# PKU-VCL-Geometry/GeoSplatting

Measured on AMD Instinct MI355X. Metric: fwd+bwd views/sec at 2M Gaussians, 800x800, higher is better.
Workload: dtype f32

## Files before the change

geosplatting_amd/_lib.py:

```python
from __future__ import annotations

import ctypes as C
import os
from typing import Optional

import torch

_HERE = os.path.dirname(os.path.abspath(__file__))
LIB_PATH = os.path.join(_HERE, "libgeosplat_hip.so")

GS_MAX_LEVELS = 16


class GsEnv(C.Structure):
    _fields_ = [("lut", C.c_void_p), ("lut_res", C.c_int), ("base", C.c_void_p), ("base_res", C.c_int),
                ("num_levels", C.c_int), ("levels", C.c_void_p * GS_MAX_LEVELS), ("res", C.c_int * GS_MAX_LEVELS),
                ("min_roughness", C.c_float), ("max_roughness", C.c_float)]


class GsTailView(C.Structure):
    _fields_ = [("viewmat", C.c_void_p), ("K", C.c_void_p), ("cam_pos", C.c_void_p), ("vis_records", C.c_void_p), ("v_packed", C.c_void_p),
                ("packed_index", C.c_void_p), ("W", C.c_int), ("H", C.c_int)]


class GsTileLevel(C.Structure):
    _fields_ = [("R", C.c_int), ("n_mirrors", C.c_int), ("margin", C.c_int), ("bw", C.c_int), ("nb", C.c_int), ("tile_begin", C.c_int),
                ("tile_end", C.c_int), ("reserved", C.c_int), ("src", C.c_void_p), ("scale", C.c_void_p), ("out_scale", C.c_void_p),
                ("bounds", C.c_void_p), ("tiles", C.c_void_p), ("segments", C.c_void_p), ("row_begin", C.c_void_p), ("row_counts", C.c_void_p),
                ("desc", C.c_void_p), ("weights", C.c_void_p), ("dst", C.c_void_p), ("lds_bytes", C.c_size_t)]


class GsDensifyTensor(C.Structure):
    _fields_ = [("src", C.c_void_p), ("dst", C.c_void_p), ("floats_per_row", C.c_int), ("kind", C.c_int)]


class GsTsdfView(C.Structure):
    _fields_ = [("depth_alpha", C.c_void_p), ("viewmat", C.c_void_p), ("K", C.c_void_p), ("W", C.c_int), ("H", C.c_int)]


class GsEnvGrad(C.Structure):
    _fields_ = [("base", C.c_void_p), ("levels", C.c_void_p * GS_MAX_LEVELS)]


SYMBOLS = [
    "gs_last_error", "gs_version", "gs_project_ws_bytes", "gs_project_fwd", "gs_project_fwd_vis", "gs_project_fwd_vis_ex", "gs_isect_emit", "gs_sort_ws_bytes",
    "gs_isect_sort", "gs_isect_bin_ws_bytes", "gs_isect_bin", "gs_isect_offsets", "gs_raster_ws_bytes", "gs_raster_fwd", "gs_raster_prepare", "gs_raster_prepare_vis", "gs_raster_composite", "gs_raster_grad_stride", "gs_raster_bwd", "gs_raster_bwd_acc", "gs_selftest_rcp", "gs_selftest_exp", "gs_selftest_cube_edges", "gs_isect_bin_cap", "gs_isect_offsets_cap", "gs_isect_bin_tiles_cap", "gs_isect_offsets_tiles_cap", "gs_raster_prepare_vis_cap", "gs_raster_composite_cap", "gs_raster_bwd_cap", "gs_raster_bwd_acc_cap", "gs_raster_composite_tone", "gs_raster_bwd_tone_acc", "gs_raster_log_ws_bytes", "gs_raster_composite_tone_log", "gs_raster_bwd_tone_log_acc", "gs_project_bwd_cap", "gs_project_bwd", "gs_project_bwd_ex", "gs_shade_fwd",
    "gs_shade_bwd_ws_bytes", "gs_shade_bwd_plan_blocks", "gs_shade_bwd", "gs_tonemap_fwd", "gs_tonemap_bwd", "gs_tonemap_fwd3", "gs_tonemap_bwd3", "gs_cubemap_mip_fwd", "gs_cubemap_mip_chain_fwd", "gs_cube_sample_linear",
    "gs_cubemap_mip_bwd", "gs_diffuse_cubemap_fwd", "gs_diffuse_cubemap_bwd", "gs_specular_bounds", "gs_specular_bounds_ws_bytes", "gs_specular_bounds_fast", "gs_cube_dir_table",
    "gs_specular_cubemap_fwd", "gs_specular_cubemap_bwd", "gs_specular_tiles_count", "gs_specular_tiles_fill",
    "gs_specular_tiles_check", "gs_specular_tiles_apply", "gs_specular_tiles_apply_multi", "gs_mgadapter_fwd", "gs_mgadapter_bwd", "gs_vertex_normals_fwd",
    "gs_vertex_normals_bwd", "gs_photo_loss_ws_bytes", "gs_photo_loss", "gs_smooth_loss_ws_bytes", "gs_smooth_loss", "gs_hashgrid_fwd", "gs_hashgrid_bwd_ws_bytes", "gs_hashgrid_bwd", "gs_hashgrid_bwd_fixed_ws_bytes", "gs_hashgrid_bwd_fixed", "gs_mlp_wgrad_ws_bytes", "gs_mlp_wgrad",
    "gs_flexicubes_ws_bytes", "gs_flexicubes_count", "gs_flexicubes_fwd", "gs_flexicubes_bwd", "gs_flexicubes_entropy_fwd",
    "gs_flexicubes_entropy_bwd", "gs_front_ws_bytes", "gs_front_fwd", "gs_isect_bin_front_ws_bytes", "gs_isect_bin_front", "gs_isect_bin_front_classes", "gs_tail_bwd", "gs_tail_bwd_multi", "gs_tail_bwd_multi_parts", "gs_tail_priv_ws_bytes", "gs_tail_priv_reduce", "gs_smooth_gather", "gs_smooth_fold", "gs_activation_chain",
    "gs_densify_stats", "gs_densify_ws_bytes", "gs_densify_plan", "gs_densify_fill",
    "gs_surfel_project_ws_bytes", "gs_surfel_project_fwd", "gs_surfel_project_bwd", "gs_surfel_raster_fwd", "gs_surfel_grad_stride",
    "gs_surfel_raster_bwd",
    "gs_tsdf_integrate", "gs_tsdf_extract_ws_bytes", "gs_tsdf_extract_count", "gs_tsdf_extract_fill",
    "gs_meshraster_ws_bytes", "gs_meshraster_fwd", "gs_meshraster_resolve", "gs_meshraster_bwd", "gs_mesh_interp_fwd",
    "gs_mesh_interp_bwd",
    "gs_mesh_topology_bytes", "gs_mesh_topology_build", "gs_meshaa_fwd", "gs_meshaa_bwd",
    "gs_tex2d_fwd", "gs_tex2d_bwd", "gs_meshshade_fwd", "gs_meshshade_bwd",
    "gs_bvh_bytes", "gs_bvh_ws_bytes", "gs_bvh_build", "gs_ray_occluded", "gs_ray_closest",
    "gs_envshade_fwd", "gs_envshade_bwd",
    "gs_denoise_tiled_fits", "gs_denoise_fwd", "gs_denoise_bwd",
]

_lib: Optional[C.CDLL] = None


class GeoSplatHipError(RuntimeError):
    pass


def lib() -> C.CDLL:
    global _lib
    if _lib is None:
        if not os.path.exists(LIB_PATH):
            raise GeoSplatHipError(
                f"{LIB_PATH} not found: build it with `python -m geosplatting_amd.build` "
                "(hipcc --offload-arch=gfx950).  geosplatting_amd has no CPU / PyTorch fallback.")
        l = C.CDLL(LIB_PATH)
        l.gs_last_error.restype = C.c_char_p
        l.gs_project_ws_bytes.restype = C.c_size_t
        l.gs_project_ws_bytes.argtypes = [C.c_int]
        l.gs_sort_ws_bytes.restype = C.c_size_t
        l.gs_sort_ws_bytes.argtypes = [C.c_int64, C.c_int, C.c_int]
        l.gs_isect_bin_ws_bytes.restype = C.c_size_t
        l.gs_isect_bin_ws_bytes.argtypes = [C.c_int, C.c_int64, C.c_int, C.c_int]
        l.gs_shade_bwd_ws_bytes.restype = C.c_size_t
        l.gs_shade_bwd_ws_bytes.argtypes = [C.c_void_p, C.c_int]
        l.gs_shade_bwd_plan_blocks.restype = C.c_int
        l.gs_shade_bwd_plan_blocks.argtypes = [C.c_void_p, C.c_int, C.c_int, C.c_void_p]
        l.gs_hashgrid_bwd_ws_bytes.restype = C.c_size_t
        l.gs_hashgrid_bwd_ws_bytes.argtypes = [C.c_int, C.c_int, C.c_int]
        l.gs_hashgrid_bwd_fixed_ws_bytes.restype = C.c_size_t
        l.gs_hashgrid_bwd_fixed_ws_bytes.argtypes = [C.c_int, C.c_int, C.c_int, C.c_int]
        l.gs_mlp_wgrad_ws_bytes.restype = C.c_size_t
        l.gs_mlp_wgrad_ws_bytes.argtypes = [C.c_int64]
        l.gs_flexicubes_ws_bytes.restype = C.c_size_t
        l.gs_flexicubes_ws_bytes.argtypes = [C.c_int, C.c_int, C.c_int]
        l.gs_photo_loss_ws_bytes.restype = C.c_size_t
        l.gs_photo_loss_ws_bytes.argtypes = [C.c_int, C.c_int]
        l.gs_smooth_loss_ws_bytes.restype = C.c_size_t
        l.gs_smooth_loss_ws_bytes.argtypes = [C.c_int, C.c_int]
        l.gs_specular_bounds_ws_bytes.restype = C.c_size_t
        l.gs_specular_bounds_ws_bytes.argtypes = [C.c_int]
        l.gs_front_ws_bytes.restype = C.c_size_t
        l.gs_front_ws_bytes.argtypes = [C.c_int]
        l.gs_isect_bin_front_ws_bytes.restype = C.c_size_t
        l.gs_isect_bin_front_ws_bytes.argtypes = [C.c_int, C.c_int64, C.c_int, C.c_int]
        l.gs_tail_priv_ws_bytes.restype = C.c_size_t
        l.gs_tail_priv_ws_bytes.argtypes = [C.c_void_p, C.c_int]
        l.gs_raster_log_ws_bytes.restype = C.c_size_t
        l.gs_raster_log_ws_bytes.argtypes = [C.c_int64, C.c_int, C.c_int, C.c_int]
        l.gs_raster_ws_bytes.restype = C.c_size_t
        l.gs_raster_ws_bytes.argtypes = [C.c_int64, C.c_int, C.c_int, C.c_int, C.c_int]
        l.gs_densify_ws_bytes.restype = C.c_size_t
        l.gs_densify_ws_bytes.argtypes = [C.c_int64, C.c_int]
        l.gs_surfel_project_ws_bytes.restype = C.c_size_t
        l.gs_surfel_project_ws_bytes.argtypes = [C.c_int]
        l.gs_tsdf_extract_ws_bytes.restype = C.c_size_t
        l.gs_tsdf_extract_ws_bytes.argtypes = [C.c_int, C.c_int, C.c_int]
        l.gs_tsdf_integrate.argtypes = [C.c_int, C.c_int, C.c_int, C.c_float, C.c_float, C.c_float, C.c_float, C.c_float, C.c_float,
                                        C.c_float, C.c_int, C.c_void_p, C.c_void_p, C.c_void_p]
        l.gs_tsdf_extract_count.argtypes = [C.c_int, C.c_int, C.c_int, C.c_void_p, C.c_void_p, C.c_size_t, C.c_void_p, C.c_void_p]
        l.gs_tsdf_extract_fill.argtypes = [C.c_int, C.c_int, C.c_int, C.c_float, C.c_float, C.c_float, C.c_float, C.c_void_p,
                                           C.c_void_p, C.c_size_t, C.c_int64, C.c_int64, C.c_void_p, C.c_void_p, C.c_void_p]
        l.gs_meshraster_ws_bytes.restype = C.c_size_t
        l.gs_meshraster_ws_bytes.argtypes = [C.c_int64, C.c_int, C.c_int]
        mesh_head = [C.c_int64, C.c_int64, C.c_void_p, C.c_void_p, C.c_float, C.c_float, C.c_float, C.c_float, C.c_int, C.c_int, C.c_float]
        l.gs_meshraster_fwd.argtypes = mesh_head + [C.c_int, C.c_void_p, C.c_size_t, C.c_void_p, C.c_void_p]
        l.gs_meshraster_resolve.argtypes = mesh_head + [C.c_void_p, C.c_size_t, C.c_void_p, C.c_void_p]
        l.gs_meshraster_bwd.argtypes = mesh_head + [C.c_void_p, C.c_void_p, C.c_void_p, C.c_void_p]
        l.gs_mesh_interp_fwd.argtypes = [C.c_int64, C.c_int, C.c_int64, C.c_int64, C.c_int, C.c_void_p, C.c_void_p, C.c_void_p, C.c_void_p,
                                         C.c_void_p]
        l.gs_mesh_interp_bwd.argtypes = [C.c_int64, C.c_int, C.c_int64, C.c_int64, C.c_int, C.c_void_p, C.c_void_p, C.c_void_p, C.c_void_p,
                                         C.c_void_p, C.c_void_p, C.c_void_p]
        l.gs_mesh_topology_bytes.restype = C.c_size_t
        l.gs_mesh_topology_bytes.argtypes = [C.c_int64]
        l.gs_mesh_topology_build.argtypes = [C.c_int64, C.c_void_p, C.c_void_p, C.c_size_t, C.c_void_p]
        aa_head = mesh_head + [C.c_int, C.c_void_p, C.c_size_t, C.c_int, C.c_void_p, C.c_void_p]
        l.gs_meshaa_fwd.argtypes = aa_head + [C.c_void_p, C.c_void_p, C.c_void_p]
        l.gs_meshaa_bwd.argtypes = aa_head + [C.c_void_p, C.c_void_p, C.c_void_p, C.c_void_p]
        tex_head = [C.c_int64, C.c_int, C.c_int, C.c_int, C.c_int, C.c_void_p, C.c_void_p]
        l.gs_tex2d_fwd.argtypes = tex_head + [C.c_void_p, C.c_void_p]
        l.gs_tex2d_bwd.argtypes = tex_head + [C.c_void_p, C.c_void_p, C.c_void_p, C.c_void_p]
        shade_head = [C.c_int, C.c_int, C.c_void_p, C.c_void_p, C.c_void_p, C.c_void_p, C.c_int, C.c_int, C.c_void_p, C.c_int, C.c_int,
                      C.c_void_p, C.c_void_p, C.c_void_p, C.c_int, C.c_float, C.c_int]
        l.gs_meshshade_fwd.argtypes = shade_head + [C.c_void_p, C.c_void_p]
        l.gs_meshshade_bwd.argtypes = shade_head + [C.c_void_p] * 8
        l.gs_bvh_bytes.restype = C.c_size_t
        l.gs_bvh_bytes.argtypes = [C.c_int64]
        l.gs_bvh_ws_bytes.restype = C.c_size_t
        l.gs_bvh_ws_bytes.argtypes = [C.c_int64]
        l.gs_bvh_build.argtypes = [C.c_int64, C.c_int64, C.c_void_p, C.c_void_p, C.c_void_p, C.c_size_t, C.c_void_p, C.c_size_t, C.c_void_p]
        ray_head = [C.c_int64, C.c_int64, C.c_void_p, C.c_void_p, C.c_void_p, C.c_int64, C.c_int, C.c_void_p, C.c_void_p, C.c_int,
                    C.c_float, C.c_float]
        l.gs_ray_occluded.argtypes = ray_head + [C.c_void_p, C.c_void_p]
        l.gs_ray_closest.argtypes = ray_head + [C.c_void_p, C.c_void_p, C.c_void_p, C.c_void_p]
        env_head = ([C.c_int64] + [C.c_void_p] * 7 + [C.c_int, C.c_int] + [C.c_void_p] * 4 + [C.c_int, C.c_int, C.c_void_p, C.c_int64, C.c_int,
                    C.c_float, C.c_int64, C.c_int64, C.c_void_p, C.c_void_p, C.c_void_p, C.c_int])
        l.gs_envshade_fwd.argtypes = env_head + [C.c_void_p] * 7
        l.gs_envshade_bwd.argtypes = env_head + [C.c_int] + [C.c_void_p] * 8
        l.gs_denoise_tiled_fits.argtypes = [C.c_int, C.c_double]
        l.gs_denoise_fwd.argtypes = [C.c_int] * 5 + [C.c_void_p] * 3 + [C.c_double, C.c_int] + [C.c_void_p] * 3
        l.gs_denoise_bwd.argtypes = [C.c_int] * 5 + [C.c_void_p] * 2 + [C.c_double, C.c_int] + [C.c_void_p] * 4
        _lib = l
    return _lib


def check(rc: int, what: str) -> None:
    if rc != 0:
        raise GeoSplatHipError(f"{what} failed ({rc}): {lib().gs_last_error().decode()}")


def ptr(t: Optional[torch.Tensor]) -> Optional[C.c_void_p]:
    if t is None:
        return None
    assert t.is_cuda and t.is_contiguous(), "device-resident contiguous tensors only"
    return C.c_void_p(t.data_ptr())


def stream() -> C.c_void_p:
    return C.c_void_p(torch.cuda.current_stream().cuda_stream)


def f32(x: float) -> C.c_float:
    return C.c_float(float(x))


def i64(x: int) -> C.c_int64:
    return C.c_int64(int(x))


def require_cuda(*tensors: torch.Tensor) -> None:
    for t in tensors:
        if t is not None and not t.is_cuda:
            raise GeoSplatHipError("geosplatting_amd ops run on the GPU only (tensor on %s); there is no CPU path" % t.device)


_shared_streams = {}


def shared_stream(device: torch.device, role: str) -> "torch.cuda.Stream":
    key = (device.index if device.index is not None else torch.cuda.current_device(), role)
    st = _shared_streams.get(key)
# ... 4 lines not shown
```

geosplatting_amd/csrc/gs_raster.hip:

```cpp
#include "gs_common.h"
#include "gs_tone.h"
#include <stdlib.h>

#pragma clang fp contract(off)

#define GS_TILE 16
#define GS_ALPHA_MIN (1.0f / 255.0f)

#ifdef GS_RASTER_STATS
__device__ unsigned long long g_raster_stats[8];
extern "C" int gs_raster_stats_read(unsigned long long* host8, int reset)
{
    if (hipMemcpyFromSymbol(host8, HIP_SYMBOL(g_raster_stats), sizeof(unsigned long long) * 8) != hipSuccess) return -1;
    if (reset) { unsigned long long z[8] = {0}; if (hipMemcpyToSymbol(HIP_SYMBOL(g_raster_stats), z, sizeof(z)) != hipSuccess) return -1; }
    return 0;
}
__device__ unsigned long long g_raster_stats2[8];
extern "C" int gs_raster_stats2_read(unsigned long long* host8, int reset)
{
    if (hipMemcpyFromSymbol(host8, HIP_SYMBOL(g_raster_stats2), sizeof(unsigned long long) * 8) != hipSuccess) return -1;
    if (reset) { unsigned long long z[8] = {0}; if (hipMemcpyToSymbol(HIP_SYMBOL(g_raster_stats2), z, sizeof(z)) != hipSuccess) return -1; }
    return 0;
}
__device__ unsigned long long g_raster_stats3[8];
// ... 1277 lines not shown
                    m2 = __builtin_elementwise_fma(sd, d, m2);
                    mxy = fmaf(sd.x, d.y, mxy);
                    c01 = __builtin_elementwise_fma((v2f)(f_w), v2f{vr.x, vr.y}, c01);
                    if (CD > 2) c2s = fmaf(f_w, vr.z, c2s);
                } while (__ballot(m != 0ull) != 0ull);
                sum[0] = m0; sum[1] = m1.x; sum[2] = m1.y; sum[3] = m2.x; sum[4] = mxy; sum[5] = m2.y;
                sum[6] = c01.x;
                if (CD > 1) sum[7] = c01.y;
                if (CD > 2) sum[8] = c2s;
            }
            lanes_lds_sync();
#ifdef GS_RASTER_PHASES
            if (blockIdx.x == 0 && threadIdx.x == 0) { const long long _t = (long long)__builtin_readcyclecounter(); atomicAdd(&g_raster_stats[3], (unsigned long long)(_t - _pw0)); _pw0 = _t; }
#endif
            {
                const float ga = ra4.z, gb = ra4.w, gc = rb4.x, go = rb4.y;
                const float M0 = sum[0], Mx = sum[1], My = sum[2];
                float out[NV];
                out[0] = (2.0f * ga) * Mx + gb * My;
                out[1] = gb * Mx + (2.0f * gc) * My;
                out[2] = 0.5f * sum[3]; out[3] = sum[4]; out[4] = 0.5f * sum[5];
                out[5] = (M0 != 0.0f) ? -M0 / go : 0.0f;
#pragma unroll
                for (int k = 0; k < CD; ++k) out[6 + k] = sum[6 + k];
                if (mine) {
#pragma unroll
                    for (int k = 0; k < NV; ++k) stage[lane * NV + k] = out[k];
                }
            }
            lanes_lds_sync();
            {
                const int r = lane / NV, k = lane - r * NV;
                for (int it = 0; r0 + it * RPI < r1; ++it) {
                    const int j = r0 + it * RPI + r;
                    if (r < RPI && j < r1 && k < 6 + D) {
                        const float v = stage[j * NV + k];
                        if (v != 0.0f) {
                            const int g = __float_as_int(qc[j].w);
                            gs_atomic_add(v_packed + (size_t)g * rec_stride + k, v);
                        }
                    }
                }
            }
#ifdef GS_RASTER_PHASES
            if (blockIdx.x == 0 && threadIdx.x == 0) atomicAdd(&g_raster_stats[4], (unsigned long long)((long long)__builtin_readcyclecounter() - _pw0));
#endif
            cumbase = __builtin_amdgcn_readlane(cum, r1 - 1);
            r0 = r1;
        }
    }
#if defined(GS_RASTER_STATS) && !defined(GS_RASTER_PHASES)
    if (lane == 0) {
#pragma unroll
        for (int k = 0; k < 8; ++k) if (walk_hist[k]) atomicAdd(&g_raster_stats3[k], (unsigned long long)walk_hist[k]);
    }
#endif
    GS_TL_END();
}

#define GS_RASTER_BLOCKS_PER_CU 4
static int gs_raster_blocks_per_cu() { return GS_RASTER_BLOCKS_PER_CU; }
static size_t gs_raster_lds_pad() { return (size_t)(160 * 1024 / gs_raster_blocks_per_cu()) - 1024; }
static size_t gs_raster_lds(size_t natural)
{
    const size_t pad = gs_raster_lds_pad();
    if (natural >= pad) return natural;
    if ((size_t)(gs_raster_blocks_per_cu() + 1) * (natural + 512) > (size_t)160 * 1024) return natural;
    return pad;
}
static size_t align256(size_t x) { return (x + 255) & ~(size_t)255; }

extern "C" size_t gs_raster_ws_bytes(int64_t n_isects, int V, int W, int H, int tile_size)
{
    if (tile_size <= 0) return 0;
    const size_t tiles = (size_t)((W + tile_size - 1) / tile_size) * (size_t)((H + tile_size - 1) / tile_size);
    const size_t n = n_isects > 0 ? (size_t)n_isects : 1;
    const size_t v = V > 0 ? (size_t)V : 1;
    return 3 * align256(n * sizeof(float4)) + align256(tiles * sizeof(int32_t)) + align256(64 * sizeof(int32_t)) +
           align256(64 * tiles * sizeof(int32_t)) + align256(4 * v * sizeof(float4));
}

struct RasterWs {
    float4 *rec0, *rec1, *rec2;
    int32_t* order;
    BwdOrder bo;
    float4* vis;
};
static RasterWs carve(void* ws, int64_t n_isects, int V, int tiles)
{
    const size_t n = n_isects > 0 ? (size_t)n_isects : 1;
    const size_t v = V > 0 ? (size_t)V : 1;
    char* p = (char*)ws;
    RasterWs r;
    r.rec0 = (float4*)p; p += align256(n * sizeof(float4));
    r.rec1 = (float4*)p; p += align256(n * sizeof(float4));
    r.rec2 = (float4*)p; p += align256(n * sizeof(float4));
    r.order = (int32_t*)p; p += align256((size_t)tiles * sizeof(int32_t));
    r.bo.bcount = (int32_t*)p; p += align256(64 * sizeof(int32_t));
    r.bo.blist = (int32_t*)p; p += align256(64 * (size_t)tiles * sizeof(int32_t));
    r.vis = (float4*)p;
    return r;
}

struct RasterOpts {
    const int64_t* counts = nullptr;
    ToneFwd tone_fwd = { 0, nullptr, nullptr };
    ToneBwd tone_bwd = { 0, nullptr, nullptr, nullptr, nullptr };
    CullLog log = { nullptr, nullptr, nullptr };
};
static GsCount isect_count(int64_t n, const RasterOpts& o)
{
    return GsCount{ (long long)n, o.counts ? (const long long*)o.counts + 1 : nullptr };
}

template <int CD>
static int launch_fwd(int W, int H, int D, const RasterWs& ws, const float* colors, const float* background,
                      int64_t n_isects, const int32_t* offsets, float* render, float* alphas, int32_t* last_ids,
                      hipStream_t s, const RasterOpts& o)
{
    const int tile_w = (W + GS_TILE - 1) / GS_TILE, tile_h = (H + GS_TILE - 1) / GS_TILE;
    if (o.tone_fwd.image && !(CD == 3 && D == 3 && background == nullptr)) {
        gs_set_error("gs_raster_composite_tone: needs D == 3 and no background");
        return GS_EINVAL;
    }
    {
        const size_t planes = CD > 3 ? 4 * (size_t)2 * (size_t)D * 64 * sizeof(float) : 0;
        const size_t lds = gs_raster_lds(4 * (size_t)GS_WIN_Q_BYTES + planes);
        if (lds > 64 * 1024)
            GS_CHECK_HIP(hipFuncSetAttribute((const void*)raster_fwd_window_kernel<CD>, hipFuncAttributeMaxDynamicSharedMemorySize, (int)lds));
        hipLaunchKernelGGL(raster_fwd_window_kernel<CD>, dim3(tile_w * tile_h), dim3(256), lds, s, W, H, tile_w, tile_w * tile_h, D,
                           ws.order, ws.rec0, ws.rec1, ws.rec2, colors, background, isect_count(n_isects, o), offsets, render, alphas,
                           last_ids, o.tone_fwd, o.log, o.log.count ? ws.bo : BwdOrder{ nullptr, nullptr });
        GS_CHECK_LAUNCH();
        return GS_OK;
    }
}

static int raster_check(const char* who, int W, int H, int tile_size, int D, int V, int64_t n_isects, const void* ws,
                        size_t ws_bytes)
{
    GS_CHECK_ARG(W > 0 && H > 0, "bad image size");
    GS_CHECK_ARG(tile_size == GS_TILE, "only tile_size=16 is built (rfstudio/model/gsplat.py:30)");
    GS_CHECK_ARG(D >= 1 && D <= GS_MAX_CHANNELS, "1 <= D <= 32");
    GS_CHECK_ARG(n_isects >= 0 && n_isects < (1ll << 31), "n_isects must fit int32");
    GS_CHECK_ARG(ws != nullptr, "workspace must not be NULL");
    GS_CHECK_ARG(V >= 0, "bad V");
    if (ws_bytes < gs_raster_ws_bytes(n_isects, V, W, H, tile_size)) { gs_set_error("%s: workspace too small", who); return GS_ENOSPC; }
    return GS_OK;
}

static int raster_prepare_impl(int W, int H, int tile_size, int D, int V, const float* means2d, const float* conics,
                               const float* opacities, const float* colors, const float* vis_records, int64_t n_isects,
                               const int32_t* offsets, const int32_t* flatten_ids, void* ws, size_t ws_bytes, void* stream,
                               const RasterOpts& o)
{
    const int rc = raster_check("gs_raster_prepare", W, H, tile_size, D, V, n_isects, ws, ws_bytes);
    if (rc != GS_OK) return rc;
    hipStream_t s = (hipStream_t)stream;
    const int tiles = ((W + GS_TILE - 1) / GS_TILE) * ((H + GS_TILE - 1) / GS_TILE);
    const RasterWs r = carve(ws, n_isects, V, tiles);
    if (n_isects > 0 && V > 0) {
        const float4* vis = (const float4*)vis_records;
        if (!vis) {
            hipLaunchKernelGGL(pack_visible_kernel, dim3(gs_cdiv(V, 256)), dim3(256), 0, s, V, D, means2d, conics, opacities, colors,
                               r.vis);
            GS_CHECK_LAUNCH();
            vis = r.vis;
        }
        hipLaunchKernelGGL(build_stream_packed_kernel, dim3(gs_cdiv(n_isects, 256)), dim3(256), 0, s, isect_count(n_isects, o), flatten_ids,
                           vis, r.rec0, r.rec1, r.rec2);
        GS_CHECK_LAUNCH();
    }
    hipLaunchKernelGGL(tile_order_kernel, dim3(1), dim3(1024), 0, s, tiles, isect_count(n_isects, o), offsets, r.order, r.bo);
    GS_CHECK_LAUNCH();
    return GS_OK;
}

static int raster_composite_impl(int W, int H, int tile_size, int D, int V, const float* colors, const float* background,
                                 int64_t n_isects, const int32_t* offsets, float* render, float* alphas, int32_t* last_ids,
                                 const void* ws, size_t ws_bytes, void* stream, const RasterOpts& o)
{
    const int rc = raster_check("gs_raster_composite", W, H, tile_size, D, V, n_isects, ws, ws_bytes);
    if (rc != GS_OK) return rc;
    hipStream_t s = (hipStream_t)stream;
    const int tiles = ((W + GS_TILE - 1) / GS_TILE) * ((H + GS_TILE - 1) / GS_TILE);
    const RasterWs r = carve((void*)ws, n_isects, V, tiles);
#define GS_FWD(CD) return launch_fwd<CD>(W, H, D, r, colors, background, n_isects, offsets, render, alphas, last_ids, s, o)
    if (D <= 3) GS_FWD(3);
    if (D <= 4) GS_FWD(4);
    if (D <= 8) GS_FWD(8);
    if (D <= 16) GS_FWD(16);
    GS_FWD(32);
#undef GS_FWD
}

template <int CD>
static int launch_bwd(int W, int H, int D, const RasterWs& ws, const float* colors, const float* background,
                      int64_t n_isects, const int32_t* offsets, const float* alphas, const int32_t* last_ids,
                      const float* v_render, const float* v_alphas, float* v_packed, int rec_stride, hipStream_t s,
                      const RasterOpts& o)
{
    const int tile_w = (W + GS_TILE - 1) / GS_TILE, tile_h = (H + GS_TILE - 1) / GS_TILE;
    if (o.tone_bwd.v_image && !(CD == 3 && D == 3 && background == nullptr)) {
        gs_set_error("gs_raster_bwd_tone: needs D == 3 and no background");
        return GS_EINVAL;
    }
    if constexpr (CD <= 3) {
        if (o.log.idx) {
            const size_t lds = gs_raster_lds(4 * (size_t)LogLds::WAVE_BYTES);
            hipLaunchKernelGGL(raster_bwd_log_kernel<CD>, dim3(tile_w * tile_h), dim3(256), lds, s, W, H, tile_w, tile_w * tile_h, D,
                               ws.order, ws.rec0, ws.rec1, ws.rec2, background, isect_count(n_isects, o), offsets, alphas, last_ids,
                               v_render, v_alphas, v_packed, rec_stride, o.tone_bwd, o.log, ws.bo);
            GS_CHECK_LAUNCH();
            return GS_OK;
        }
    }
    {
        size_t lds = 4 * ((size_t)Lanes2Lds<CD>::WAVE_BYTES + (CD > 3 ? 2 * (size_t)D * 64 * 4 : 0));
        if (lds < gs_raster_lds_pad()) lds = gs_raster_lds_pad();
        if (lds > 64 * 1024)
            GS_CHECK_HIP(hipFuncSetAttribute((const void*)raster_bwd_lanes2_kernel<CD>, hipFuncAttributeMaxDynamicSharedMemorySize, (int)lds));
        hipLaunchKernelGGL(raster_bwd_lanes2_kernel<CD>, dim3(tile_w * tile_h), dim3(256), lds, s, W, H, tile_w, tile_w * tile_h, D,
                           ws.order, ws.rec0, ws.rec1, ws.rec2, colors, background, isect_count(n_isects, o), offsets, alphas, last_ids,
                           v_render, v_alphas, v_packed, rec_stride, o.tone_bwd);
        GS_CHECK_LAUNCH();
        return GS_OK;
    }
}

extern "C" int gs_raster_grad_stride(int D) { return ((6 + D) + 15) / 16 * 16; }

static int raster_bwd_impl(int W, int H, int tile_size, int D, int V, const float* colors, const float* background,
                           int64_t n_isects, const int32_t* offsets, const float* alphas, const int32_t* last_ids,
                           const float* v_render, const float* v_alphas, float* v_packed, const void* ws,
                           size_t ws_bytes, void* stream, bool zero, const RasterOpts& o)
{
    const int rc = raster_check("gs_raster_bwd", W, H, tile_size, D, V, n_isects, ws, ws_bytes);
    if (rc != GS_OK) return rc;
    hipStream_t s = (hipStream_t)stream;
    const int rec_stride = gs_raster_grad_stride(D);
    if (V > 0 && zero) GS_CHECK_HIP(gs_zero_async(v_packed, sizeof(float) * (size_t)rec_stride * (size_t)V, s));
    if (n_isects == 0 || V == 0) return GS_OK;
    const int tiles = ((W + GS_TILE - 1) / GS_TILE) * ((H + GS_TILE - 1) / GS_TILE);
    const RasterWs r = carve((void*)ws, n_isects, V, tiles);
#define GS_BWD(CD) return launch_bwd<CD>(W, H, D, r, colors, background, n_isects, offsets, alphas, last_ids, v_render, v_alphas, v_packed, rec_stride, s, o)
    if (D <= 3) GS_BWD(3);
    if (D <= 4) GS_BWD(4);
    if (D <= 8) GS_BWD(8);
    if (D <= 16) GS_BWD(16);
    GS_BWD(32);
#undef GS_BWD
}

static CullLog carve_log(const void* log_ws, int64_t n_isects)
{
    const size_t n = n_isects > 0 ? (size_t)n_isects : 1;
    char* p = (char*)log_ws;
    CullLog l;
    l.mask = (unsigned long long*)p; p += align256(4 * n * sizeof(unsigned long long));
    l.idx = (int32_t*)p; p += align256(4 * n * sizeof(int32_t));
    l.count = (int32_t*)p;
    return l;
}
extern "C" size_t gs_raster_log_ws_bytes(int64_t n_isects, int W, int H, int tile_size)
{
    if (tile_size <= 0) return 0;
    const size_t n = n_isects > 0 ? (size_t)n_isects : 1;
    const size_t tiles = (size_t)((W + tile_size - 1) / tile_size) * (size_t)((H + tile_size - 1) / tile_size);
    return align256(4 * n * sizeof(unsigned long long)) + align256(4 * n * sizeof(int32_t)) + align256(4 * tiles * sizeof(int32_t));
}

extern "C" int gs_raster_prepare(int W, int H, int tile_size, int D, int V, const float* means2d, const float* conics,
                                 const float* opacities, const float* colors, int64_t n_isects, const int32_t* offsets,
                                 const int32_t* flatten_ids, void* ws, size_t ws_bytes, void* stream)
{
    return raster_prepare_impl(W, H, tile_size, D, V, means2d, conics, opacities, colors, nullptr, n_isects, offsets, flatten_ids,
                               ws, ws_bytes, stream, RasterOpts{});
}

extern "C" int gs_raster_prepare_vis(int W, int H, int tile_size, int D, int V, const float* vis_records, int64_t n_isects,
                                     const int32_t* offsets, const int32_t* flatten_ids, void* ws, size_t ws_bytes, void* stream)
{
    GS_CHECK_ARG(vis_records != nullptr || V == 0, "vis_records (written by gs_project_fwd_vis) must not be NULL");
    return raster_prepare_impl(W, H, tile_size, D, V, nullptr, nullptr, nullptr, nullptr, vis_records, n_isects, offsets,
                               flatten_ids, ws, ws_bytes, stream, RasterOpts{});
}

extern "C" int gs_raster_composite(int W, int H, int tile_size, int D, int V, const float* colors, const float* background,
                                   int64_t n_isects, const int32_t* offsets, float* render, float* alphas,
                                   int32_t* last_ids, const void* ws, size_t ws_bytes, void* stream)
{
    return raster_composite_impl(W, H, tile_size, D, V, colors, background, n_isects, offsets, render, alphas, last_ids, ws,
                                 ws_bytes, stream, RasterOpts{});
}

extern "C" int gs_raster_fwd(int W, int H, int tile_size, int D, int V, const float* means2d, const float* conics,
                             const float* opacities, const float* colors, const float* background,
                             int64_t n_isects, const int32_t* offsets, const int32_t* flatten_ids,
                             float* render, float* alphas, int32_t* last_ids, void* ws, size_t ws_bytes, void* stream)
{
    const int rc = raster_prepare_impl(W, H, tile_size, D, V, means2d, conics, opacities, colors, nullptr, n_isects, offsets,
                                       flatten_ids, ws, ws_bytes, stream, RasterOpts{});
    if (rc != GS_OK) return rc;
    return raster_composite_impl(W, H, tile_size, D, V, colors, background, n_isects, offsets, render, alphas, last_ids, ws,
                                 ws_bytes, stream, RasterOpts{});
}

extern "C" int gs_raster_bwd(int W, int H, int tile_size, int D, int V, const float* colors, const float* background,
                             int64_t n_isects, const int32_t* offsets, const float* alphas, const int32_t* last_ids,
                             const float* v_render, const float* v_alphas, float* v_packed, const void* ws,
                             size_t ws_bytes, void* stream)
{
    return raster_bwd_impl(W, H, tile_size, D, V, colors, background, n_isects, offsets, alphas, last_ids, v_render, v_alphas,
                           v_packed, ws, ws_bytes, stream, true, RasterOpts{});
}

extern "C" int gs_raster_bwd_acc(int W, int H, int tile_size, int D, int V, const float* colors, const float* background,
                                 int64_t n_isects, const int32_t* offsets, const float* alphas, const int32_t* last_ids,
                                 const float* v_render, const float* v_alphas, float* v_packed, const void* ws,
                                 size_t ws_bytes, void* stream)
{
    return raster_bwd_impl(W, H, tile_size, D, V, colors, background, n_isects, offsets, alphas, last_ids, v_render, v_alphas,
                           v_packed, ws, ws_bytes, stream, false, RasterOpts{});
}

extern "C" int gs_raster_prepare_vis_cap(int W, int H, int tile_size, int D, int V_cap, const float* vis_records, int64_t n_isects_cap,
                                         const int64_t* counts_dev, const int32_t* offsets, const int32_t* flatten_ids, void* ws,
                                         size_t ws_bytes, void* stream)
{
    GS_CHECK_ARG(counts_dev != nullptr, "counts_dev must not be NULL");
    GS_CHECK_ARG(vis_records != nullptr || V_cap == 0, "vis_records (written by gs_project_fwd_vis) must not be NULL");
    RasterOpts o;
    o.counts = counts_dev;
    return raster_prepare_impl(W, H, tile_size, D, V_cap, nullptr, nullptr, nullptr, nullptr, vis_records, n_isects_cap, offsets,
                               flatten_ids, ws, ws_bytes, stream, o);
}

extern "C" int gs_raster_composite_cap(int W, int H, int tile_size, int D, int V_cap, const float* colors, const float* background,
                                       int64_t n_isects_cap, const int64_t* counts_dev, const int32_t* offsets, float* render,
                                       float* alphas, int32_t* last_ids, const void* ws, size_t ws_bytes, void* stream)
{
    GS_CHECK_ARG(counts_dev != nullptr, "counts_dev must not be NULL");
    RasterOpts o;
    o.counts = counts_dev;
    return raster_composite_impl(W, H, tile_size, D, V_cap, colors, background, n_isects_cap, offsets, render, alphas, last_ids, ws,
                                 ws_bytes, stream, o);
}

extern "C" int gs_raster_bwd_cap(int W, int H, int tile_size, int D, int V_cap, const float* colors, const float* background,
                                 int64_t n_isects_cap, const int64_t* counts_dev, const int32_t* offsets, const float* alphas,
                                 const int32_t* last_ids, const float* v_render, const float* v_alphas, float* v_packed, const void* ws,
                                 size_t ws_bytes, void* stream)
{
    GS_CHECK_ARG(counts_dev != nullptr, "counts_dev must not be NULL");
    RasterOpts o;
    o.counts = counts_dev;
    return raster_bwd_impl(W, H, tile_size, D, V_cap, colors, background, n_isects_cap, offsets, alphas, last_ids, v_render, v_alphas,
                           v_packed, ws, ws_bytes, stream, true, o);
}

extern "C" int gs_raster_bwd_acc_cap(int W, int H, int tile_size, int D, int V_cap, const float* colors, const float* background,
                                     int64_t n_isects_cap, const int64_t* counts_dev, const int32_t* offsets, const float* alphas,
                                     const int32_t* last_ids, const float* v_render, const float* v_alphas, float* v_packed,
                                     const void* ws, size_t ws_bytes, void* stream)
{
    GS_CHECK_ARG(counts_dev != nullptr, "counts_dev must not be NULL");
    RasterOpts o;
    o.counts = counts_dev;
    return raster_bwd_impl(W, H, tile_size, D, V_cap, colors, background, n_isects_cap, offsets, alphas, last_ids, v_render, v_alphas,
                           v_packed, ws, ws_bytes, stream, false, o);
}

extern "C" int gs_raster_composite_tone(int W, int H, int tile_size, int V, const float* colors, int64_t n_isects,
                                        const int64_t* counts_dev, const int32_t* offsets, float* render, float* alphas,
                                        int32_t* last_ids, int tone_mode, const float* exposure, float* image, const void* ws,
                                        size_t ws_bytes, void* stream)
{
    GS_CHECK_ARG(tone_mode >= 0 && tone_mode <= 2 && exposure != nullptr && image != nullptr, "bad tone mode / exposure / image");
    RasterOpts o;
    o.counts = counts_dev;
    o.tone_fwd = ToneFwd{ tone_mode, exposure, (float4*)image };
    return raster_composite_impl(W, H, tile_size, 3, V, colors, nullptr, n_isects, offsets, render, alphas, last_ids, ws, ws_bytes,
                                 stream, o);
}

extern "C" int gs_raster_bwd_tone_acc(int W, int H, int tile_size, int V, const float* colors, int64_t n_isects,
                                      const int64_t* counts_dev, const int32_t* offsets, const float* render, const float* alphas,
                                      const int32_t* last_ids, int tone_mode, const float* exposure, const float* v_image,
                                      float* v_packed, float* v_exposure, const void* ws, size_t ws_bytes, void* stream)
{
    GS_CHECK_ARG(tone_mode >= 0 && tone_mode <= 2 && exposure != nullptr && v_image != nullptr && render != nullptr && v_exposure != nullptr,
                 "bad tone mode / exposure / v_image / render / v_exposure");
    RasterOpts o;
    o.counts = counts_dev;
    o.tone_bwd = ToneBwd{ tone_mode, exposure, render, (const float4*)v_image, v_exposure };
    return raster_bwd_impl(W, H, tile_size, 3, V, colors, nullptr, n_isects, offsets, alphas, last_ids, nullptr, nullptr, v_packed, ws,
                           ws_bytes, stream, false, o);
}

extern "C" int gs_raster_composite_tone_log(int W, int H, int tile_size, int V, const float* colors, int64_t n_isects,
                                            const int64_t* counts_dev, const int32_t* offsets, float* render, float* alphas,
                                            int32_t* last_ids, int tone_mode, const float* exposure, float* image, const void* ws,
                                            size_t ws_bytes, void* log_ws, size_t log_bytes, void* stream)
{
    GS_CHECK_ARG(log_ws != nullptr && tile_size == GS_TILE, "log_ws must not be NULL");
    if (log_bytes < gs_raster_log_ws_bytes(n_isects, W, H, tile_size)) { gs_set_error("gs_raster_composite_tone_log: log workspace too small"); return GS_ENOSPC; }
    GS_CHECK_ARG(tone_mode >= 0 && tone_mode <= 2 && exposure != nullptr && image != nullptr, "bad tone mode / exposure / image");
    RasterOpts o;
    o.counts = counts_dev;
    o.tone_fwd = ToneFwd{ tone_mode, exposure, (float4*)image };
    o.log = carve_log(log_ws, n_isects);
    return raster_composite_impl(W, H, tile_size, 3, V, colors, nullptr, n_isects, offsets, render, alphas, last_ids, ws, ws_bytes,
                                 stream, o);
}

extern "C" int gs_raster_bwd_tone_log_acc(int W, int H, int tile_size, int V, const float* colors, int64_t n_isects,
                                          const int64_t* counts_dev, const int32_t* offsets, const float* render, const float* alphas,
                                          const int32_t* last_ids, int tone_mode, const float* exposure, const float* v_image,
                                          float* v_packed, float* v_exposure, const void* ws, size_t ws_bytes, const void* log_ws,
                                          size_t log_bytes, void* stream)
{
    GS_CHECK_ARG(log_ws != nullptr && tile_size == GS_TILE, "log_ws must not be NULL");
    if (log_bytes < gs_raster_log_ws_bytes(n_isects, W, H, tile_size)) { gs_set_error("gs_raster_bwd_tone_log_acc: log workspace too small"); return GS_ENOSPC; }
    GS_CHECK_ARG(tone_mode >= 0 && tone_mode <= 2 && exposure != nullptr && v_image != nullptr && render != nullptr && v_exposure != nullptr,
                 "bad tone mode / exposure / v_image / render / v_exposure");
    RasterOpts o;
    o.counts = counts_dev;
    o.tone_bwd = ToneBwd{ tone_mode, exposure, render, (const float4*)v_image, v_exposure };
    o.log = carve_log(log_ws, n_isects);
    return raster_bwd_impl(W, H, tile_size, 3, V, colors, nullptr, n_isects, offsets, alphas, last_ids, nullptr, nullptr, v_packed, ws,
                           ws_bytes, stream, false, o);
}


__global__ void __launch_bounds__(256) selftest_rcp_kernel(uint32_t lo_bits, uint32_t hi_bits, unsigned long long* mismatches)
{
    const uint64_t n = (uint64_t)hi_bits - lo_bits + 1;
    unsigned long long bad = 0;
    for (uint64_t i = (uint64_t)blockIdx.x * blockDim.x + threadIdx.x; i < n; i += (uint64_t)gridDim.x * blockDim.x) {
        const float x = __uint_as_float(lo_bits + (uint32_t)i);
        const v2f r = gs_rcp_exact2(v2f{x, x});
        const float d = __fdiv_rn(1.0f, x);
        bad += (__float_as_uint(r.x) != __float_as_uint(d)) + (__float_as_uint(r.y) != __float_as_uint(d));
    }
    if (bad) atomicAdd(mismatches, bad);
}

extern "C" int gs_selftest_rcp(uint32_t lo_bits, uint32_t hi_bits, uint64_t* mismatches_dev, void* stream)
{
    GS_CHECK_ARG(mismatches_dev != nullptr && hi_bits >= lo_bits, "bad range");
    hipStream_t s = (hipStream_t)stream;
    GS_CHECK_HIP(gs_zero_async(mismatches_dev, sizeof(uint64_t), s));
    hipLaunchKernelGGL(selftest_rcp_kernel, dim3(4096), dim3(256), 0, s, lo_bits, hi_bits, (unsigned long long*)mismatches_dev);
    GS_CHECK_LAUNCH();
    return GS_OK;
}

__global__ void __launch_bounds__(256) selftest_exp_kernel(uint32_t lo_bits, uint32_t hi_bits, unsigned long long* out)
{
    const uint64_t n = (uint64_t)hi_bits - lo_bits + 1;
    unsigned long long sum = 0;
    double worst = 0.0;
    for (uint64_t i = (uint64_t)blockIdx.x * blockDim.x + threadIdx.x; i < n; i += (uint64_t)gridDim.x * blockDim.x) {
        const float x = __uint_as_float(lo_bits + (uint32_t)i);
        const float r = gs_exp_neg(x);
        sum += (unsigned long long)__float_as_uint(r) * (2ull * i + 1ull);
        const double ref = exp(-(double)x);
        const double e = fabs((double)r - ref) / ref;
        worst = e > worst ? e : worst;
    }
    atomicAdd(out, sum);
    atomicMax(out + 1, (unsigned long long)__double_as_longlong(worst));
}

extern "C" int gs_selftest_exp(uint32_t lo_bits, uint32_t hi_bits, uint64_t* out_dev, void* stream)
{
    GS_CHECK_ARG(out_dev != nullptr && hi_bits >= lo_bits, "bad range");
    hipStream_t s = (hipStream_t)stream;
    GS_CHECK_HIP(gs_zero_async(out_dev, 2 * sizeof(uint64_t), s));
    hipLaunchKernelGGL(selftest_exp_kernel, dim3(4096), dim3(256), 0, s, lo_bits, hi_bits, (unsigned long long*)out_dev);
    GS_CHECK_LAUNCH();
    return GS_OK;
}
```

geosplatting_amd/csrc/gs_sort.hip:

```cpp
#include "gs_common.h"
#include "gs_segsort_dev.h"

#include <cstdlib>
#include <cstring>

#define RS_THREADS 256
#define RS_WAVES 4
#define RS_ITEMS 8
#define RS_TILE (RS_THREADS * RS_ITEMS)
#define RS_WCHUNK (64 * RS_ITEMS)

typedef unsigned long long u64;

static int tile_bits(int tile_w, int tile_h)
{
    unsigned n = (unsigned)(tile_w * tile_h);
    int b = 0;
    while (n > 1) { n >>= 1; ++b; }
    return b + 1;
}

struct PairItem { u64 key; int32_t val; };
struct PairIn {
    const u64* keys; const int32_t* vals;
// ... 318 lines not shown
}

extern "C" int gs_isect_bin_tiles_cap(int V_cap, const float* means2d, const int32_t* radii, const float* depths, const int64_t* counts_dev,
                                      int64_t n_isects_cap, int tile_size, int tile_w, int tile_h, int32_t* tile_ids_sorted,
                                      int32_t* flatten_ids_sorted, void* ws, size_t ws_bytes, int64_t* status_dev, void* stream)
{
    GS_CHECK_ARG(counts_dev != nullptr && status_dev != nullptr && tile_ids_sorted != nullptr, "counts_dev / status_dev / tile_ids_sorted must not be NULL");
    hipLaunchKernelGGL(capacity_check_kernel, dim3(1), dim3(64), 0, (hipStream_t)stream, (const long long*)counts_dev, (long long)V_cap,
                       (long long)n_isects_cap, (long long*)status_dev);
    GS_CHECK_LAUNCH();
    return isect_bin_impl(V_cap, means2d, radii, depths, n_isects_cap, (const long long*)counts_dev, tile_size, tile_w, tile_h,
                          nullptr, flatten_ids_sorted, ws, ws_bytes, stream, tile_ids_sorted);
}

struct KeyIn {
    const unsigned* keys;
    __device__ __forceinline__ uint2 load(int64_t i) const { return make_uint2(keys[i], (unsigned)i); }
};
#define BF_HIST_MAX 8192

__global__ void __launch_bounds__(256)
bin_setup_kernel(unsigned* __restrict__ state, int n_state_words,
                 const long long* __restrict__ counts, long long v_cap, long long i_cap, long long* __restrict__ status)
{
    const int i = blockIdx.x * blockDim.x + threadIdx.x, stride = gridDim.x * blockDim.x;
    for (int k = i; k < n_state_words; k += stride) state[k] = 0u;
    if (i == 0 && counts != nullptr && status != nullptr) {
        const long long V = counts[0], I = counts[1];
        if (V > v_cap || I > i_cap) {
            status[0] = GS_ENOSPC;
            if (I > status[1]) status[1] = I;
            if (V > status[2]) status[2] = V;
        }
    }
}

#define BF_VALID (1ull << 63)
#define BF_SPIN_LIMIT (1 << 22)

__global__ void __launch_bounds__(EM_THREADS)
emit_chained_kernel(GsCount vc, const uint2* __restrict__ order, const uint2* __restrict__ rect, unsigned* __restrict__ ctrl,
                    u64* __restrict__ desc, int n_blocks, int tile_w, uint2* __restrict__ items, unsigned item_cap,
                    long long* __restrict__ status )
{
    const int V = (int)gs_count(vc);
    __shared__ unsigned ws[EM_THREADS / 64];
    __shared__ unsigned s_block;
    __shared__ unsigned long long s_base;
    const int lane = threadIdx.x & 63, wave = threadIdx.x >> 6;
    if (threadIdx.x == 0) s_block = atomicAdd(ctrl, 1u);
    __syncthreads();
    const int block = (int)s_block;
    u64* agg = desc; u64* pre = desc + n_blocks;
    const int r0 = block * EM_TILE + (int)threadIdx.x * EM_PER;
    int v[EM_PER]; unsigned c[EM_PER]; uint2 q[EM_PER];
    unsigned mine = 0u;
#pragma unroll
    for (int k = 0; k < EM_PER; ++k) {
        const int r = r0 + k;
        v[k] = r < V ? (int)order[r].y : -1;
        q[k] = v[k] >= 0 ? rect[v[k]] : make_uint2(0u, 0u);
        c[k] = rect_count(q[k]);
        mine += c[k];
    }
    unsigned incl = mine;
    incl = gs_wave_incl_scan(incl);
    if (lane == 63) ws[wave] = incl;
    __syncthreads();
    unsigned before = 0u, total = 0u;
    for (int w = 0; w < EM_THREADS / 64; ++w) { if (w < wave) before += ws[w]; total += ws[w]; }
    if (wave == 0) {
        unsigned long long acc = 0ull;
        if (block > 0) {
            if (lane == 0) __hip_atomic_store(&agg[block], (u64)total | BF_VALID, __ATOMIC_RELAXED, __HIP_MEMORY_SCOPE_AGENT);
            int pos = block - 1;
            bool done = false;
            while (!done) {
                u64 pv[EM_LOOK], av[EM_LOOK];
#pragma unroll
                for (int j = 0; j < EM_LOOK; ++j) {
                    const int idx = pos - 64 * j - lane;
                    pv[j] = av[j] = 0ull;
                    if (idx >= 0) {
                        pv[j] = __hip_atomic_load(&pre[idx], __ATOMIC_RELAXED, __HIP_MEMORY_SCOPE_AGENT);
                        av[j] = __hip_atomic_load(&agg[idx], __ATOMIC_RELAXED, __HIP_MEMORY_SCOPE_AGENT);
                    }
                }
#pragma unroll
                for (int j = 0; j < EM_LOOK; ++j) {
                    if (done) break;
                    const int idx = pos - 64 * j - lane;
                    bool isP = idx < 0;
                    u64 val = 0ull;
                    if (idx >= 0) {
                        int spins = 0;
                        for (;;) {
                            if (pv[j] & BF_VALID) { isP = true; val = pv[j]; break; }
                            if (av[j] & BF_VALID) { val = av[j]; break; }
                            if (++spins > BF_SPIN_LIMIT) { atomicExch(ctrl + 1, 1u); if (status) status[0] = GS_ENOSPC; break; }
                            __builtin_amdgcn_s_sleep(2);
                            pv[j] = __hip_atomic_load(&pre[idx], __ATOMIC_RELAXED, __HIP_MEMORY_SCOPE_AGENT);
                            av[j] = __hip_atomic_load(&agg[idx], __ATOMIC_RELAXED, __HIP_MEMORY_SCOPE_AGENT);
                        }
                    }
                    const u64 pmask = __ballot(isP);
                    const int first = pmask ? __builtin_ctzll(pmask) : 64;
                    if (lane <= first) acc += val & ~BF_VALID;
                    if (pmask) done = true;
                }
                pos -= 64 * EM_LOOK;
            }
        }
        const unsigned long long base = gs_wave_sum_u64(acc);
        if (lane == 0) {
            __hip_atomic_store(&pre[block], (u64)(base + total) | BF_VALID, __ATOMIC_RELAXED, __HIP_MEMORY_SCOPE_AGENT);
            s_base = base;
        }
    }
    __syncthreads();
    unsigned long long cur = s_base + before + incl - mine;
#pragma unroll
    for (int k = 0; k < EM_PER; ++k) {
        if (v[k] < 0 || c[k] == 0u) continue;
        const int x0 = (int)(q[k].x & 0xffffu), y0 = (int)(q[k].x >> 16), x1 = (int)(q[k].y & 0xffffu), y1 = (int)(q[k].y >> 16);
        for (int i = y0; i < y1; ++i)
            for (int j = x0; j < x1; ++j) {
                const unsigned t = (unsigned)(i * tile_w + j);
                if (cur < (unsigned long long)item_cap) items[cur] = make_uint2(t, (unsigned)v[k]);
                ++cur;
            }
    }
}

#define SEG_CLASSES 2
#define SEG_CAP0 2048
#define SEG_LG_CHUNK 13
#define SEG_CHUNK (1 << SEG_LG_CHUNK)
#define SEG_GMAX 4
#define SEG_THREADS(cap) ((cap) >> SEG_GMAX)
#define SEG_BINS 64
static size_t seg_lds_bytes(int cap) { return (size_t)(cap + (cap >> 5) + 1) * sizeof(u64); }

extern "C" int gs_isect_bin_front_classes(int* caps, int max)
{
    const int c[2] = { SEG_CAP0, SEG_CHUNK };
    for (int i = 0; i < 2 && i < max; ++i) if (caps) caps[i] = c[i];
    return 2;
}

struct SegLists {
    unsigned* count; int32_t* lists;
    unsigned* cursor;
    const long long* counts; long long v_cap, i_cap; long long* status;
};

__device__ __forceinline__ int seg_class(unsigned len) { return len <= SEG_CAP0 ? 0 : 1; }
__device__ __forceinline__ int seg_bin(unsigned len)
{
    const int l2 = 31 - __clz((int)len);
    const int half = l2 > 0 ? (int)((len >> (l2 - 1)) & 1u) : 0;
    return SEG_BINS - 1 - (2 * l2 + half);
}

__global__ void __launch_bounds__(1024)
tile_offsets_scan_kernel(int n_tiles, const unsigned* __restrict__ tile_counts, GsCount nc, int32_t* __restrict__ offsets, SegLists sl)
{
    __shared__ unsigned wsum[16];
    __shared__ unsigned s_bin[SEG_CLASSES * SEG_BINS];
    const unsigned n = (unsigned)gs_count(nc);
    const int lane = threadIdx.x & 63, wave = threadIdx.x >> 6;
    if (sl.count && threadIdx.x < SEG_CLASSES * SEG_BINS) s_bin[threadIdx.x] = 0u;
    if (sl.count && threadIdx.x == 0 && sl.counts != nullptr && sl.status != nullptr) {
        const long long V = sl.counts[0], I = sl.counts[1];
        if (V > sl.v_cap || I > sl.i_cap) {
            sl.status[0] = GS_ENOSPC;
            if (I > sl.status[1]) sl.status[1] = I;
            if (V > sl.status[2]) sl.status[2] = V;
        }
    }
    __syncthreads();
    unsigned carry = 0u;
    for (int i0 = 0; i0 < n_tiles; i0 += 1024) {
        const int i = i0 + threadIdx.x;
        const unsigned v = i < n_tiles ? tile_counts[i] : 0u;
        unsigned incl = v;
        incl = gs_wave_incl_scan(incl);
        if (lane == 63) wsum[wave] = incl;
        __syncthreads();
        unsigned before = 0u, all = 0u;
        for (int w = 0; w < 16; ++w) { if (w < wave) before += wsum[w]; all += wsum[w]; }
        if (i < n_tiles) {
            const unsigned o = carry + before + incl - v;
            const unsigned beg = o < n ? o : n, end = o + v < n ? o + v : n;
            offsets[i] = (int32_t)beg;
            if (sl.count) sl.cursor[i] = 0u;
            if (sl.count && end > beg) atomicAdd(&s_bin[seg_class(end - beg) * SEG_BINS + seg_bin(end - beg)], 1u);
        }
        carry += all;
        __syncthreads();
    }
    if (!sl.count) return;
    if (wave < SEG_CLASSES) {
        const unsigned v = s_bin[wave * SEG_BINS + lane];
        const unsigned incl = gs_wave_incl_scan(v);
        s_bin[wave * SEG_BINS + lane] = incl - v;
        if (lane == 63) sl.count[wave] = incl;
    }
    __syncthreads();
    for (int i = threadIdx.x; i < n_tiles; i += 1024) {
        const unsigned beg = (unsigned)offsets[i];
        unsigned end = n;
        if (i + 1 < n_tiles) end = (unsigned)__hip_atomic_load(&offsets[i + 1], __ATOMIC_RELAXED, __HIP_MEMORY_SCOPE_WORKGROUP);
        if (end > beg) {
            const int c = seg_class(end - beg);
            const unsigned pos = atomicAdd(&s_bin[c * SEG_BINS + seg_bin(end - beg)], 1u);
            sl.lists[(size_t)c * n_tiles + pos] = i;
        }
    }
}

#define SC_THREADS 512
#define SC_PER 8
#define SC_TILE (SC_THREADS * SC_PER)

__global__ void __launch_bounds__(SC_THREADS)
bin_scatter_kernel(GsCount vc, const unsigned* __restrict__ keys, const uint2* __restrict__ rects, unsigned key_mask, u64 item_bias, int tile_w, int tile_h,
                   const int32_t* __restrict__ offsets, unsigned* __restrict__ cursor, u64* __restrict__ items, unsigned item_cap)
{
    extern __shared__ unsigned s_pos[];
    const int V = (int)gs_count(vc);
    const int n_tiles = tile_w * tile_h;
    const int s0 = (int)blockIdx.x * SC_TILE + (int)threadIdx.x;
    if ((long long)blockIdx.x * SC_TILE >= V) return;
    for (int t = threadIdx.x; t < n_tiles; t += SC_THREADS) s_pos[t] = 0u;
    unsigned key[SC_PER]; uint2 q[SC_PER];
#pragma unroll
    for (int k = 0; k < SC_PER; ++k) {
        const int v = s0 + k * SC_THREADS;
        const int vv = v < V ? v : V - 1;
        key[k] = keys[vv];
        q[k] = rects[vv];
        if (v >= V) q[k] = make_uint2(0u, 0u);
    }
#pragma unroll
    for (int k = 0; k < SC_PER; ++k) {
        int x1 = (int)(q[k].y & 0xffffu), y1 = (int)(q[k].y >> 16);
        x1 = x1 < tile_w ? x1 : tile_w; y1 = y1 < tile_h ? y1 : tile_h;
        q[k].y = (unsigned)x1 | ((unsigned)y1 << 16);
    }
    __syncthreads();
#pragma unroll
    for (int k = 0; k < SC_PER; ++k) {
        const int x0 = (int)(q[k].x & 0xffffu), y0 = (int)(q[k].x >> 16), x1 = (int)(q[k].y & 0xffffu), y1 = (int)(q[k].y >> 16);
        for (int i = y0; i < y1; ++i)
            for (int j = x0; j < x1; ++j) atomicAdd(&s_pos[i * tile_w + j], 1u);
    }
    __syncthreads();
    for (int t0 = threadIdx.x; t0 < n_tiles; t0 += 4 * SC_THREADS) {
        unsigned c[4], o[4], b[4];
#pragma unroll
        for (int u = 0; u < 4; ++u) {
            const int t = t0 + u * SC_THREADS;
            c[u] = t < n_tiles ? s_pos[t] : 0u;
            o[u] = c[u] ? (unsigned)offsets[t] : 0u;
        }
#pragma unroll
        for (int u = 0; u < 4; ++u) b[u] = c[u] ? atomicAdd(&cursor[t0 + u * SC_THREADS], c[u]) : 0u;
#pragma unroll
        for (int u = 0; u < 4; ++u) if (c[u]) s_pos[t0 + u * SC_THREADS] = o[u] + b[u];
    }
    __syncthreads();
#pragma unroll
    for (int k = 0; k < SC_PER; ++k) {
        const int x0 = (int)(q[k].x & 0xffffu), y0 = (int)(q[k].x >> 16), x1 = (int)(q[k].y & 0xffffu), y1 = (int)(q[k].y >> 16);
        const u64 item = item_bias | ((u64)(key[k] & key_mask) << 31) | (u64)(unsigned)(s0 + k * SC_THREADS);
        for (int i = y0; i < y1; ++i)
            for (int j = x0; j < x1; ++j) {
                const unsigned pos = atomicAdd(&s_pos[i * tile_w + j], 1u);
                if (pos < item_cap) items[pos] = item;
            }
    }
}

template <int THREADS, bool F64>
__global__ void __launch_bounds__(THREADS)
seg_sort_kernel(const int32_t* __restrict__ list, const unsigned* __restrict__ list_count, int n_tiles, const int32_t* __restrict__ offsets,
                GsCount ic, GsCount vc, u64* items, int32_t* __restrict__ flat)
{
    extern __shared__ u64 s_seg[];
    if (blockIdx.x >= *list_count) return;
    const int t = list[blockIdx.x];
    const int n_all = (int)gs_count(ic);
    const int beg = offsets[t], end = t + 1 < n_tiles ? offsets[t + 1] : n_all;
    const int n = end - beg;
    if (n <= 0) return;
    const long long V = gs_count(vc);
    const unsigned vmax = V > 0 ? (unsigned)(V - 1) : 0u;
    const int tid = threadIdx.x;
    int P = 1 << SEG_GMAX;
    while (P < n) P <<= 1;
    for (int i = tid; i < P; i += THREADS) s_seg[gs_seg_phys<true>(i)] = i < n ? items[beg + i] : gs_seg_inf<F64>();
    __syncthreads();
    GS_SEG_SORT_BODY(SEG_GMAX, true, F64, false, s_seg, n, P, tid, THREADS, __syncthreads());
    for (int i = tid; i < n; i += THREADS) {
        const unsigned slot = (unsigned)s_seg[gs_seg_phys<true>(i)] & 0x7fffffffu;
        flat[beg + i] = (int32_t)(slot < vmax ? slot : vmax);
    }
}

template <int THREADS, int LG_CHUNK, bool F64>
__global__ void __launch_bounds__(THREADS)
seg_sort_large_kernel(const int32_t* __restrict__ list, const unsigned* __restrict__ list_count, int n_tiles, const int32_t* __restrict__ offsets,
                      GsCount ic, GsCount vc, u64* items, int32_t* __restrict__ flat)
{
    __shared__ u64 s_seg[(1 << LG_CHUNK) + (1 << (LG_CHUNK - 5)) + 1];
    if (blockIdx.x >= *list_count) return;
    const int t = list[blockIdx.x];
    const int n_all = (int)gs_count(ic);
    const int beg = offsets[t], end = t + 1 < n_tiles ? offsets[t + 1] : n_all;
    const int n = end - beg;
    if (n <= 0) return;
    const long long V = gs_count(vc);
    const unsigned vmax = V > 0 ? (unsigned)(V - 1) : 0u;
    gs_seg_hybrid<SEG_GMAX, LG_CHUNK, THREADS, F64>(s_seg, items + beg, n, (int)threadIdx.x, [] { __syncthreads(); },
        [=](int i, u64 w) {
            const unsigned slot = (unsigned)w & 0x7fffffffu;
            flat[beg + i] = (int32_t)(slot < vmax ? slot : vmax);
        });
}

__global__ void __launch_bounds__(256)
bin_offsets_tiles_kernel(GsCount nc, const int32_t* __restrict__ tiles, int n_tiles, int32_t* __restrict__ offsets)
{
    const int64_t n = gs_count(nc);
    const int64_t i = (int64_t)blockIdx.x * blockDim.x + threadIdx.x;
    if (n == 0 && i == 0)
        for (int t = 0; t < n_tiles; ++t) offsets[t] = 0;
    if (i >= n) return;
    const int cur = tiles[i];
    if (i == 0) {
        for (int t = 0; t <= cur && t < n_tiles; ++t) offsets[t] = 0;
    } else {
        const int prev = tiles[i - 1];
        for (int t = prev + 1; t <= cur && t < n_tiles; ++t) offsets[t] = (int32_t)i;
    }
    if (i == n - 1)
        for (int t = cur + 1; t < n_tiles; ++t) offsets[t] = (int32_t)n;
}


static size_t tf_state_words(int n_tiles) { return (size_t)n_tiles + SEG_CLASSES; }
static size_t tf_ws_bytes(int64_t n_isects, int n_tiles)
{
    return align256(tf_state_words(n_tiles) * 4) + align256((size_t)SEG_CLASSES * n_tiles * 4) + align256((size_t)n_isects * 8) + 256;
}
static size_t bf_radix_ws_bytes(size_t v, size_t n)
{
    return table_bytes((int64_t)(v > n ? v : n)) + 2 * align256(v * 8) + 2 * align256(n * 8) + bf_state_bytes((int)v) + align256(n * 4) + 256;
}

extern "C" size_t gs_isect_bin_front_ws_bytes(int V, int64_t n_isects, int tile_w, int tile_h)
{
    const size_t v = V > 0 ? (size_t)V : 1, n = n_isects > 0 ? (size_t)n_isects : 1;
    const int64_t n_tiles = (int64_t)tile_w * tile_h;
    if (n_tiles > 0 && n_tiles <= BF_HIST_MAX) return tf_ws_bytes((int64_t)n, (int)n_tiles);
    return bf_radix_ws_bytes(v, n);
}

static int bin_front_tile_first(int V, const uint32_t* depth_keys, const uint32_t* tile_rects, const uint32_t* tile_counts,
                                const int64_t* counts_dev, int64_t n_isects, int key_bits, int tile_w, int tile_h, int32_t* flatten_ids_sorted,
                                int32_t* isect_offsets, void* ws, int64_t* status_dev, hipStream_t s)
{
    const int n_tiles = tile_w * tile_h;
    const GsCount vc{ (long long)V, (const long long*)counts_dev }, ic{ (long long)n_isects, counts_dev ? (const long long*)counts_dev + 1 : nullptr };
    char* p = (char*)ws;
    unsigned* cursor = (unsigned*)p;
    unsigned* class_count = cursor + n_tiles; p += align256(tf_state_words(n_tiles) * 4);
    int32_t* lists = (int32_t*)p; p += align256((size_t)SEG_CLASSES * n_tiles * 4);
    u64* items = (u64*)p;
    hipLaunchKernelGGL(tile_offsets_scan_kernel, dim3(1), dim3(1024), 0, s, n_tiles, (const unsigned*)tile_counts, ic, isect_offsets,
                       SegLists{ class_count, lists, cursor, (const long long*)counts_dev, (long long)V, (long long)n_isects, (long long*)status_dev });
    GS_CHECK_LAUNCH();
    const bool f64 = key_bits == 24;
    hipLaunchKernelGGL(bin_scatter_kernel, dim3(gs_cdiv(V, SC_TILE)), dim3(SC_THREADS), (size_t)n_tiles * 4, s, vc,
                       (const unsigned*)depth_keys, (const uint2*)tile_rects, f64 ? 0xffffffu : 0xffffffffu, f64 ? (1ull << 62) : 0ull, tile_w, tile_h,
                       (const int32_t*)isect_offsets, cursor, items, (unsigned)n_isects);
    GS_CHECK_LAUNCH();
    const int caps[SEG_CLASSES] = { 0, SEG_CAP0 };
    for (int c = 0; c < SEG_CLASSES; ++c) {
        const int64_t most = n_isects / (caps[c] + 1);
        const int grid = (int)(most < n_tiles ? most : n_tiles);
        if (grid == 0) continue;
        const int32_t* list = lists + (size_t)c * n_tiles;
#define SEG_LAUNCH(KERNEL, T, LDS) hipLaunchKernelGGL(KERNEL, dim3(grid), dim3(T), LDS, s, list, (const unsigned*)(class_count + c), n_tiles, \
                                                      (const int32_t*)isect_offsets, ic, vc, items, flatten_ids_sorted)
        if (c == 0) {
            if (f64) SEG_LAUNCH((seg_sort_kernel<SEG_THREADS(SEG_CAP0), true>), SEG_THREADS(SEG_CAP0), seg_lds_bytes(SEG_CAP0));
            else SEG_LAUNCH((seg_sort_kernel<SEG_THREADS(SEG_CAP0), false>), SEG_THREADS(SEG_CAP0), seg_lds_bytes(SEG_CAP0));
        } else {
            if (f64) SEG_LAUNCH((seg_sort_large_kernel<SEG_THREADS(SEG_CHUNK), SEG_LG_CHUNK, true>), SEG_THREADS(SEG_CHUNK), 0);
            else SEG_LAUNCH((seg_sort_large_kernel<SEG_THREADS(SEG_CHUNK), SEG_LG_CHUNK, false>), SEG_THREADS(SEG_CHUNK), 0);
        }
#undef SEG_LAUNCH
        GS_CHECK_LAUNCH();
    }
    return GS_OK;
}

extern "C" int gs_isect_bin_front(int V_cap, const uint32_t* depth_keys, const uint32_t* tile_rects, const uint32_t* tile_counts,
                                  const int64_t* counts_dev, int64_t n_isects_cap, int key_bits, int tile_w, int tile_h, int32_t* flatten_ids_sorted,
                                  int32_t* isect_offsets, void* ws, size_t ws_bytes, int64_t* status_dev, void* stream)
{
    const int V = V_cap;
    const int64_t n_isects = n_isects_cap;
    GS_CHECK_ARG(V >= 0 && n_isects >= 0 && tile_w > 0 && tile_h > 0 && (key_bits == 24 || key_bits == 32), "bad sizes or key width");
    GS_CHECK_ARG(n_isects < (1ll << 31), "n_isects must fit int32");
    GS_CHECK_ARG((int64_t)tile_w * tile_h < (1ll << 24) && tile_w < 65536 && tile_h < 65536, "tile grid too large");
    GS_CHECK_ARG(isect_offsets != nullptr && (counts_dev == nullptr || status_dev != nullptr), "null argument");
    hipStream_t s = (hipStream_t)stream;
    const int n_tiles = tile_w * tile_h;
    if (V == 0 || n_isects == 0) { GS_CHECK_HIP(gs_zero_async(isect_offsets, sizeof(int32_t) * (size_t)n_tiles, s)); return GS_OK; }
    GS_CHECK_ARG(depth_keys != nullptr && tile_rects != nullptr && flatten_ids_sorted != nullptr && ws != nullptr, "null argument");
    if (tile_counts != nullptr && n_tiles <= BF_HIST_MAX) {
        if (ws_bytes < tf_ws_bytes(n_isects, n_tiles)) { gs_set_error("gs_isect_bin_front: workspace too small"); return GS_ENOSPC; }
        return bin_front_tile_first(V, depth_keys, tile_rects, tile_counts, counts_dev, n_isects, key_bits, tile_w, tile_h, flatten_ids_sorted,
                                    isect_offsets, ws, status_dev, s);
    }
    if (ws_bytes < bf_radix_ws_bytes((size_t)V, (size_t)n_isects)) { gs_set_error("gs_isect_bin_front: workspace too small for the radix path (no tile_counts)"); return GS_ENOSPC; }
    const GsCount vc{ (long long)V, (const long long*)counts_dev }, ic{ (long long)n_isects, counts_dev ? (const long long*)counts_dev + 1 : nullptr };
    char* p = (char*)ws;
    unsigned* table = (unsigned*)p; p += table_bytes((int64_t)V > n_isects ? (int64_t)V : n_isects);
    uint2* da = (uint2*)p; p += align256((size_t)V * 8);
    uint2* db = (uint2*)p; p += align256((size_t)V * 8);
    uint2* ia = (uint2*)p; p += align256((size_t)n_isects * 8);
    uint2* ib = (uint2*)p; p += align256((size_t)n_isects * 8);
    unsigned* state = (unsigned*)p; p += bf_state_bytes(V);
    int32_t* tile_ids = (int32_t*)p;
    const int eblocks = (V + EM_TILE - 1) / EM_TILE;
    const int n_state_words = (int)(bf_state_bytes(V) / 4);
    hipLaunchKernelGGL(bin_setup_kernel, dim3(gs_cdiv(n_state_words, 256) < 64 ? gs_cdiv(n_state_words, 256) : 64),
                       dim3(256), 0, s, state, n_state_words, (const long long*)counts_dev,
                       (long long)V_cap, (long long)n_isects_cap, (long long*)status_dev);
    GS_CHECK_LAUNCH();
    int rc = radix_pass<uint2>(vc, KeyIn{ depth_keys }, XDigit{ 0, 255u }, U2Out{ da }, 8, table, s);
    if (rc != GS_OK) return rc;
    rc = radix_pass<uint2>(vc, U2In{ da }, XDigit{ 8, 255u }, U2Out{ db }, 8, table, s);
    if (rc != GS_OK) return rc;
    rc = radix_pass<uint2>(vc, U2In{ db }, XDigit{ 16, 255u }, U2Out{ da }, 8, table, s);
    if (rc != GS_OK) return rc;
    const uint2* order = da;
    if (key_bits == 32) {
        rc = radix_pass<uint2>(vc, U2In{ da }, XDigit{ 24, 255u }, U2Out{ db }, 8, table, s);
        if (rc != GS_OK) return rc;
        order = db;
    }
    unsigned* ctrl = state; u64* desc = (u64*)((char*)state + 16);
    hipLaunchKernelGGL(emit_chained_kernel, dim3(eblocks), dim3(EM_THREADS), 0, s, vc, order, (const uint2*)tile_rects, ctrl, desc,
                       eblocks + 1, tile_w, ia, (unsigned)n_isects, (long long*)status_dev);
    GS_CHECK_LAUNCH();
    int tb = 0;
    while ((1 << tb) < n_tiles) ++tb;
    if (tb < 1) tb = 1;
    const int npass = (tb + 7) / 8, width = (tb + npass - 1) / npass;
    uint2* src = ia; uint2* dst = ib;
    for (int pass = 0; pass < npass; ++pass) {
        const int shift = pass * width;
        const int nbits = (tb - shift) < width ? (tb - shift) : width;
        if (pass == npass - 1)
            rc = radix_pass<uint2>(ic, U2In{ src }, XDigit{ shift, (1u << nbits) - 1u }, FinalTiles{ tile_ids, flatten_ids_sorted }, nbits, table, s);
        else
            rc = radix_pass<uint2>(ic, U2In{ src }, XDigit{ shift, (1u << nbits) - 1u }, U2Out{ dst }, nbits, table, s);
        if (rc != GS_OK) return rc;
        uint2* t = src; src = dst; dst = t;
    }
    hipLaunchKernelGGL(bin_offsets_tiles_kernel, dim3(gs_cdiv(n_isects, 256)), dim3(256), 0, s, ic, tile_ids, n_tiles, isect_offsets);
    GS_CHECK_LAUNCH();
    return GS_OK;
}

static int isect_bin_impl(int V, const float* means2d, const int32_t* radii, const float* depths, int64_t n_isects,
                          const long long* counts_dev, int tile_size, int tile_w, int tile_h, int64_t* isect_ids_sorted,
                          int32_t* flatten_ids_sorted, void* ws, size_t ws_bytes, void* stream, int32_t* tile_ids_sorted)
{
    const GsCount vc{ (long long)V, counts_dev }, ic{ (long long)n_isects, counts_dev ? counts_dev + 1 : nullptr };
    GS_CHECK_ARG(V >= 0 && n_isects >= 0 && tile_size > 0 && tile_w > 0 && tile_h > 0, "bad sizes");
    GS_CHECK_ARG(n_isects < (1ll << 31), "n_isects must fit int32");
    GS_CHECK_ARG((int64_t)tile_w * tile_h < (1ll << 24), "more than 2^24 tiles");
    if (V == 0 || n_isects == 0) return GS_OK;
    GS_CHECK_ARG(ws != nullptr, "workspace must not be NULL");
    if (ws_bytes < gs_isect_bin_ws_bytes(V, n_isects, tile_w, tile_h)) { gs_set_error("gs_isect_bin: workspace too small"); return GS_ENOSPC; }
    hipStream_t s = (hipStream_t)stream;
    char* p = (char*)ws;
    unsigned* table = (unsigned*)p; p += table_bytes((int64_t)V > n_isects ? (int64_t)V : n_isects);
    uint2* da = (uint2*)p; p += align256((size_t)V * 8);
    uint2* db = (uint2*)p; p += align256((size_t)V * 8);
    uint2* rect = (uint2*)p; p += align256((size_t)V * 8);
    const int eblocks = (V + EM_TILE - 1) / EM_TILE;
    unsigned* state = (unsigned*)p; p += bf_state_bytes(V);
    uint2* ia = (uint2*)p; p += align256((size_t)n_isects * 8);
    uint2* ib = (uint2*)p; p += align256((size_t)n_isects * 8);
    int tb = 0;
    while ((1 << tb) < tile_w * tile_h) ++tb;
    if (tb < 1) tb = 1;
    const int npass = (tb + 7) / 8, width = (tb + npass - 1) / npass;
    int rc = GS_OK;
    rc = radix_pass<uint2>(vc, DepthIn{ depths }, XDigit{ 0, 255u }, U2Out{ da }, 8, table, s);
    if (rc != GS_OK) return rc;
    rc = radix_pass<uint2>(vc, U2In{ da }, XDigit{ 8, 255u }, U2Out{ db }, 8, table, s);
    if (rc != GS_OK) return rc;
    rc = radix_pass<uint2>(vc, U2In{ db }, XDigit{ 16, 255u }, U2Out{ da }, 8, table, s);
    if (rc != GS_OK) return rc;
    rc = radix_pass<uint2>(vc, U2In{ da }, XDigit{ 24, 255u }, U2Out{ db }, 8, table, s);
    if (rc != GS_OK) return rc;
    GS_CHECK_ARG(tile_w < 65536 && tile_h < 65536, "tile grid too large");
    hipLaunchKernelGGL(tile_rect_kernel, dim3(gs_cdiv(V, 256)), dim3(256), 0, s, vc, means2d, radii, tile_size, tile_w, tile_h, rect);
    GS_CHECK_LAUNCH();
    {
        const int n_state_words = (int)(bf_state_bytes(V) / 4);
        hipLaunchKernelGGL(bin_setup_kernel, dim3(gs_cdiv(n_state_words, 256) < 64 ? gs_cdiv(n_state_words, 256) : 64), dim3(256), 0, s, state,
                           n_state_words, (const long long*)nullptr, 0ll, 0ll, (long long*)nullptr);
        GS_CHECK_LAUNCH();
        hipLaunchKernelGGL(emit_chained_kernel, dim3(eblocks), dim3(EM_THREADS), 0, s, vc, (const uint2*)db, (const uint2*)rect, state,
                           (u64*)((char*)state + 16), eblocks + 1, tile_w, ia, (unsigned)n_isects, (long long*)nullptr);
        GS_CHECK_LAUNCH();
    }
    uint2* src = ia; uint2* dst = ib;
    for (int pass = 0; pass < npass; ++pass) {
        const int shift = pass * width;
        const int nbits = (tb - shift) < width ? (tb - shift) : width;
        if (pass == npass - 1 && tile_ids_sorted != nullptr)
            rc = radix_pass<uint2>(ic, U2In{ src }, XDigit{ shift, (1u << nbits) - 1u },
                                   FinalTiles{ tile_ids_sorted, flatten_ids_sorted }, nbits, table, s);
        else if (pass == npass - 1)
            rc = radix_pass<uint2>(ic, U2In{ src }, XDigit{ shift, (1u << nbits) - 1u },
                                   FinalOut{ (u64*)isect_ids_sorted, flatten_ids_sorted, depths }, nbits, table, s);
        else
            rc = radix_pass<uint2>(ic, U2In{ src }, XDigit{ shift, (1u << nbits) - 1u }, U2Out{ dst }, nbits, table, s);
        if (rc != GS_OK) return rc;
        uint2* t = src; src = dst; dst = t;
    }
    return GS_OK;
}
```

geosplatting_amd/engine.py:

```python
from __future__ import annotations

import collections
import contextlib
import os
from dataclasses import dataclass
from typing import Callable, Dict, List, Optional, Sequence, Tuple

import torch
from torch import Tensor

from . import _lib as L
from .cameras import Camera
from .parallel import GradBucket, collectives_active
from . import front as F
from .shading import _MODE, _TONE, RenderableAttrs, _make_env, get_fg_lut
from .splitsum import TextureSplitSum, as_splitsum, as_splitsum_backward, as_splitsum_forward, can_shard_prefilter
from .splats import SplatSet

PARAM_NAMES = ("means", "scales", "quats", "opacities", "normals", "kd", "ks", "cubemap", "exposure")


@dataclass
class PathParams:
    means: Tensor; scales: Tensor; quats: Tensor; opacities: Tensor
    normals: Tensor; kd: Tensor; ks: Tensor
    cubemap: Tensor
    exposure: Tensor

    def named(self) -> Dict[str, Tensor]:
        return {k: getattr(self, k) for k in PARAM_NAMES}

    def shapes(self) -> Dict[str, Sequence[int]]:
        return {k: tuple(v.shape) if v.dim() > 0 else (1,) for k, v in self.named().items()}


def _auto_tail_schedule(n_views: int):
    if n_views <= 4:
        return {0: [1], 1: [1], 2: [1, 1], 3: [2, 1], 4: [2, 1, 1]}[max(n_views, 0)]
    r, sched = n_views - 2, []
    while r > 0:
        k = 3 if (r >= 3 and r != 4) else min(r, 2)
        sched.append(k)
        r -= k
    return sched + [2]


@dataclass
class Smoothing:
    kinds: Tuple[int, int, int]
    weights: Tuple[float, float, float]
    background: Tensor
    gt: Optional[Sequence[Tensor]] = None


@dataclass
class _Geometry:
    scales_act: Tensor; opac_act: Tensor
    i_cap: Optional[int]
    key_bits: int; key_base: int
    status: Optional[Tensor]
    tight: bool
    early: Dict[int, Tuple[Tensor, Tensor]]


@dataclass
class _Views:
    b: Dict[str, Tensor]
    images: Optional[List[Tensor]]
    g_base: Tensor; g_levels: List[Tensor]; g_flat: Tensor
    env: TextureSplitSum
    sharded: bool; world: int; all_reduce: bool
    main: Optional[torch.cuda.Stream]
    pstream: Optional[torch.cuda.Stream]
    tail_job: Optional[dict]
    smooth_grads: Optional[Tuple[Tensor, Tensor, Tensor]] = None
    captured: bool = False


class RenderStep:
    def __init__(self, params: PathParams, min_roughness: float = 0.1, max_metallic: float = 1.0, mode: str = "pbr",
                 tone_type: str = "naive", prefilter: bool = True, fused: bool = True, fg_lut: Optional[Tensor] = None):
        self.p = params
        self.fg_lut = None if fg_lut is None else fg_lut.to(params.means.device, torch.float32).contiguous()
        self.min_roughness, self.max_metallic, self.mode, self.tone_type = min_roughness, max_metallic, mode, tone_type
        self.prefilter = prefilter
        self.fused = fused
        self.bucket = GradBucket(params.shapes(), params.means.device)
        self._static_env: Optional[TextureSplitSum] = None
        self._cameras = F.CameraCache(params.means.device)
        self._side_stream = None
        self._tail_stream = None
        self._use_capacity = os.environ.get("GEOSPLAT_CAPACITY", "1") != "0"
        self._key_lo = self._key_hi = None
        self._key32 = os.environ.get("GEOSPLAT_KEY_BITS", "24") == "32"
        self._cap_margin = float(os.environ.get("GEOSPLAT_CAPACITY_MARGIN", "1.25"))
        self._i_cap = None
        self._status = None
        self._status_host = None
        self._status_event = None
        self._status_pending = collections.deque()
        self._status_pool = []
        self.kernel_events = None
        self.tail_events = None
        self._seen_counts = []
        self._exact_max_i = 0
        self._pre_group = None
        self.truncated_steps = 0
        self.chunked_tails = 0
        self._overflow_unreported = False
        n_fly = int(os.environ.get("GEOSPLAT_STEPS_IN_FLIGHT", "3"))
        self._max_in_flight = max(1, n_fly)
        self._in_flight = collections.deque() if n_fly > 0 else None
        self.last_smoothing_loss = None
        self.last_attribute_renders = None

    def _prefilter_group(self):
        import torch.distributed as dist
        if self._pre_group is None:
            self._pre_group = dist.new_group()
        return self._pre_group

    def rebind(self, params: PathParams) -> None:
        self.p = params
        if {k: tuple(v) for k, v in params.shapes().items()} != self.bucket.shapes:
            self.bucket = GradBucket(params.shapes(), params.means.device, comm_stream=self.bucket.comm_stream)

    @property
    def _cam_cache(self):
        return {k: (e[0], e[1], k[3], e[2], e[3]) for k, e in self._cameras.entries.items()}

    def invalidate_cameras(self) -> None:
        self._cameras.clear()

    def _activations(self, out: Optional[Tuple[Tensor, Tensor]] = None) -> Tuple[Tensor, Tensor]:
        p = self.p
        if out is None:
            return p.scales.detach().exp(), torch.sigmoid(p.opacities.detach()).squeeze(-1).contiguous()
        torch.exp(p.scales.detach(), out=out[0])
        torch.sigmoid(p.opacities.detach().squeeze(-1), out=out[1])
        return out

    def _geometry(self, cameras, bin_first: bool, act: Optional[Tuple[Tensor, Tensor]] = None) -> _Geometry:
        p = self.p
        dev = p.means.device
        scales_act, opac_act = act if act is not None else self._activations()
        main = torch.cuda.current_stream(dev)
        if self._use_capacity and self._status is None:
            self._status = torch.zeros(4, dtype=torch.int64, device=dev)
        if self._side_stream is None:
            self._side_stream = F.front_streams(dev)
        tight = os.environ.get("GEOSPLAT_TIGHT_TILES", "1") != "0"
        i_cap = self._i_cap if self._use_capacity else None
        key_bits, key_base = F.binning_keys(self._key_lo, self._key_hi) if (i_cap is not None and not self._key32) else (32, 0)
        status = self._status if (key_bits == 24 or self._use_capacity) else None
        geo = _Geometry(scales_act, opac_act, i_cap, key_bits, key_base, status, tight, {})
        if bin_first and i_cap is not None and len(cameras) > 0:
            side = self._side_stream[0]
            ev_a = torch.cuda.Event(); ev_a.record(main)
            side.wait_event(ev_a)
            cam_t = self._cameras.get(cameras[0], side)
            with torch.cuda.stream(side):
                fr = self._front(geo, cameras[0], cam_t, None, records=False)
                binned, _, _ = F.bin_stage(fr, i_cap, self._status, prepare=False)
            self._seen_counts.append((fr.host_counts, fr.event))
            geo.early[0] = (binned["flatten_ids"], binned["isect_offsets"])
            for t in (scales_act, opac_act):
                t.record_stream(side)
        return geo

    def _front(self, geo: _Geometry, cam: Camera, cam_t, e, records: bool = True, binning: bool = True) -> F.Front:
        p = self.p
        keys = (geo.key_base, geo.key_bits, geo.status) if binning else (0, 32, None)
        return F.front_stage(p.means.detach(), p.quats.detach(), geo.scales_act, geo.opac_act, p.normals.detach(), p.kd.detach(),
                             p.ks.detach(), *cam_t, e, cam.width, cam.height, self.min_roughness, self.max_metallic, _MODE[self.mode],
                             *keys, want_packed_index=records, records=records, binning=binning, tight_tiles=geo.tight)

    def _env_args(self, env: TextureSplitSum):
        env_d = TextureSplitSum(env.base.detach(), [l.detach().contiguous() for l in env.levels], env.min_roughness, env.max_roughness)
        return env_d, _make_env(get_fg_lut(self.p.means.device) if self.fg_lut is None else self.fg_lut, env_d)

    def _records(self, cameras, geo: _Geometry, env: TextureSplitSum) -> Dict[int, F.Front]:
        _, e = self._env_args(env)
        cur = torch.cuda.current_stream(self.p.means.device)
        return {j: self._front(geo, cameras[j], self._cameras.get(cameras[j], cur), e, binning=False) for j in sorted(geo.early)}

    def _pyramid(self, sharded: bool, world: int) -> TextureSplitSum:
        if not self.prefilter:
            if self._static_env is None:
                self._static_env = as_splitsum_forward(self.p.cubemap)
            return self._static_env
        if sharded:
            import torch.distributed as dist
            return as_splitsum_forward(self.p.cubemap, rank=dist.get_rank(), world=world, group=self._prefilter_group(), sharded=True)
        return as_splitsum_forward(self.p.cubemap)

    def _sharding(self, all_reduce: bool):
        import torch.distributed as dist
        world = dist.get_world_size() if (all_reduce and dist.is_available() and dist.is_initialized()) else 1
        sharded = (self.prefilter and all_reduce and collectives_active() and os.environ.get("GEOSPLAT_SHARD_PREFILTER", "1") != "0"
                   and can_shard_prefilter(int(self.p.cubemap.shape[1]), world))
        return world, sharded

    def _views(self, cameras, upstream, all_reduce, keep_images, geo: _Geometry, env: Optional[TextureSplitSum] = None,
               recs: Optional[Dict[int, F.Front]] = None, smoothing: Optional[Smoothing] = None) -> _Views:
        lib = L.lib()
        p = self.p
        dev = p.means.device
        N = p.means.shape[0]
        f32 = torch.float32
        st = L.stream
        mode, tone = _MODE[self.mode], _TONE[self.tone_type]
        world, sharded = self._sharding(all_reduce)
        scales_act, opac_act = geo.scales_act, geo.opac_act
        means, quats = p.means.detach(), p.quats.detach()
        normals, kd, ks = p.normals.detach(), p.kd.detach(), p.ks.detach()
        main = torch.cuda.current_stream(dev)
        sides = self._side_stream
        i_cap, early = geo.i_cap, geo.early
        cres = int(p.cubemap.shape[1])
        tex_res = [cres]
        while tex_res[-1] > 16:
            tex_res.append(tex_res[-1] // 2)
        tex_sizes = [6 * tex_res[-1] * tex_res[-1] * 3] + [6 * r * r * 3 for r in tex_res]
        sm_sizes = [3 * N, 2 * N, 3 * N, 1, max([c.width * c.height for c in cameras] + [1])] if smoothing is not None else []
        sc = self.bucket.zero_with_scratch([3 * N, N, sum(tex_sizes)] + sm_sizes)
        b = self.bucket.unpack()
        smooth_grads = None
        self.last_smoothing_loss = self.last_attribute_renders = None
        if smoothing is not None:
            smooth_grads = (sc[3].view(N, 3), sc[4].view(N, 2), sc[5].view(N, 3))
            smooth_loss, zero_alphas = sc[6].view(()), sc[7]
            bg9 = smoothing.background.detach().to(dev, f32).reshape(3).repeat(3).contiguous()
            self.last_smoothing_loss = smooth_loss
            self.last_attribute_renders = [] if keep_images else None
        g_scales_act = sc[0].view(N, 3); g_opac_act = sc[1]
        exposure = p.exposure.detach().reshape(1).contiguous()
        if env is None:
            env = self._pyramid(sharded, world)
        env_d, e = self._env_args(env)
        g_flat, g_base, g_levels, eg = F.texel_grads(env_d, sc[2])
        self.last_texel_grads = (g_base, g_levels)
        images = []
        tail = self._tail_stream
        if tail is None:
            tail = self._tail_stream = L.shared_stream(dev, "tail")
        for sd in sides:
            sd.wait_stream(main)
        tail.wait_stream(main)

        tail_sched = F.tail_schedule(_auto_tail_schedule(len(cameras)))
        pending_tails = []
        n_tail_launches = 0
        pstream = None
        n_chunks = max(1, int(os.environ.get("GEOSPLAT_TAIL_CHUNKS", "4")))
        defer_tail = all_reduce and collectives_active() and n_chunks > 1 and N >= 4096
        tail_job = None

        cam_ts = {}

        def start_view(cam, j):
            side = sides[j % len(sides)]
            cam_t = cam_ts[j] = self._cameras.get(cam, side)
            if recs is not None and j in recs:
                return recs[j], j, side
            with torch.cuda.stream(side):
                fr = self._front(geo, cam, cam_t, e, binning=j not in early)
            return fr, j, side

        def bin_view(item):
            fr, j, side = item
            with torch.cuda.stream(side):
                if i_cap is not None:
                    self._seen_counts.append((fr.host_counts, fr.event))
                state, V, I = F.bin_stage(fr, i_cap, self._status, binned=early.get(j))
                if i_cap is None:
                    self._exact_max_i = max(self._exact_max_i, I)
                    self._key_lo, self._key_hi = F.learn_depth_range(self._key_lo, self._key_hi, fr.host_counts)
                    F.release_counts4(fr.host_counts)
                state["v_packed"] = torch.zeros(max(V, 1), lib.gs_raster_grad_stride(3), dtype=f32, device=dev)
                if smoothing is not None:
                    state["v_packed9"] = torch.zeros(max(V, 1), lib.gs_raster_grad_stride(9), dtype=f32, device=dev)
                ev = torch.cuda.Event(); ev.record(side)
            for t in state.values():
                if isinstance(t, torch.Tensor):
                    t.record_stream(main)
            return state, V, I, ev

        n_views = len(cameras)
        proj = [start_view(cameras[j], j) for j in range(min(2, n_views))]
        binned = bin_view(proj.pop(0)) if n_views else None
        for i, cam in enumerate(cameras):
            vm, K, cam_pos = cam_ts.pop(i)
            W, H = cam.width, cam.height
            s, V, I, ev = binned
            main.wait_event(ev)
            kev = self.kernel_events
            if kev is not None:
                k0 = torch.cuda.Event(enable_timing=True); k0.record(main)
            log_ws = F.log_ws(I, W, H, dev)
            img, render, alphas, last_ids = F.composite_fwd(s, V, I, W, H, tone, exposure, log_ws)
            if kev is not None:
                k1 = torch.cuda.Event(enable_timing=True); k1.record(main)
                kev.append(("raster_fwd_kernel", k0, k1))
            v_img = upstream(i, img).contiguous()
            if kev is not None:
                k2 = torch.cuda.Event(enable_timing=True); k2.record(main)
            F.composite_bwd(s, V, I, W, H, tone, exposure, render, alphas, last_ids, log_ws, v_img, b["exposure"])
            if kev is not None:
                k3 = torch.cuda.Event(enable_timing=True); k3.record(main)
                kev.append(("raster_bwd_kernel", k2, k3))
            if smoothing is not None:
                attr = F.smooth_view(s, V, I, W, H, kd, ks, normals, bg9, None if smoothing.gt is None else smoothing.gt[i],
                                     smoothing.kinds, smoothing.weights, smooth_loss, zero_alphas, *smooth_grads)
                if keep_images:
                    self.last_attribute_renders.append(attr)
            if i + 2 < n_views:
                proj.append(start_view(cameras[i + 2], i + 2))
            binned = bin_view(proj.pop(0)) if i + 1 < n_views else None
            pending_tails.append((vm, K, cam_pos, s["vis_records"], s["v_packed"], s["packed_index"], W, H))
            last = i == n_views - 1
            if len(pending_tails) == tail_sched[min(n_tail_launches, len(tail_sched) - 1)] or last:
                targs = (means, quats, scales_act, opac_act, normals, kd, ks, e, eg, self.min_roughness, self.max_metallic, mode,
                         b["means"], b["quats"], g_scales_act, g_opac_act, b["normals"], b["kd"], b["ks"])
                if last and defer_tail:
                    tail_job = dict(targs=(pending_tails,) + targs, accumulate=n_tail_launches > 0, n_chunks=n_chunks)
                else:
                    used = F.tail_batch(pending_tails, targs, n_tail_launches > 0, last, tail, sides[0], self.tail_events)
                    if last:
                        pstream = used[1]
                    n_tail_launches += 1
                    pending_tails = []
            if keep_images:
                images.append(img)
        main.wait_stream(tail)
        if smooth_grads is not None and tail_job is None:
            for name, g in zip(("kd", "ks", "normals"), smooth_grads):
                b[name].add_(g)
            if pstream is not None:
                pstream.wait_stream(main)
            smooth_grads = None
        if i_cap is not None:
            if torch.cuda.is_current_stream_capturing():
                if self._status_host is None:
                    self._status_host = torch.zeros(4, dtype=torch.int64).pin_memory()
                self._status_host.copy_(self._status, non_blocking=True)
                self._status_event = torch.cuda.Event(); self._status_event.record()
            else:
                snap = self._status_pool.pop() if self._status_pool else torch.zeros(4, dtype=torch.int64).pin_memory()
                snap.copy_(self._status, non_blocking=True)
                self._status.fill_(0)
                ev_s = torch.cuda.Event(); ev_s.record()
                self._status_pending.append((snap, ev_s))
        if tail_job is None:
            with torch.cuda.stream(pstream if pstream is not None else main):
                L.check(lib.gs_activation_chain(L.i64(N), L.ptr(g_scales_act), L.ptr(scales_act), L.ptr(g_opac_act), L.ptr(opac_act),
                                                L.ptr(b["scales"]), L.ptr(b["opacities"]), st()), "gs_activation_chain")
            if pstream is not None:
                for t in (scales_act, opac_act):
                    t.record_stream(pstream)
        return _Views(b, images if keep_images else None, g_base, g_levels, g_flat, env, sharded, world, all_reduce, main, pstream,
                      tail_job, smooth_grads)

    def _step(self, cameras, upstream, all_reduce, keep_images, smoothing: Optional[Smoothing] = None):
        geo = self._geometry(cameras, bin_first=self.prefilter)
        return self._finish(self._views(cameras, upstream, all_reduce, keep_images, geo, smoothing=smoothing))

    def _finish(self, ctx: _Views):
        import torch.distributed as dist
        b, env, main = ctx.b, ctx.env, ctx.main
        pstream = ctx.pstream
        chunked = ctx.tail_job is not None
        if chunked:
            pstream = self._chunked_tail(ctx)
            main.wait_stream(self._tail_stream)
        head_stream = pstream if pstream is not None else main
        if ctx.sharded:
            grp = self._prefilter_group()
            dist.all_reduce(ctx.g_flat, op=dist.ReduceOp.SUM, group=grp)
            if not chunked:
                start_head, _ = self.bucket.all_reduce_split("cubemap")
                with torch.cuda.stream(head_stream):
                    start_head()
            g_cube = as_splitsum_backward(ctx.g_base, ctx.g_levels, min_roughness=env.min_roughness, max_roughness=env.max_roughness,
                                          rank=dist.get_rank(), world=ctx.world, group=grp, sharded=True)
            b["cubemap"].copy_(g_cube)
            if pstream is not None:
                main.wait_stream(pstream)
            self.bucket.all_reduce_names(["exposure"])
            return b, ctx.images
        start_head, finish = self.bucket.all_reduce_split("cubemap") if ctx.all_reduce else ((lambda: None), (lambda: None))
        if not chunked:
            with torch.cuda.stream(head_stream):
                start_head()
        if self.prefilter:
            as_splitsum_backward(ctx.g_base, ctx.g_levels, min_roughness=env.min_roughness, max_roughness=env.max_roughness,
                                 out=b["cubemap"])
        if pstream is not None:
            main.wait_stream(pstream)
        finish()
        return b, ctx.images

    def _chunked_tail(self, ctx: _Views):
        job = ctx.tail_job
        lib = L.lib()
        b = ctx.b
        self.chunked_tails += 1
        (views, means, quats, scales_act, opac_act, normals, kd, ks, e, eg, mr, mm, mode, g_means, g_quats, g_scales_act, g_opac_act,
         g_normals, g_kd, g_ks) = job["targs"]
        N = means.shape[0]
        C_ = job["n_chunks"]
        bounds = [min(N, ((N * k // C_ + 1023) // 1024) * 1024) for k in range(C_)] + [N]
        tail, pstream = self._tail_stream, self._side_stream[0]
        names = [k for k in PARAM_NAMES if k not in ("cubemap", "exposure")]
        tail.wait_stream(ctx.main)
        for c in range(C_):
            n0, n1 = bounds[c], bounds[c + 1]
            if n1 <= n0:
                continue
            sl = lambda t: t[n0:n1]
            vc = [(vm, K, cp, vis, vp, pidx[n0:n1], W, H) for (vm, K, cp, vis, vp, pidx, W, H) in views]
            args = (vc, sl(means), sl(quats), sl(scales_act), sl(opac_act), sl(normals), sl(kd), sl(ks), e, eg, mr, mm, mode, sl(g_means),
                    sl(g_quats), sl(g_scales_act), sl(g_opac_act), sl(g_normals), sl(g_kd), sl(g_ks))
            with torch.cuda.stream(tail):
                F.tail_multi_stage(*args, accumulate=job["accumulate"], parts=1)
                ev_sh = torch.cuda.Event(); ev_sh.record(tail)
            with torch.cuda.stream(pstream):
                pstream.wait_event(ev_sh)
                F.tail_multi_stage(*args, accumulate=job["accumulate"], parts=2)
                L.check(lib.gs_activation_chain(L.i64(n1 - n0), L.ptr(sl(g_scales_act)), L.ptr(sl(scales_act)), L.ptr(sl(g_opac_act)),
                                                L.ptr(sl(opac_act)), L.ptr(b["scales"][n0:n1]), L.ptr(b["opacities"][n0:n1]), L.stream()),
                        "gs_activation_chain")
                if ctx.smooth_grads is not None:
                    for name, g in zip(("kd", "ks", "normals"), ctx.smooth_grads):
                        b[name][n0:n1].add_(g[n0:n1])
                ev_c = torch.cuda.Event(); ev_c.record(pstream)
            self.bucket.all_reduce_rows(names, n0, n1, after=ev_c)
        if not ctx.captured:
            for tv in views:
                for t in tv[:6]:
                    t.record_stream(tail); t.record_stream(pstream)
            for t in (scales_act, opac_act, g_scales_act, g_opac_act):
                t.record_stream(tail); t.record_stream(pstream)
        return pstream

    def _capture(self, n_pinned: int, record):
        dev = self.p.means.device
        F.reserve_pinned(n_pinned)
        if self._status is None:
            self._status = torch.zeros(4, dtype=torch.int64, device=dev)
        if self._status_host is None:
            self._status_host = torch.zeros(4, dtype=torch.int64).pin_memory()
        warm = torch.cuda.Stream(device=dev)
        warm.wait_stream(torch.cuda.current_stream(dev))
        with torch.cuda.stream(warm):
            record(lambda own_pool=False: contextlib.nullcontext())
        torch.cuda.current_stream(dev).wait_stream(warm)
        torch.cuda.synchronize(dev)
        self.poll_capacity(_internal=True)
        graphs = []

        def phase(own_pool: bool = False):
            graphs.append(torch.cuda.CUDAGraph())
            return torch.cuda.graph(graphs[-1], pool=graphs[0].pool() if (len(graphs) > 1 and not own_pool) else None)
        out = record(phase)
        counts = [hc for hc, _ in self._seen_counts]
        self._seen_counts = []
        self._status_event = None
        cap = self._i_cap
        status_host = self._status_host

        def check() -> bool:
            torch.cuda.synchronize(dev)
            worst = max([int(hc[1]) for hc in counts] + [0])
            truncated, key32, need_i = F.status_overflow(status_host)
            overflow = truncated or worst > cap
            if overflow:
                check.stale = True
                self.truncated_steps += 1
                self._key32 = self._key32 or key32
                self._exact_max_i = max(self._exact_max_i, worst, need_i)
                self._status.zero_(); status_host.zero_()
            return not overflow
        check.stale = False
        return out, graphs, check

    def capture(self, cameras: List[Camera], upstream: Callable[[int, Tensor], Tensor], keep_images: bool = False,
                smoothing: Optional[Smoothing] = None):
        if smoothing is not None:
            raise NotImplementedError("the smoothing regularisers run on the eager fused step (__call__), not in a captured graph")
        if not (self.fused and self.mode == "pbr"):
            raise RuntimeError("capture() needs the fused path")
        if self._i_cap is None:
            raise RuntimeError("capture() needs a known capacity: run one eager step and poll_capacity(wait=True) first")

        def record(phase):
            with phase():
                return self._step(cameras, upstream, False, keep_images)
        out, (graph,), check = self._capture(2 * len(cameras) + 2, record)

        def replay():
            if check.stale:
                raise RuntimeError("this captured step overflowed its capacity / key range (check() returned False): capture() again")
            graph.replay()
            return out
        replay.check = check
        replay.graph = graph
        return replay

    def capture_views(self, cameras: List[Camera], upstream: Callable[[int, Tensor], Tensor], all_reduce: bool = True,
                      keep_images: bool = False, smoothing: Optional[Smoothing] = None):
        if smoothing is not None:
            raise NotImplementedError("the smoothing regularisers run on the eager fused step (__call__), not in a captured graph")
        if not (self.fused and self.mode == "pbr" and self.prefilter):
            raise RuntimeError("capture_views() needs the fused path with the prefilter in the step")
        if self._i_cap is None:
            raise RuntimeError("capture_views() needs a known capacity: run one eager step and poll_capacity(wait=True) first")
        dev = self.p.means.device
        world, sharded = self._sharding(all_reduce)
        first = self._pyramid(sharded, world)
        pyramid = TextureSplitSum(first.base.detach().clone(), [l.detach().clone() for l in first.levels], first.min_roughness,
                                  first.max_roughness)
        slots = [pyramid.base] + list(pyramid.levels)
        two = os.environ.get("GEOSPLAT_GEO_GRAPH", "1") != "0"
        act = (torch.empty_like(self.p.scales.detach()), torch.empty_like(self.p.opacities.detach().squeeze(-1)))
        self._activations(act)

        def record(phase):
            geo = recs = None
            if two:
                with phase():
                    geo = self._geometry(cameras, bin_first=True, act=act)
                    for sd in self._side_stream:
                        torch.cuda.current_stream(dev).wait_stream(sd)
                with phase(own_pool=True):
                    recs = self._records(cameras, geo, pyramid)
            with phase():
                if geo is None:
                    geo = self._geometry(cameras, bin_first=False, act=act)
                ctx = self._views(cameras, upstream, all_reduce, keep_images, geo, env=pyramid, recs=recs)
                if ctx.pstream is not None:
                    ctx.main.wait_stream(ctx.pstream)
                    ctx.pstream = None
            return ctx
        ctx, graphs, check = self._capture(6 * len(cameras) + 2, record)
        geo_graph, rec_graph, graph = graphs if two else (None, None, graphs[0])
        geo_stream = L.shared_stream(dev, "geo") if two else None
        ctx.main = None
        ctx.captured = True

        def step():
            if check.stale:
                raise RuntimeError("these captured views overflowed their capacity / key range (check() returned False): capture_views() again")
            cur = torch.cuda.current_stream(dev)
# ... 162 lines not shown
```

geosplatting_amd/front.py:

```python
from __future__ import annotations

import ctypes as C
import os
from typing import Optional

import torch
from torch import Tensor

from . import _lib as L

_pinned_pool4 = []


def pinned_counts4() -> Tensor:
    return _pinned_pool4.pop() if _pinned_pool4 else torch.empty(4, dtype=torch.int64).pin_memory()


def release_counts4(t: Tensor) -> None:
    _pinned_pool4.append(t)


def reserve_pinned(n: int) -> None:
    while len(_pinned_pool4) < n:
        _pinned_pool4.append(torch.empty(4, dtype=torch.int64).pin_memory())


class Front:
    __slots__ = ("vis", "keys", "rects", "tile_counts", "packed_index", "counts", "host_counts", "event", "whs", "key_bits", "N")


def front_stage(means: Tensor, quats: Tensor, scales: Tensor, opacities: Tensor, normals: Tensor, kd: Tensor, ks: Tensor,
                viewmat: Tensor, K: Tensor, cam_pos: Tensor, env_struct, W: int, H: int, min_roughness: float, max_metallic: float,
                mode: int, key_base: int = 0, key_bits: int = 32, status: Optional[Tensor] = None, tile_size: int = 16,
                eps2d: float = 0.3, near: float = 0.01, far: float = 1e10, radius_clip: float = 0.0, want_packed_index: bool = False,
                records: bool = True, binning: bool = True, tight_tiles: bool = False) -> Front:
    lib = L.lib()
    dev = means.device
    N = means.shape[0]
    fr = Front()
    fr.vis = torch.empty(max(N, 1), 16, dtype=torch.float32, device=dev) if records else None
    fr.keys = torch.empty(max(N, 1), dtype=torch.int32, device=dev) if binning else None
    fr.rects = torch.empty(max(N, 1), 2, dtype=torch.int32, device=dev) if binning else None
    fr.counts = torch.empty(4, dtype=torch.int64, device=dev)
    tw, th = (W + tile_size - 1) // tile_size, (H + tile_size - 1) // tile_size
    fr.tile_counts = torch.empty(tw * th, dtype=torch.int32, device=dev) if (binning and tw * th <= 8192) else None
    fr.packed_index = torch.empty(max(N, 1), dtype=torch.int32, device=dev) if want_packed_index else None
    ws_bytes = lib.gs_front_ws_bytes(N)
    ws = torch.empty(ws_bytes, dtype=torch.uint8, device=dev)
    L.check(lib.gs_front_fwd(N, L.ptr(means), L.ptr(quats), L.ptr(scales), L.ptr(opacities), L.ptr(normals), L.ptr(kd), L.ptr(ks),
                             L.ptr(viewmat), L.ptr(K), L.ptr(cam_pos), L.f32(min_roughness), L.f32(max_metallic), mode,
                             C.byref(env_struct) if env_struct is not None else None, W, H, tile_size, L.f32(eps2d), L.f32(near), L.f32(far), L.f32(radius_clip),
                             C.c_uint32(int(key_base) & 0xffffffff), int(key_bits), L.ptr(fr.vis), L.ptr(fr.keys), L.ptr(fr.rects),
                             L.ptr(fr.tile_counts), L.ptr(fr.packed_index), 1 if tight_tiles else 0, L.ptr(fr.counts), L.ptr(status), L.ptr(ws), C.c_size_t(ws_bytes), L.stream()), "gs_front_fwd")
    fr.host_counts = pinned_counts4()
    fr.host_counts.copy_(fr.counts, non_blocking=True)
    fr.event = torch.cuda.Event()
    fr.event.record()
    fr.whs = (W, H, tile_size)
    fr.key_bits = int(key_bits)
    fr.N = N
    return fr


def depth_range(host_counts: Tensor):
    if int(host_counts[0]) <= 0:
        return None
    return 0xffffffff - int(host_counts[2]), int(host_counts[3])


def learn_depth_range(lo: Optional[int], hi: Optional[int], host_counts: Tensor):
    rng = depth_range(host_counts)
    if rng is None:
        return lo, hi
    return (rng[0] if lo is None else min(lo, rng[0])), (rng[1] if hi is None else max(hi, rng[1]))


def binning_keys(lo: Optional[int], hi: Optional[int]):
    if lo is None:
        return 32, 0
    base = max(0, lo - (1 << 22))
    if hi - base < (1 << 24) - (1 << 21):
        return 24, base
    return 32, 0


def bin_stage(fr: Front, i_cap: Optional[int], status: Optional[Tensor], prepare: bool = True, binned=None):
    lib = L.lib()
    W, H, tile_size = fr.whs
    dev = fr.counts.device
    tw, th = (W + tile_size - 1) // tile_size, (H + tile_size - 1) // tile_size
    st = L.stream()
    if i_cap is None:
        fr.event.synchronize()
        V, I = int(fr.host_counts[0]), int(fr.host_counts[1])
        if V < 0 or I < 0 or I >= 2 ** 31:
            raise L.GeoSplatHipError(f"bad intersection count V={V} I={I}")
        counts = None
    else:
        V, I, counts = fr.N, int(i_cap), fr.counts
    if binned is not None:
        flat, offsets = binned
    else:
        flat = torch.empty(max(I, 1), dtype=torch.int32, device=dev)
        offsets = torch.empty(th * tw, dtype=torch.int32, device=dev)
        bin_bytes = lib.gs_isect_bin_front_ws_bytes(V, L.i64(I), tw, th)
        bin_ws = torch.empty(max(bin_bytes, 1), dtype=torch.uint8, device=dev)
        L.check(lib.gs_isect_bin_front(V, L.ptr(fr.keys), L.ptr(fr.rects), L.ptr(fr.tile_counts), L.ptr(counts), L.i64(I), fr.key_bits, tw, th,
                                       L.ptr(flat), L.ptr(offsets), L.ptr(bin_ws), C.c_size_t(bin_bytes),
                                       L.ptr(status) if counts is not None else None, st), "gs_isect_bin_front")
    if not prepare:
        return dict(flatten_ids=flat, isect_offsets=offsets, counts=counts, keys=fr.keys, rects=fr.rects, tile_counts=fr.tile_counts), V, I
    rws_bytes = lib.gs_raster_ws_bytes(L.i64(I), V, W, H, tile_size)
    rws = torch.empty(rws_bytes, dtype=torch.uint8, device=dev)
    if counts is None:
        L.check(lib.gs_raster_prepare_vis(W, H, tile_size, 3, V, L.ptr(fr.vis), L.i64(I), L.ptr(offsets), L.ptr(flat), L.ptr(rws),
                                          C.c_size_t(rws_bytes), st), "gs_raster_prepare_vis")
    else:
        L.check(lib.gs_raster_prepare_vis_cap(W, H, tile_size, 3, V, L.ptr(fr.vis), L.i64(I), L.ptr(counts), L.ptr(offsets), L.ptr(flat),
                                              L.ptr(rws), C.c_size_t(rws_bytes), st), "gs_raster_prepare_vis_cap")
    state = dict(vis_records=fr.vis, flatten_ids=flat, isect_offsets=offsets, raster_ws=rws, counts=counts, keys=fr.keys, rects=fr.rects,
                 tile_counts=fr.tile_counts, packed_index=fr.packed_index)
    return state, V, I


def tail_stage(V: int, counts: Optional[Tensor], means: Tensor, quats: Tensor, scales: Tensor, opacities: Tensor, normals: Tensor,
               kd: Tensor, ks: Tensor, viewmat: Tensor, K: Tensor, cam_pos: Tensor, env_struct, env_grad_struct, W: int, H: int,
               min_roughness: float, max_metallic: float, mode: int, vis: Tensor, v_packed: Tensor, g_means: Tensor, g_quats: Tensor,
               g_scales: Tensor, g_opacities: Tensor, g_normals: Tensor, g_kd: Tensor, g_ks: Tensor, eps2d: float = 0.3,
               priv: Optional[Tensor] = None) -> None:
    lib = L.lib()
    L.check(lib.gs_tail_bwd(V, L.ptr(counts), L.ptr(means), L.ptr(quats), L.ptr(scales), L.ptr(opacities), L.ptr(normals), L.ptr(kd),
                            L.ptr(ks), L.ptr(viewmat), L.ptr(K), L.ptr(cam_pos), L.f32(min_roughness), L.f32(max_metallic), mode,
                            C.byref(env_struct), W, H, L.f32(eps2d), L.ptr(vis), L.ptr(v_packed), int(v_packed.shape[1]),
                            L.ptr(g_means), L.ptr(g_quats), L.ptr(g_scales), L.ptr(g_opacities), L.ptr(g_normals), L.ptr(g_kd),
                            L.ptr(g_ks), C.byref(env_grad_struct), L.ptr(priv), C.c_size_t(0 if priv is None else priv.numel()),
                            L.stream()), "gs_tail_bwd")


def tail_priv_alloc(env_struct, mode: int, device) -> Optional[Tensor]:
    n = L.lib().gs_tail_priv_ws_bytes(C.byref(env_struct), mode)
    return torch.zeros(n, dtype=torch.uint8, device=device) if n > 0 else None


def tail_priv_reduce(env_struct, env_grad_struct, mode: int, priv: Optional[Tensor]) -> None:
    if priv is not None:
        L.check(L.lib().gs_tail_priv_reduce(C.byref(env_struct), mode, L.ptr(priv), C.c_size_t(priv.numel()), C.byref(env_grad_struct),
                                            L.stream()), "gs_tail_priv_reduce")


def tail_multi_stage(views, means: Tensor, quats: Tensor, scales: Tensor, opacities: Tensor, normals: Tensor, kd: Tensor, ks: Tensor,
                     env_struct, env_grad_struct, min_roughness: float, max_metallic: float, mode: int, g_means: Tensor, g_quats: Tensor,
                     g_scales: Tensor, g_opacities: Tensor, g_normals: Tensor, g_kd: Tensor, g_ks: Tensor, accumulate: bool,
                     eps2d: float = 0.3, priv: Optional[Tensor] = None, parts: int = 3) -> None:
    lib = L.lib()
    arr = (L.GsTailView * len(views))()
    stride = None
    for i, (vm, K, cp, vis, vp, pidx, W, H) in enumerate(views):
        arr[i].viewmat = vm.data_ptr(); arr[i].K = K.data_ptr(); arr[i].cam_pos = cp.data_ptr()
        arr[i].vis_records = vis.data_ptr(); arr[i].v_packed = vp.data_ptr(); arr[i].packed_index = pidx.data_ptr()
        arr[i].W = int(W); arr[i].H = int(H)
        assert stride in (None, int(vp.shape[1]))
        stride = int(vp.shape[1])
    L.check(lib.gs_tail_bwd_multi_parts(int(parts), means.shape[0], len(views), arr, L.ptr(means), L.ptr(quats), L.ptr(scales), L.ptr(opacities), L.ptr(normals),
                                  L.ptr(kd), L.ptr(ks), L.f32(min_roughness), L.f32(max_metallic), mode, C.byref(env_struct), L.f32(eps2d),
                                  stride, L.ptr(g_means), L.ptr(g_quats), L.ptr(g_scales), L.ptr(g_opacities), L.ptr(g_normals), L.ptr(g_kd),
                                  L.ptr(g_ks), 1 if accumulate else 0, C.byref(env_grad_struct), L.ptr(priv),
                                  C.c_size_t(0 if priv is None else priv.numel()), L.stream()), "gs_tail_bwd_multi_parts")


def front_streams(dev: torch.device):
    return [L.shared_stream(dev, "front0"), L.shared_stream(dev, "front1")]


class CameraCache:
    MAX_ENTRIES = 4096

    def __init__(self, dev: torch.device):
        self.dev = dev
        self.entries = {}

    def get(self, cam, stream: torch.cuda.Stream):
        c2w = cam.c2w
        intr = (float(cam.fx), float(cam.fy), float(cam.cx), float(cam.cy), int(cam.width), int(cam.height))
        host = c2w.device.type == "cpu"
        fp = c2w.detach().numpy().tobytes() if host else None
        key = (c2w.data_ptr(), tuple(c2w.shape), tuple(c2w.stride()), intr)
        hit = self.entries.get(key)
        if hit is not None and hit[1] == c2w._version and hit[3] == fp:
            return hit[2]
        if len(self.entries) >= self.MAX_ENTRIES:
            self.entries.pop(next(iter(self.entries)))
        caller = torch.cuda.current_stream(self.dev)
        if not host and stream != caller:
            stream.wait_stream(caller)
        with torch.cuda.stream(stream):
            tensors = (cam.view_matrix.to(self.dev, torch.float32).contiguous(),
                       cam.intrinsic_matrix.to(self.dev, torch.float32).contiguous(),
                       c2w.detach()[:, 3].to(self.dev, torch.float32).contiguous())
            ev = torch.cuda.Event(); ev.record(stream)
        for f in front_streams(self.dev):
            if f != stream:
                f.wait_event(ev)
        self.entries[key] = (c2w, c2w._version, tensors, fp)
        return tensors

    def clear(self) -> None:
        self.entries.clear()


def texel_grads(env, flat: Optional[Tensor] = None):
    sizes = [env.base.numel()] + [l.numel() for l in env.levels]
    if flat is None or flat.numel() != sum(sizes):
        flat = torch.zeros(sum(sizes), dtype=torch.float32, device=env.base.device)
    parts = torch.split(flat, sizes)
    g_base = parts[0].view_as(env.base)
    g_levels = [q.view_as(l) for q, l in zip(parts[1:], env.levels)]
    eg = L.GsEnvGrad(); eg.base = g_base.data_ptr()
    for i, g in enumerate(g_levels):
        eg.levels[i] = g.data_ptr()
    return flat, g_base, g_levels, eg


def log_ws(I: int, W: int, H: int, dev: torch.device) -> Tensor:
    return torch.empty(L.lib().gs_raster_log_ws_bytes(L.i64(I), W, H, 16), dtype=torch.uint8, device=dev)


def composite_fwd(state, V: int, I: int, W: int, H: int, tone: int, exposure: Tensor, log: Tensor):
    dev = state["isect_offsets"].device
    f32 = torch.float32
    render = torch.empty(H, W, 3, dtype=f32, device=dev); alphas = torch.empty(H, W, dtype=f32, device=dev)
    last_ids = torch.empty(H, W, dtype=torch.int32, device=dev); img = torch.empty(H, W, 4, dtype=f32, device=dev)
    rws = state["raster_ws"]
    L.check(L.lib().gs_raster_composite_tone_log(W, H, 16, V, None, L.i64(I), L.ptr(state["counts"]), L.ptr(state["isect_offsets"]),
                                                 L.ptr(render), L.ptr(alphas), L.ptr(last_ids), tone, L.ptr(exposure), L.ptr(img),
                                                 L.ptr(rws), C.c_size_t(rws.numel()), L.ptr(log), C.c_size_t(log.numel()), L.stream()),
            "gs_raster_composite_tone_log")
    return img, render, alphas, last_ids


def composite_bwd(state, V: int, I: int, W: int, H: int, tone: int, exposure: Tensor, render: Tensor, alphas: Tensor,
                  last_ids: Tensor, log: Tensor, v_img: Tensor, g_exp: Tensor) -> None:
    rws = state["raster_ws"]
    L.check(L.lib().gs_raster_bwd_tone_log_acc(W, H, 16, V, None, L.i64(I), L.ptr(state["counts"]), L.ptr(state["isect_offsets"]),
                                               L.ptr(render), L.ptr(alphas), L.ptr(last_ids), tone, L.ptr(exposure), L.ptr(v_img),
                                               L.ptr(state["v_packed"]), L.ptr(g_exp), L.ptr(rws), C.c_size_t(rws.numel()), L.ptr(log),
                                               C.c_size_t(log.numel()), L.stream()), "gs_raster_bwd_tone_log_acc")


def smooth_view(state, V: int, I: int, W: int, H: int, kd: Tensor, ks: Tensor, normals: Tensor, bg9: Tensor, gt: Optional[Tensor],
                kinds, weights, loss: Tensor, zero_alphas: Tensor, g_kd: Tensor, g_ks: Tensor, g_normals: Tensor) -> Tensor:
    lib = L.lib()
    dev = kd.device
    st = L.stream()
    counts, vis, offsets, rws = state["counts"], state["vis_records"], state["isect_offsets"], state["raster_ws"]
    cols = torch.empty(max(V, 1), 9, dtype=torch.float32, device=dev)
    L.check(lib.gs_smooth_gather(V, L.ptr(counts), L.ptr(vis), L.ptr(kd), L.ptr(ks), L.ptr(normals), L.ptr(cols), st), "gs_smooth_gather")
    render = torch.empty(H, W, 9, dtype=torch.float32, device=dev)
    alphas = torch.empty(H, W, dtype=torch.float32, device=dev)
    last_ids = torch.empty(H, W, dtype=torch.int32, device=dev)
    if counts is None:
        L.check(lib.gs_raster_composite(W, H, 16, 9, V, L.ptr(cols), L.ptr(bg9), L.i64(I), L.ptr(offsets), L.ptr(render), L.ptr(alphas),
                                        L.ptr(last_ids), L.ptr(rws), C.c_size_t(rws.numel()), st), "gs_raster_composite")
    else:
        L.check(lib.gs_raster_composite_cap(W, H, 16, 9, V, L.ptr(cols), L.ptr(bg9), L.i64(I), L.ptr(counts), L.ptr(offsets), L.ptr(render),
                                            L.ptr(alphas), L.ptr(last_ids), L.ptr(rws), C.c_size_t(rws.numel()), st), "gs_raster_composite_cap")
    from .loss import smooth_loss_and_grad
    _, v_img = smooth_loss_and_grad(render, gt, kinds, weights, out=loss)
    v9 = state["v_packed9"]
    if counts is None:
        L.check(lib.gs_raster_bwd_acc(W, H, 16, 9, V, L.ptr(cols), L.ptr(bg9), L.i64(I), L.ptr(offsets), L.ptr(alphas), L.ptr(last_ids),
                                      L.ptr(v_img), L.ptr(zero_alphas), L.ptr(v9), L.ptr(rws), C.c_size_t(rws.numel()), st), "gs_raster_bwd_acc")
    else:
# ... 43 lines not shown
```

geosplatting_amd/parallel.py:

```python
from __future__ import annotations

from typing import Dict, List, Optional, Sequence

import torch
import torch.distributed as dist
from torch import Tensor


def collectives_active() -> bool:
    import os
    if not (dist.is_available() and dist.is_initialized()):
        return False
    return dist.get_world_size() > 1 or os.environ.get("GEOSPLAT_COLLECTIVES_AT_WORLD1") == "1"


def shard_views(num_views: int, rank: int, world_size: int) -> List[int]:
    return list(range(rank, num_views, world_size))


class GradBucket:

    def __init__(self, shapes: Dict[str, Sequence[int]], device: torch.device, comm_stream=None):
        self.names = list(shapes.keys())
        self.shapes = {k: tuple(v) for k, v in shapes.items()}
        self.offsets: Dict[str, int] = {}
        off = 0
        for k in self.names:
            self.offsets[k] = off
            n = 1
            for s in self.shapes[k]:
                n *= int(s)
            off += (n + 63) // 64 * 64
        self.numel = off
        self.storage = torch.zeros(off, dtype=torch.float32, device=device)
        self.flat = self.storage[:off]
        if device.type == "cuda":
            from ._lib import shared_stream
            self.comm_stream = comm_stream if comm_stream is not None else shared_stream(device, "comm")
        else:
            self.comm_stream = None

    def zero_with_scratch(self, sizes: Sequence[int]) -> List[Tensor]:
        offs, off = [], self.numel
        for n in sizes:
            offs.append(off)
            off += (int(n) + 63) // 64 * 64
        if self.storage.numel() < off:
            self.storage = torch.zeros(off, dtype=torch.float32, device=self.storage.device)
            self.flat = self.storage[:self.numel]
        else:
            self.storage[:off].zero_()
        return [self.storage[o:o + int(n)] for o, n in zip(offs, sizes)]

    def view(self, name: str) -> Tensor:
        o = self.offsets[name]
        n = 1
        for s in self.shapes[name]:
            n *= int(s)
        return self.flat[o:o + n].view(self.shapes[name])

    def pack(self, grads: Dict[str, Optional[Tensor]]) -> None:
        dst, src = [], []
        for k in self.names:
            g = grads.get(k)
            if g is None:
                self.view(k).zero_()
            else:
                dst.append(self.view(k)); src.append(g.reshape(self.shapes[k]).to(torch.float32))
        if dst:
            torch._foreach_copy_(dst, src)

    def all_reduce(self, average: bool = False, async_op: bool = False):
        if not collectives_active():
            return (lambda: None) if async_op else None
        if self.comm_stream is not None and async_op:
            self.comm_stream.wait_stream(torch.cuda.current_stream())
            with torch.cuda.stream(self.comm_stream):
                dist.all_reduce(self.flat, op=dist.ReduceOp.SUM)
                if average:
                    self.flat.div_(dist.get_world_size())

            def wait():
                torch.cuda.current_stream().wait_stream(self.comm_stream)
            return wait
        dist.all_reduce(self.flat, op=dist.ReduceOp.SUM)
        if average:
            self.flat.div_(dist.get_world_size())
        return (lambda: None) if async_op else None

    def all_reduce_split(self, first_of_tail: str):
        cut = self.offsets[first_of_tail]
        head, tail = self.flat[:cut], self.flat[cut:]
        if not collectives_active():
            return (lambda: None), (lambda: None)
        cs = self.comm_stream

        def start_head():
            if cs is not None:
                cs.wait_stream(torch.cuda.current_stream())
                with torch.cuda.stream(cs):
                    dist.all_reduce(head, op=dist.ReduceOp.SUM)
            else:
                dist.all_reduce(head, op=dist.ReduceOp.SUM)

        def finish():
            if cs is not None:
                cs.wait_stream(torch.cuda.current_stream())
                with torch.cuda.stream(cs):
                    dist.all_reduce(tail, op=dist.ReduceOp.SUM)
                torch.cuda.current_stream().wait_stream(cs)
            else:
                dist.all_reduce(tail, op=dist.ReduceOp.SUM)
        return start_head, finish

    def all_reduce_rows(self, names: Sequence[str], n0: int, n1: int, after=None) -> None:
        if not collectives_active():
            return
        views = [self.view(k)[n0:n1] for k in names]
        cs = self.comm_stream
        if cs is None:
            for v in views:
                dist.all_reduce(v, op=dist.ReduceOp.SUM)
            return
        if after is not None:
            cs.wait_event(after)
        else:
            cs.wait_stream(torch.cuda.current_stream())
        with torch.cuda.stream(cs):
            _all_reduce_coalesced(views)

    def join_comm(self) -> None:
        if self.comm_stream is not None and collectives_active():
            torch.cuda.current_stream().wait_stream(self.comm_stream)

    def all_reduce_names(self, names: Sequence[str], group=None) -> None:
        if not collectives_active():
            return
        cs = self.comm_stream
        if cs is not None:
            cs.wait_stream(torch.cuda.current_stream())
            with torch.cuda.stream(cs):
                for k in names:
                    dist.all_reduce(self.view(k), op=dist.ReduceOp.SUM, group=group)
            torch.cuda.current_stream().wait_stream(cs)
        else:
            for k in names:
                dist.all_reduce(self.view(k), op=dist.ReduceOp.SUM, group=group)

    def unpack(self) -> Dict[str, Tensor]:
        return {k: self.view(k) for k in self.names}


def _all_reduce_coalesced(tensors: Sequence[Tensor]) -> None:
    mgr = getattr(dist, "_coalescing_manager", None)
    if mgr is not None and tensors[0].is_cuda and dist.get_backend() == "nccl":
        try:
            with mgr(device=tensors[0].device):
                for t in tensors:
                    dist.all_reduce(t, op=dist.ReduceOp.SUM)
            return
        except TypeError:
            pass
    for t in tensors:
        dist.all_reduce(t, op=dist.ReduceOp.SUM)


def init_distributed_from_env(device_type: str = "cuda"):
    import os
    world = int(os.environ.get("WORLD_SIZE", "1"))
    rank = int(os.environ.get("RANK", "0"))
    local = int(os.environ.get("LOCAL_RANK", "0"))
    backend = "nccl" if device_type == "cuda" else "gloo"
    if device_type == "cuda":
        if os.environ.get("GEOSPLAT_DEBUG_SHARE_GPU") == "1":
            local, backend = 0, "gloo"
        torch.cuda.set_device(local)
        device = torch.device("cuda", local)
    else:
        device = torch.device("cpu")
    if (world > 1 or os.environ.get("GEOSPLAT_COLLECTIVES_AT_WORLD1") == "1") and not dist.is_initialized():
        os.environ.setdefault("MASTER_ADDR", "127.0.0.1")
        os.environ.setdefault("MASTER_PORT", "29500")
        dist.init_process_group(backend, rank=rank, world_size=world)
    return rank, world, device
```

geosplatting_amd/viewbatch.py:

```python
from __future__ import annotations

import collections
import os
import threading
import warnings
from typing import Dict, List, Optional, Tuple

import torch
from torch import Tensor

from . import _lib as L
from . import front as F
from .cameras import Camera
from .splitsum import TextureSplitSum


class GeoSplatCapacityError(L.GeoSplatHipError):
    """A view had more tile intersections (or a depth range wider) than the capacity it was launched with: its image and gradients
    are those of a truncated list.  The capacity has been raised; repeat the step."""


class _DeviceState:
    def __init__(self, dev: torch.device):
        self.dev = dev
# ... 89 lines not shown
            z = lambda *s: torch.empty(*s, dtype=torch.float32, device=dev)
            g_flat, g_base, g_levels, eg = F.texel_grads(self.env)
            self.g = dict(means=z(N, 3), quats=z(N, 4), scales_act=z(N, 3), opac_act=z(N), normals=z(N, 3), kd=z(N, 3), ks=z(N, 2),
                          g_flat=g_flat, base=g_base, levels=g_levels, eg=eg)
            self.n_tail = 0
            self.sched = F.tail_schedule([2])
            ev = torch.cuda.Event(); ev.record()
            self.st.tail.wait_event(ev)
            for f in self.st.fronts:
                f.wait_event(ev)
        return self.g

    def discard_pass(self) -> None:
        if self.g is None:
            return
        main = torch.cuda.current_stream(self.st.dev)
        main.wait_stream(self.st.tail)
        for f in self.st.fronts:
            main.wait_stream(f)
        for v in self.pending:
            v.state = v.render = v.alphas = v.last_ids = v.log_ws = None
        self.g, self.pending, self.n_tail = None, [], 0

    def end_of_backward(self) -> None:
        if self.g is not None:
            self.discard_pass()

    def launch_tail(self, final: bool) -> None:
        views, self.pending = self.pending, []
        if not views:
            return
        st, t, g = self.st, self.t, self.g
        mr, mm, mode = self.cfg
        tv = [(v.cam[0], v.cam[1], v.cam[2], v.state["vis_records"], v.state["v_packed"], v.state["packed_index"], v.W, v.H) for v in views]
        args = (t["means"], t["quats"], self.scales_act, self.opac_act, t["normals"], t["kd"], t["ks"], self.e, g["eg"], mr, mm, mode,
                g["means"], g["quats"], g["scales_act"], g["opac_act"], g["normals"], g["kd"], g["ks"])
        used = F.tail_batch(tv, args, self.n_tail > 0, final, st.tail, st.fronts[0])
        self.n_tail += 1
        for v in views:
            v.state = v.render = v.alphas = v.last_ids = v.log_ws = None
        for name in ("means", "quats", "scales_act", "opac_act", "normals", "kd", "ks", "g_flat"):
            for s in used:
                g[name].record_stream(s)


def _capacity_error(v: "_View") -> GeoSplatCapacityError:
    return GeoSplatCapacityError(
        f"splat(): view {v.index} of a step had {v.i_seen} tile intersections (capacity {v.cap_used}) or left the 24-bit depth-key "
        f"range: its image and gradients come from a truncated list.  The capacity is now {v.cap.i_cap(v.N)}; repeat the step "
        "(viewbatch.retry_on_capacity does; GEOSPLAT_CAPACITY=0 reads the exact counts back for every view instead).")


def _poll_unchecked(st: _DeviceState, wait_views=None) -> None:
    with st.lock:
        keep = collections.deque()
        while st.unchecked:
            v = st.unchecked.popleft()
            if wait_views is not None and any(v is w for w in wait_views):
                v.event.synchronize()
            if not v.event.query():
                keep.append(v)
                continue
            hc = v.host_counts
            v.i_seen = int(hc[1])
            cap = v.cap
            over = v.i_seen > v.cap_used
            if v.key_bits == 24:
                rng = F.depth_range(hc)
                if rng is not None and (rng[0] < v.key_base or rng[1] >= v.key_base + (1 << 24)):
                    over = True
                    cap.key32 = True
            hs = v.host_status
            if hs is not None:
                truncated, key32, _ = F.status_overflow(hs)
                over = over or truncated
                cap.key32 = cap.key32 or key32
                F.release_counts4(hs)
                v.host_status = None
            cap.learn(hc, v.N)
            F.release_counts4(hc)
            v.host_counts = None
            v.status = None
            v.over = over
        st.unchecked = keep


def _warn_unreported(step: "_Step") -> None:
    for v in step.views:
        if v.over and not v.reported:
            v.reported = True
            warnings.warn(str(_capacity_error(v)), RuntimeWarning)


def _view_forward(step: _Step, cam: Camera, exposure: Tensor, tone: int, want_grad: bool) -> Tuple[Tensor, _View]:
    st, t = step.st, step.t
    dev = st.dev
    mr, mm, mode = step.cfg
    W, H = int(cam.width), int(cam.height)
    N = t["means"].shape[0]
    main = torch.cuda.current_stream(dev)
    side = st.fronts[st.n_views % len(st.fronts)]
    st.n_views += 1
    _poll_unchecked(st)
    with st.lock:
        cap = st.caps.get((W, H))
        if cap is None:
            cap = st.caps[(W, H)] = _Capacity()
            while len(st.caps) > _MAX_CAPS:
                st.caps.popitem(last=False)
        else:
            st.caps.move_to_end((W, H))
        if cap.first_step is None and want_grad:
            cap.first_step = step.key
    exact = (not want_grad) or (not _use_capacity()) or cap.ratio is None or cap.first_step == step.key
    i_cap = None if exact else cap.i_cap(N)
    key_bits, key_base = (32, 0) if exact else cap.keys()
    status = None
    if not exact:
        with torch.cuda.stream(side):
            status = torch.zeros(4, dtype=torch.int64, device=dev)
    tight = os.environ.get("GEOSPLAT_TIGHT_TILES", "1") != "0"
    side.wait_event(step.ready)
    cam_t = st.cameras.get(cam, side)
    v = _View()
    v.cam, v.W, v.H, v.tone, v.exact, v.cap, v.done, v.index = cam_t, W, H, tone, exact, cap, (False if want_grad else None), len(step.views)
    v.N, v.status, v.over, v.i_seen, v.reported = N, status, False, 0, False
    with torch.cuda.stream(side):
        fr = F.front_stage(t["means"], t["quats"], step.scales_act, step.opac_act, t["normals"], t["kd"], t["ks"], cam_t[0], cam_t[1],
                           cam_t[2], step.e, W, H, mr, mm, mode, key_base, key_bits, status,
                           want_packed_index=want_grad, tight_tiles=tight)
        state, V, I = F.bin_stage(fr, i_cap, status, prepare=False)
        v_packed = torch.zeros(max(V, 1), L.lib().gs_raster_grad_stride(3), dtype=torch.float32, device=dev) if want_grad else None
        log_ws = F.log_ws(I, W, H, dev)
        v.host_status = None
        if not exact:
            v.host_status = F.pinned_counts4()
            v.host_status.copy_(status, non_blocking=True)
        ev = torch.cuda.Event(); ev.record(side)
    if exact:
        cap.learn(fr.host_counts, N)
        F.release_counts4(fr.host_counts)
        v.host_counts = None
    else:
        v.host_counts, v.event, v.cap_used, v.key_bits, v.key_base = fr.host_counts, ev, i_cap, key_bits, key_base
        with st.lock:
            st.unchecked.append(v)
    for x in list(state.values()) + [log_ws, v_packed, step.scales_act, step.opac_act] + list(cam_t):
        if isinstance(x, Tensor):
            x.record_stream(main)
    main.wait_event(ev)
    for x in (fr.vis, fr.counts, fr.packed_index):
        if x is not None:
            x.record_stream(main)
    state, V, I = F.bin_stage(fr, i_cap, status, binned=(state["flatten_ids"], state["isect_offsets"]))
    if v_packed is not None:
        state["v_packed"] = v_packed
    img, render, alphas, last_ids = F.composite_fwd(state, V, I, W, H, tone, exposure, log_ws)
    v.V, v.I, v.state, v.render, v.alphas, v.last_ids, v.log_ws, v.exposure = V, I, state, render, alphas, last_ids, log_ws, exposure
    return img, v


def _view_backward(step: _Step, v: _View, v_img: Tensor) -> Tensor:
    if v.state is None:
        raise L.GeoSplatHipError("splat(): backward through a view a second time (its buffers were released after the first; "
                                 "render the view again instead of retain_graph)")
    v_img = v_img.contiguous().float()
    g_exp = torch.zeros(1, dtype=torch.float32, device=step.st.dev)
    gather = step.has_gather
    if gather:
        if step.g is None:
            torch.autograd.Variable._execution_engine.queue_callback(step.end_of_backward)
        step.grads()
    try:
        return _view_backward_launch(step, v, v_img, g_exp, gather)
    except BaseException:
        step.discard_pass()
        raise


def _view_backward_launch(step: _Step, v: _View, v_img: Tensor, g_exp: Tensor, gather: bool) -> Tensor:
    F.composite_bwd(v.state, v.V, v.I, v.W, v.H, v.tone, v.exposure, v.render, v.alphas, v.last_ids, v.log_ws, v_img, g_exp)
    v.done = True
    if not gather:
        v.state = v.render = v.alphas = v.last_ids = v.log_ws = None
        return g_exp
    step.pending.append(v)
    k = step.sched[min(step.n_tail, len(step.sched) - 1)]
    remaining = sum(1 for w in step.views if not w.done)
    if len(step.pending) >= k and remaining > 0:
        step.launch_tail(final=False)
    return g_exp


_PARAMS = ("means", "scales", "quats", "opacities", "normals", "kd", "ks")


class _Gather(torch.autograd.Function):

    @staticmethod
    def forward(ctx, step: _Step, *tensors: Tensor):
        ctx.step = step
        ctx.shapes = [tuple(x.shape) for x in tensors]
        ctx.set_materialize_grads(False)
        return tuple(x.detach() for x in tensors)

    @staticmethod
    def backward(ctx, *unused):
        step: _Step = ctx.step
        st = step.st
        if step.g is None:
            return (None,) * (1 + len(ctx.shapes))
        step.launch_tail(final=True)
        g, step.g = step.g, None
        main = torch.cuda.current_stream(st.dev)
        done = [v for v in step.views if v.done]
        tail_stream = st.fronts[0]
        tail_stream.wait_stream(st.tail)
        with torch.cuda.stream(tail_stream):
            g_scales = g["scales_act"] * step.scales_act
            g_opac = (g["opac_act"] * step.opac_act * (1.0 - step.opac_act)).reshape(ctx.shapes[3])
        main.wait_stream(st.tail)
        main.wait_stream(tail_stream)
        for x in (g_scales, g_opac):
            x.record_stream(main)
        for x in (g["scales_act"], g["opac_act"], step.scales_act, step.opac_act):
            x.record_stream(tail_stream)
        _poll_unchecked(st, wait_views=[v for v in done if v.host_counts is not None])
        bad = [v for v in done if v.over and not v.reported]
        if bad:
            for v in bad:
                v.reported = True
            raise _capacity_error(bad[0])
        out = [g["means"], g_scales, g["quats"], g_opac, g["normals"], g["kd"], g["ks"], g["base"]] + list(g["levels"])
        return (None, *[x.reshape(s) for x, s in zip(out, ctx.shapes)])


class _SplatView(torch.autograd.Function):
    @staticmethod
    def forward(ctx, step: _Step, cam: Camera, tone: int, exposure: Tensor, *gathered: Tensor):
        exposure_d = exposure.detach().reshape(1).contiguous().float()
        img, view = _view_forward(step, cam, exposure_d, tone, True)
        step.views.append(view)
        ctx.step, ctx.view, ctx.n, ctx.exp_shape = step, view, len(gathered), tuple(exposure.shape)
        ctx.set_materialize_grads(False)
        return img

    @staticmethod
    def backward(ctx, v_img):
        none = (None,) * (4 + ctx.n)
        if v_img is None:
            return none
        g_exp = _view_backward(ctx.step, ctx.view, v_img)
        return (None, None, None, g_exp.reshape(ctx.exp_shape)) + (None,) * ctx.n


def splat_view(means: Tensor, scales: Tensor, quats: Tensor, opacities: Tensor, normals: Tensor, kd: Tensor, ks: Tensor, camera: Camera,
               exposure: Tensor, envmap: TextureSplitSum, lut: Tensor, min_roughness: float, max_metallic: float, mode: int,
               tone: int) -> Tensor:
    raw = dict(zip(_PARAMS, (means, scales, quats, opacities, normals, kd, ks)))
    L.require_cuda(*raw.values())
    st = _state(means.device)
    srcs = list(raw.values()) + [envmap.base] + list(envmap.levels)
    cfg = (float(min_roughness), float(max_metallic), int(mode))
    key = (tuple((id(x), x._version, x.data_ptr()) for x in srcs), cfg, id(lut), float(envmap.min_roughness), float(envmap.max_roughness),
           torch.is_grad_enabled() and any(x.requires_grad for x in srcs))
    exposure = torch.as_tensor(exposure, dtype=torch.float32, device=st.dev)
    params_grad = key[-1]
    want_grad = torch.is_grad_enabled() and (params_grad or exposure.requires_grad)
    step = st.current
    if step is None or step.key != key:
        conv = [x if (x.dtype == torch.float32 and x.is_contiguous()) else x.float().contiguous() for x in srcs]
        det = dict(zip(_PARAMS, (x.detach() for x in conv[:7])))
        env_d = TextureSplitSum(conv[7].detach(), [x.detach() for x in conv[8:]], envmap.min_roughness, envmap.max_roughness)
        if step is not None:
            _warn_unreported(step)
            step.gathered = None
            step.srcs = None
        step = _Step(st, key, det, env_d, lut, cfg)
        step.srcs = srcs
        step.has_gather = params_grad
        step.gathered = _Gather.apply(step, *conv) if params_grad else None
        st.current = step
    if not want_grad:
        img, _ = _view_forward(step, camera, exposure.detach().reshape(1).contiguous(), tone, False)
        return img
    return _SplatView.apply(step, camera, tone, exposure, *(step.gathered or ()))


def reset() -> None:
    for st in _states.values():
        with st.lock:
            if st.current is not None:
                st.current.gathered = None
            st.current = None
            st.caps.clear()


def retry_on_capacity(step_fn, max_retries: int = 2):
    def wrapped(*a, **k):
        for attempt in range(max_retries + 1):
            try:
                return step_fn(*a, **k)
            except GeoSplatCapacityError:
                if attempt == max_retries:
                    raise
    return wrapped
```

include/geosplat_hip.h:

```cpp
#ifndef GEOSPLAT_HIP_H
#define GEOSPLAT_HIP_H

#include <stddef.h>
#include <stdint.h>

#ifdef __cplusplus
extern "C" {
#endif

#define GS_OK            0
#define GS_EINVAL       -1
#define GS_ENOSPC       -2
#define GS_ELAUNCH      -3

#define GS_MAX_LEVELS   16
#define GS_MAX_CHANNELS 32

#define GS_MODE_PBR      0
#define GS_MODE_DIFFUSE  1
#define GS_MODE_SPECULAR 2
#define GS_TONE_NONE     0
#define GS_TONE_NAIVE    1
#define GS_TONE_ACES     2

// ... 134 lines not shown

int gs_project_bwd(int N, int V, int D, const float* means, const float* quats, const float* scales,
                   const float* opacities, const float* viewmat, const float* K, int W, int H, float eps2d,
                   const int32_t* gaussian_ids, const float* conics, const float* compensations,
                   const float* v_packed, int rec_stride , const float* v_depths,
                   float* v_means, float* v_quats, float* v_scales, float* v_opacities, float* v_colors,
                   int accumulate, void* stream);

int gs_project_bwd_ex(int N, int V, int D, const float* means, const float* quats, const float* scales,
                      const float* opacities, const float* viewmat, const float* K, int W, int H, float eps2d,
                      const int32_t* gaussian_ids, const float* conics, const float* compensations,
                      const float* v_packed, int rec_stride, const float* v_depths, const float* sh_coeffs, int sh_K,
                      int sh_degree, int flags, float* v_means, float* v_quats, float* v_scales, float* v_opacities,
                      float* v_colors, float* g_sh_coeffs, int accumulate, void* stream);

typedef struct GsEnv {
    const float* lut;
    int          lut_res;
    const float* base;
    int          base_res;
    int          num_levels;
    const float* levels[GS_MAX_LEVELS];
    int          res[GS_MAX_LEVELS];
    float        min_roughness;
    float        max_roughness;
} GsEnv;

typedef struct GsEnvGrad {
    float* base;
    float* levels[GS_MAX_LEVELS];
} GsEnvGrad;

int gs_shade_fwd(int N, const float* means, const float* normals, const float* kd, const float* ks,
                 const float* cam_pos, float min_roughness, float max_metallic, int mode,
                 const GsEnv* env , float* colors, void* stream);

size_t gs_shade_bwd_ws_bytes(const GsEnv* env , int mode);
int gs_shade_bwd_plan_blocks(const GsEnv* env , int mode, int N, int* block_threads);

int gs_shade_bwd(int N, const float* means, const float* normals, const float* kd, const float* ks,
                 const float* cam_pos, float min_roughness, float max_metallic, int mode,
                 const GsEnv* env , const float* v_colors,
                 float* v_means, float* v_normals, float* v_kd, float* v_ks,
                 const GsEnvGrad* env_grad , int accumulate, void* ws, size_t ws_bytes, void* stream);

int gs_tonemap_fwd(int64_t P, int mode, const float* rgba, const float* exposure, float* out, void* stream);
int gs_tonemap_fwd3(int64_t P, int mode, const float* render, const float* alphas, const float* exposure, float* out, void* stream);
int gs_tonemap_bwd3(int64_t P, int mode, const float* render, const float* alphas, const float* exposure, const float* v_out,
                    float* v_render, float* v_alphas, float* v_exposure, int accumulate, void* stream);
int gs_tonemap_bwd(int64_t P, int mode, const float* rgba, const float* exposure, const float* v_out,
                   float* v_rgba, float* v_exposure, int accumulate, void* stream);

int gs_cubemap_mip_fwd(int R, int C, const float* in, float* out, void* stream);
int gs_cubemap_mip_chain_fwd(int R, int n_levels, const float* in, float* const* outs, void* stream);
int gs_cube_sample_linear(int64_t n, const float* tex, int R, const float* dirs, float scale, float* out,
                          void* stream);
int gs_cubemap_mip_bwd(int R, const float* v_out, float* v_in, int accumulate, void* stream);
int gs_diffuse_cubemap_fwd(int R, const float* cubemap, float* out, void* stream);
int gs_diffuse_cubemap_bwd(int R, const float* v_out, float* v_cubemap, int accumulate, void* stream);
int gs_specular_bounds(int R, float costheta_cutoff, float* bounds, void* stream);
size_t gs_specular_bounds_ws_bytes(int R);
int gs_specular_bounds_fast(int R, float costheta_cutoff, const float* dir_table, float* bounds, void* ws, size_t ws_bytes, void* stream);
int gs_cube_dir_table(int R, float* table, void* stream);
int gs_specular_cubemap_fwd(int R, const float* cubemap, const float* bounds, const float* dir_table,
                            float roughness, float costheta_cutoff, float* out, void* stream);
int gs_specular_cubemap_bwd(int R, const float* bounds, const float* dir_table, const float* v_out_rgb,
                            float roughness, float costheta_cutoff, float* v_cubemap, int accumulate, void* stream);

int gs_specular_tiles_count(int R, float roughness, float costheta_cutoff, int backward, int margin, int bw, int nb, const float* bounds,
                            const float* dir_table, const int32_t* tiles, int n_tiles, int32_t* row_counts, int32_t* extents,
                            uint64_t* pairs, void* stream);
int gs_specular_tiles_fill(int R, float roughness, float costheta_cutoff, int backward, int margin, int bw, int nb, const float* bounds,
                           const float* dir_table, const int32_t* tiles, int n_tiles, const int64_t* row_begin,
                           const int32_t* segments, int32_t* desc, float* weights, void* stream);
int gs_specular_tiles_check(int R, const float* bounds, const float* dir_table, uint64_t* out2, void* stream);
int gs_specular_tiles_apply(int R, int backward, int n_mirrors, int margin, int bw, int nb, const float* src, const float* scale,
                            const float* out_scale, const float* bounds, const int32_t* tiles, const int32_t* segments,
                            const int64_t* row_begin, const int32_t* row_counts, const int32_t* desc, const float* weights, float* dst,
                            int tile_begin, int tile_end, size_t lds_bytes, void* stream);

typedef struct GsTileLevel {
    int R, n_mirrors, margin, bw, nb, tile_begin, tile_end, reserved;
    const float* src; const float* scale; const float* out_scale; const float* bounds;
    const int32_t* tiles; const int32_t* segments; const int64_t* row_begin; const int32_t* row_counts; const int32_t* desc;
    const float* weights; float* dst; size_t lds_bytes;
} GsTileLevel;
int gs_specular_tiles_apply_multi(int n_levels, const GsTileLevel* levels, int backward, void* stream);

int gs_mgadapter_fwd(int F, const float* vertices, const int64_t* faces, const float* vnormals,
                     float* means, float* scales, float* quats, float* normals, void* stream);
int gs_mgadapter_bwd(int F, int V, const float* vertices, const int64_t* faces, const float* vnormals,
                     const float* v_means, const float* v_scales, const float* v_quats, const float* v_normals,
                     float* v_vertices, float* v_vnormals, void* stream);

int gs_vertex_normals_fwd(int F, int V, const float* vertices, const int64_t* faces, float* raw, float* vnormals,
                          void* stream);
int gs_vertex_normals_bwd(int F, int V, const float* vertices, const int64_t* faces, const float* raw,
                          const float* v_vnormals, float* v_raw, float* v_vertices, int accumulate, void* stream);

size_t gs_photo_loss_ws_bytes(int W, int H);
int gs_photo_loss(int W, int H, const float* rgb, const float* alpha, const float* gt_rgba, int gt_is_srgb,
                  const float* train_bg, const float* metric_bg, float ssim_lambda, float mask_weight,
                  float grad_scale, float* out, float* v_rgb, float* v_alpha, void* ws, size_t ws_bytes, void* stream);

size_t gs_smooth_loss_ws_bytes(int W, int H);
int gs_smooth_loss(int W, int H, const float* img, const float* gt_rgb, const int* kinds, const float* weights, float* out,
                   float* v_img, void* ws, size_t ws_bytes, void* stream);

int gs_hashgrid_fwd(int N, int L, int F, int log2_T, const float* scalings_host, const float* x, const float* table,
                    float* out, void* stream);
size_t gs_hashgrid_bwd_ws_bytes(int N, int L, int F);
int gs_hashgrid_bwd(int N, int L, int F, int log2_T, const float* scalings_host, const float* x, const float* table,
                    const float* v_out, float table_grad_scale, float* v_table, int accumulate, float* v_x,
                    void* ws ,
                    size_t ws_bytes, void* stream);

size_t gs_hashgrid_bwd_fixed_ws_bytes(int N, int L, int F, int log2_T);
int gs_hashgrid_bwd_fixed(int N, int L, int F, int log2_T, const float* scalings_host, const float* x, const float* table,
                          const float* v_out, float table_grad_scale, float* v_table, int accumulate, float* v_x, void* ws,
                          size_t ws_bytes, void* stream);

size_t gs_mlp_wgrad_ws_bytes(int64_t N);
int gs_mlp_wgrad(int64_t N, int O, int I, const float* dY, const float* X, float scale, float* dW, int accumulate,
                 void* ws, size_t ws_bytes, void* stream);

size_t gs_flexicubes_ws_bytes(int R0, int R1, int R2);
int gs_flexicubes_count(int R0, int R1, int R2, const float* sdf, void* ws, size_t ws_bytes, int64_t* counts, void* stream);
int gs_flexicubes_fwd(int R0, int R1, int R2, const float* vertices, const float* sdf, const float* alpha,
                      const float* beta, const float* gamma, float weight_scale, float sdf_eps, const void* ws,
                      size_t ws_bytes, int64_t Q, int64_t num_quads, int64_t K, float* out_vertices, int64_t* out_faces,
                      float* L_dev, void* stream);
int gs_flexicubes_bwd(int R0, int R1, int R2, const float* vertices, const float* sdf, const float* alpha,
                      const float* beta, const float* gamma, float weight_scale, float sdf_eps, const void* ws,
                      size_t ws_bytes, int64_t Q, int64_t num_quads, int64_t K, const float* out_vertices,
                      const float* v_out_vertices, const float* v_L_dev, float* g_vd_scratch, float* g_vertices,
                      float* g_sdf, float* g_alpha, float* g_beta, float* g_gamma, void* stream);
int gs_flexicubes_entropy_fwd(int R0, int R1, int R2, const float* sdf, void* ws, size_t ws_bytes, float* out, void* stream);
int gs_flexicubes_entropy_bwd(int R0, int R1, int R2, const float* sdf, const void* ws, size_t ws_bytes, const float* v_out,
                              float* g_sdf, int accumulate, void* stream);

size_t gs_front_ws_bytes(int N);
int gs_front_fwd(int N, const float* means, const float* quats, const float* scales, const float* opacities,
                 const float* normals, const float* kd, const float* ks, const float* viewmat, const float* K,
                 const float* cam_pos, float min_roughness, float max_metallic, int mode, const GsEnv* env,
                 int W, int H, int tile_size, float eps2d, float near_plane, float far_plane, float radius_clip,
                 uint32_t key_base, int key_bits, float* vis_records, uint32_t* depth_keys, uint32_t* tile_rects,
                 uint32_t* tile_counts, int32_t* packed_index ,
                 int tight_tiles, int64_t* counts4, int64_t* status4, void* ws, size_t ws_bytes, void* stream);
size_t gs_isect_bin_front_ws_bytes(int V, int64_t n_isects, int tile_w, int tile_h);
int gs_isect_bin_front_classes(int* caps, int max);
int gs_isect_bin_front(int V_cap, const uint32_t* depth_keys, const uint32_t* tile_rects, const uint32_t* tile_counts,
                       const int64_t* counts_dev, int64_t n_isects_cap, int key_bits, int tile_w, int tile_h, int32_t* flatten_ids_sorted,
                       int32_t* isect_offsets, void* ws, size_t ws_bytes, int64_t* status_dev, void* stream);
int gs_tail_bwd(int V_cap, const int64_t* counts_dev, const float* means, const float* quats, const float* scales,
                const float* opacities, const float* normals, const float* kd, const float* ks, const float* viewmat,
                const float* K, const float* cam_pos, float min_roughness, float max_metallic, int mode, const GsEnv* env,
                int W, int H, float eps2d, const float* vis_records, const float* v_packed, int rec_stride,
                float* v_means, float* v_quats, float* v_scales, float* v_opacities, float* v_normals, float* v_kd, float* v_ks,
                const GsEnvGrad* env_grad, void* priv_ws, size_t priv_ws_bytes, void* stream);
typedef struct GsTailView {
    const float* viewmat; const float* K; const float* cam_pos;
    const float* vis_records; const float* v_packed; const int32_t* packed_index;
    int W, H;
} GsTailView;
int gs_tail_bwd_multi(int N, int n_views, const GsTailView* views , const float* means, const float* quats,
                      const float* scales, const float* opacities, const float* normals, const float* kd, const float* ks,
                      float min_roughness, float max_metallic, int mode, const GsEnv* env, float eps2d, int rec_stride,
                      float* v_means, float* v_quats, float* v_scales, float* v_opacities, float* v_normals, float* v_kd, float* v_ks,
                      int accumulate, const GsEnvGrad* env_grad, void* priv_ws, size_t priv_ws_bytes, void* stream);
int gs_tail_bwd_multi_parts(int parts, int N, int n_views, const GsTailView* views , const float* means, const float* quats,
                            const float* scales, const float* opacities, const float* normals, const float* kd, const float* ks,
                            float min_roughness, float max_metallic, int mode, const GsEnv* env, float eps2d, int rec_stride,
                            float* v_means, float* v_quats, float* v_scales, float* v_opacities, float* v_normals, float* v_kd, float* v_ks,
                            int accumulate, const GsEnvGrad* env_grad, void* priv_ws, size_t priv_ws_bytes, void* stream);
size_t gs_tail_priv_ws_bytes(const GsEnv* env , int mode);
int gs_tail_priv_reduce(const GsEnv* env , int mode, const void* priv_ws, size_t priv_ws_bytes, const GsEnvGrad* env_grad,
                        void* stream);

int gs_smooth_gather(int V_cap, const int64_t* counts_dev, const float* vis_records, const float* kd, const float* ks,
                     const float* normals, float* cols, void* stream);
int gs_smooth_fold(int V_cap, const int64_t* counts_dev, const float* vis_records, const float* v_packed9, int stride9, float* v_packed,
                   int stride, float* v_kd, float* v_ks, float* v_normals, void* stream);

int gs_activation_chain(int64_t N, const float* g_scales_act, const float* scales_act, const float* g_opac_act, const float* opac_act,
                        float* v_scales, float* v_opacities, void* stream);

#define GS_DENSIFY_COPY         0
#define GS_DENSIFY_MEANS        1
#define GS_DENSIFY_SCALES       2
#define GS_DENSIFY_MOMENT       3
#define GS_DENSIFY_MODE_DENSIFY 0
#define GS_DENSIFY_MODE_CULL    1
#define GS_DENSIFY_MAX_TENSORS  32
#define GS_DENSIFY_MAX_SPLITS   8
#define GS_DENSIFY_MAX_N        (((int64_t)1) << 27)

typedef struct GsDensifyTensor {
    const float* src;
    float*       dst;
    int          floats_per_row;
    int          kind;
} GsDensifyTensor;

int gs_densify_stats(int V, const int64_t* gaussian_ids, const float* v_means2d, int64_t N, float* xys_grad_norm, float* vis_counts,
                     void* stream);
size_t gs_densify_ws_bytes(int64_t N, int num_splits);
int gs_densify_plan(int64_t N, const float* scales, const float* opacities, const float* xys_grad_norm, const float* vis_counts,
                    float half_extent, float grad_thresh, float size_thresh, float alpha_thresh, float scale_thresh, int num_splits,
                    int mode, void* ws, size_t ws_bytes, int64_t* totals, void* stream);
int gs_densify_fill(int64_t N, int num_splits, void* ws, size_t ws_bytes, int64_t n_selected, int64_t n_split, int64_t n_dup,
                    const GsDensifyTensor* table , int n_tensors, const float* quats, const float* scales, const float* randn,
                    int64_t* indices, void* stream);

size_t gs_surfel_project_ws_bytes(int N);
int gs_surfel_project_fwd(int N, const float* means, const float* quats, const float* scales, const float* opacities,
                          const float* colors, int Dc, const float* sh_coeffs, int sh_K, int sh_degree, int depth_channel,
                          const float* viewmat, const float* K, int W, int H, int tile_size, float near_plane, float far_plane,
                          float radius_clip, int32_t* gaussian_ids, int32_t* radii, float* means2d, float* depths,
                          float* ray_transforms, float* normals, float* opacities_packed, float* colors_packed,
                          int32_t* tiles_per_gauss, void* ws, size_t ws_bytes, int64_t* counts, void* stream);

int gs_surfel_project_bwd(int N, int V, int Dc, const float* means, const float* quats, const float* scales,
                          const float* sh_coeffs, int sh_K, int sh_degree, const float* viewmat, const float* K,
                          const int32_t* gaussian_ids, const float* v_ray_transforms, const float* v_means2d,
                          const float* v_depths, const float* v_normals, const float* v_opacities, const float* v_colors,
                          int stride, float* g_means, float* g_quats, float* g_scales, float* g_opacities, float* g_colors,
                          float* g_sh, void* stream);

int gs_surfel_raster_fwd(int W, int H, int tile_size, int C, int depth_channel, int distloss, int V, const float* ray_transforms,
                         const float* means2d, const float* opacities, const float* colors, const float* normals,
                         const float* background, int64_t n_isects, const int32_t* offsets, const int32_t* flatten_ids,
                         float* render, float* alphas, float* render_normals, float* render_distort, float* render_median,
                         int32_t* last_ids, float* final_T, float* final_D, void* stream);

int gs_surfel_grad_stride(void);

int gs_surfel_raster_bwd(int W, int H, int tile_size, int C, int depth_channel, int distloss, int V, const float* ray_transforms,
                         const float* means2d, const float* opacities, const float* colors, const float* normals,
                         const float* depths, const float* background, int64_t n_isects, const int32_t* offsets,
                         const int32_t* flatten_ids, const int32_t* last_ids, const float* final_T, const float* final_D,
                         const float* v_render, const float* v_alphas, const float* v_normals, const float* v_distort,
                         float* v_packed, float* v_densify, void* stream);

#define GS_TSDF_MAX_VIEWS 16
typedef struct GsTsdfView {
    const float* depth_alpha;
    const float* viewmat; const float* K;
    int W, H;
} GsTsdfView;
int gs_tsdf_integrate(int R0, int R1, int R2, float origin_x, float origin_y, float origin_z, float voxel_size, float sdf_trunc,
                      float alpha_trunc, float depth_trunc, int n_views, const GsTsdfView* views , float* volume,
                      void* stream);
size_t gs_tsdf_extract_ws_bytes(int R0, int R1, int R2);
int gs_tsdf_extract_count(int R0, int R1, int R2, const float* volume, void* ws, size_t ws_bytes, int64_t* counts, void* stream);
int gs_tsdf_extract_fill(int R0, int R1, int R2, float origin_x, float origin_y, float origin_z, float voxel_size, const float* volume,
                         void* ws, size_t ws_bytes, int64_t n_vertices, int64_t n_triangles, float* vertices, int64_t* faces,
                         void* stream);

size_t gs_meshraster_ws_bytes(int64_t F, int H, int W);
int gs_meshraster_fwd(int64_t V, int64_t F, const float* vc, const int32_t* faces, float fx, float fy, float cx, float cy, int H, int W,
                      float near, int cull, void* ws, size_t ws_bytes, uint64_t* stats, void* stream);
int gs_meshraster_resolve(int64_t V, int64_t F, const float* vc, const int32_t* faces, float fx, float fy, float cx, float cy, int H,
                          int W, float near, const void* ws, size_t ws_bytes, float* rast, void* stream);
int gs_meshraster_bwd(int64_t V, int64_t F, const float* vc, const int32_t* faces, float fx, float fy, float cx, float cy, int H, int W,
                      float near, const float* rast, const float* d_rast, float* d_vc, void* stream);
int gs_mesh_interp_fwd(int64_t P, int C, int64_t F, int64_t V, int per_face_vertex, const float* rast, const int32_t* faces,
                       const float* attr, float* out, void* stream);
int gs_mesh_interp_bwd(int64_t P, int C, int64_t F, int64_t V, int per_face_vertex, const float* rast, const int32_t* faces,
                       const float* attr, const float* d_out, float* d_attr, float* d_rast, void* stream);

size_t gs_mesh_topology_bytes(int64_t F);
int gs_mesh_topology_build(int64_t F, const int32_t* faces, void* topo, size_t topo_bytes, void* stream);
int gs_meshaa_fwd(int64_t V, int64_t F, const float* vc, const int32_t* faces, float fx, float fy, float cx, float cy, int H, int W,
                  float near, int cull, const void* topo, size_t topo_bytes, int C, const float* rast, const float* color, float* out,
                  int32_t* dbg, void* stream);
int gs_meshaa_bwd(int64_t V, int64_t F, const float* vc, const int32_t* faces, float fx, float fy, float cx, float cy, int H, int W,
                  float near, int cull, const void* topo, size_t topo_bytes, int C, const float* rast, const float* color,
                  const float* d_out, float* d_color, float* d_vc, void* stream);

#define GS_TEX_WRAP      0
#define GS_TEX_CLAMP     1
#define GS_OCC_TEXTURE   0
#define GS_OCC_NONE      1
int gs_tex2d_fwd(int64_t P, int Ht, int Wt, int C, int boundary, const float* tex, const float* uv, float* out, void* stream);
int gs_tex2d_bwd(int64_t P, int Ht, int Wt, int C, int boundary, const float* tex, const float* uv, const float* d_out,
                 float* d_uv, float* d_tex, void* stream);
int gs_meshshade_fwd(int H, int W, const float* rast, const float* position, const float* normal, const float* uv,
                     int kd_h, int kd_w, const float* kd, int ks_h, int ks_w, const float* ks, const float* cam_pos,
                     const GsEnv* env , int occlusion, float min_visibility, int bend_back_normal, float* color, void* stream);
int gs_meshshade_bwd(int H, int W, const float* rast, const float* position, const float* normal, const float* uv,
                     int kd_h, int kd_w, const float* kd, int ks_h, int ks_w, const float* ks, const float* cam_pos,
                     const GsEnv* env , int occlusion, float min_visibility, int bend_back_normal, const float* d_color,
                     float* d_position, float* d_normal, float* d_uv, float* d_kd, float* d_ks, const GsEnvGrad* env_grad ,
                     void* stream);

size_t gs_bvh_bytes(int64_t F);
size_t gs_bvh_ws_bytes(int64_t F);
int gs_bvh_build(int64_t V, int64_t F, const float* vertices, const int32_t* faces, void* bvh, size_t bvh_bytes, void* ws,
                 size_t ws_bytes, void* stream);
int gs_ray_occluded(int64_t V, int64_t F, const float* vertices, const int32_t* faces, const void* bvh ,
                    int64_t P, int S, const float* origins , const float* dirs, int dirs_per_point ,
                    float tmin, float tmax, uint8_t* out , void* stream);
int gs_ray_closest(int64_t V, int64_t F, const float* vertices, const int32_t* faces, const void* bvh ,
                   int64_t P, int S, const float* origins , const float* dirs, int dirs_per_point, float tmin, float tmax,
                   float* t , int32_t* face , float* bary , void* stream);

// ... 23 lines not shown
```

Before: 768.4.

## Build raster tile order inside binning scan and skip separate order kernel

Makes the tile-offsets scan kernel in the binning stage also write the raster tile processing order and zero the backward bucket counts directly into the raster workspace, so the single-block tile_order_kernel launch in raster prepare can be skipped. It also stops the pinned host copy of the counts when binning is not requested, and narrows the zeroing of the gradient bucket scratch so stored rows are not cleared. This removes a serial one-block kernel and some memset and copy work per view, but the order is now built with shared atomics within a class, which may differ from the previous ordering.

```diff
diff --git a/geosplatting_amd/_lib.py b/geosplatting_amd/_lib.py
--- a/geosplatting_amd/_lib.py
+++ b/geosplatting_amd/_lib.py
@@ -51,7 +51,7 @@
     "gs_specular_tiles_check", "gs_specular_tiles_apply", "gs_specular_tiles_apply_multi", "gs_mgadapter_fwd", "gs_mgadapter_bwd", "gs_vertex_normals_fwd",
     "gs_vertex_normals_bwd", "gs_photo_loss_ws_bytes", "gs_photo_loss", "gs_smooth_loss_ws_bytes", "gs_smooth_loss", "gs_hashgrid_fwd", "gs_hashgrid_bwd_ws_bytes", "gs_hashgrid_bwd", "gs_hashgrid_bwd_fixed_ws_bytes", "gs_hashgrid_bwd_fixed", "gs_mlp_wgrad_ws_bytes", "gs_mlp_wgrad",
     "gs_flexicubes_ws_bytes", "gs_flexicubes_count", "gs_flexicubes_fwd", "gs_flexicubes_bwd", "gs_flexicubes_entropy_fwd",
-    "gs_flexicubes_entropy_bwd", "gs_front_ws_bytes", "gs_front_fwd", "gs_isect_bin_front_ws_bytes", "gs_isect_bin_front", "gs_isect_bin_front_classes", "gs_tail_bwd", "gs_tail_bwd_multi", "gs_tail_bwd_multi_parts", "gs_tail_priv_ws_bytes", "gs_tail_priv_reduce", "gs_smooth_gather", "gs_smooth_fold", "gs_activation_chain",
+    "gs_flexicubes_entropy_bwd", "gs_front_ws_bytes", "gs_front_fwd", "gs_isect_bin_front_ws_bytes", "gs_isect_bin_front", "gs_isect_bin_front_classes", "gs_isect_bin_front_order", "gs_raster_ws_order", "gs_raster_prepare_vis_ordered", "gs_raster_prepare_vis_ordered_cap", "gs_tail_bwd", "gs_tail_bwd_multi", "gs_tail_bwd_multi_parts", "gs_tail_priv_ws_bytes", "gs_tail_priv_reduce", "gs_smooth_gather", "gs_smooth_fold", "gs_activation_chain",
     "gs_densify_stats", "gs_densify_ws_bytes", "gs_densify_plan", "gs_densify_fill",
     "gs_surfel_project_ws_bytes", "gs_surfel_project_fwd", "gs_surfel_project_bwd", "gs_surfel_raster_fwd", "gs_surfel_grad_stride",
     "gs_surfel_raster_bwd",
diff --git a/geosplatting_amd/csrc/gs_raster.hip b/geosplatting_amd/csrc/gs_raster.hip
--- a/geosplatting_amd/csrc/gs_raster.hip
+++ b/geosplatting_amd/csrc/gs_raster.hip
@@ -1453,7 +1453,7 @@
 static int raster_prepare_impl(int W, int H, int tile_size, int D, int V, const float* means2d, const float* conics,
                                const float* opacities, const float* colors, const float* vis_records, int64_t n_isects,
                                const int32_t* offsets, const int32_t* flatten_ids, void* ws, size_t ws_bytes, void* stream,
-                               const RasterOpts& o)
+                               const RasterOpts& o, bool ordered = false)
 {
     const int rc = raster_check("gs_raster_prepare", W, H, tile_size, D, V, n_isects, ws, ws_bytes);
     if (rc != GS_OK) return rc;
@@ -1472,6 +1472,7 @@
                            vis, r.rec0, r.rec1, r.rec2);
         GS_CHECK_LAUNCH();
     }
+    if (ordered) return GS_OK;
     hipLaunchKernelGGL(tile_order_kernel, dim3(1), dim3(1024), 0, s, tiles, isect_count(n_isects, o), offsets, r.order, r.bo);
     GS_CHECK_LAUNCH();
     return GS_OK;
@@ -1637,6 +1638,39 @@
                                flatten_ids, ws, ws_bytes, stream, o);
 }
 
+extern "C" int gs_raster_ws_order(void* ws, size_t ws_bytes, int64_t n_isects, int V, int W, int H, int tile_size, int32_t** order,
+                                  int32_t** bcount)
+{
+    GS_CHECK_ARG(order != nullptr && bcount != nullptr, "null argument");
+    const int rc = raster_check("gs_raster_ws_order", W, H, tile_size, 1, V, n_isects, ws, ws_bytes);
+    if (rc != GS_OK) return rc;
+    const int tiles = ((W + GS_TILE - 1) / GS_TILE) * ((H + GS_TILE - 1) / GS_TILE);
+    const RasterWs r = carve(ws, n_isects, V, tiles);
+    *order = r.order;
+    *bcount = r.bo.bcount;
+    return GS_OK;
+}
+
+extern "C" int gs_raster_prepare_vis_ordered(int W, int H, int tile_size, int D, int V, const float* vis_records, int64_t n_isects,
+                                             const int32_t* offsets, const int32_t* flatten_ids, void* ws, size_t ws_bytes, void* stream)
+{
+    GS_CHECK_ARG(vis_records != nullptr || V == 0, "vis_records (written by gs_project_fwd_vis) must not be NULL");
+    return raster_prepare_impl(W, H, tile_size, D, V, nullptr, nullptr, nullptr, nullptr, vis_records, n_isects, offsets,
+                               flatten_ids, ws, ws_bytes, stream, RasterOpts{}, true);
+}
+
+extern "C" int gs_raster_prepare_vis_ordered_cap(int W, int H, int tile_size, int D, int V_cap, const float* vis_records,
+                                                 int64_t n_isects_cap, const int64_t* counts_dev, const int32_t* offsets,
+                                                 const int32_t* flatten_ids, void* ws, size_t ws_bytes, void* stream)
+{
+    GS_CHECK_ARG(counts_dev != nullptr, "counts_dev must not be NULL");
+    GS_CHECK_ARG(vis_records != nullptr || V_cap == 0, "vis_records (written by gs_project_fwd_vis) must not be NULL");
+    RasterOpts o;
+    o.counts = counts_dev;
+    return raster_prepare_impl(W, H, tile_size, D, V_cap, nullptr, nullptr, nullptr, nullptr, vis_records, n_isects_cap, offsets,
+                               flatten_ids, ws, ws_bytes, stream, o, true);
+}
+
 extern "C" int gs_raster_composite_cap(int W, int H, int tile_size, int D, int V_cap, const float* colors, const float* background,
                                        int64_t n_isects_cap, const int64_t* counts_dev, const int32_t* offsets, float* render,
                                        float* alphas, int32_t* last_ids, const void* ws, size_t ws_bytes, void* stream)
diff --git a/geosplatting_amd/csrc/gs_sort.hip b/geosplatting_amd/csrc/gs_sort.hip
--- a/geosplatting_amd/csrc/gs_sort.hip
+++ b/geosplatting_amd/csrc/gs_sort.hip
@@ -494,6 +494,8 @@
     unsigned* count; int32_t* lists;
     unsigned* cursor;
     const long long* counts; long long v_cap, i_cap; long long* status;
+    int32_t* order;
+    int32_t* bcount;
 };
 
 __device__ __forceinline__ int seg_class(unsigned len) { return len <= SEG_CAP0 ? 0 : 1; }
@@ -509,9 +511,12 @@
 {
     __shared__ unsigned wsum[16];
     __shared__ unsigned s_bin[SEG_CLASSES * SEG_BINS];
+    __shared__ unsigned s_total[SEG_CLASSES + 1];
     const unsigned n = (unsigned)gs_count(nc);
     const int lane = threadIdx.x & 63, wave = threadIdx.x >> 6;
     if (sl.count && threadIdx.x < SEG_CLASSES * SEG_BINS) s_bin[threadIdx.x] = 0u;
+    if (sl.count && threadIdx.x == 0) s_total[SEG_CLASSES] = 0u;
+    if (sl.count && sl.bcount && threadIdx.x < 64) sl.bcount[threadIdx.x] = 0;
     if (sl.count && threadIdx.x == 0 && sl.counts != nullptr && sl.status != nullptr) {
         const long long V = sl.counts[0], I = sl.counts[1];
         if (V > sl.v_cap || I > sl.i_cap) {
@@ -546,9 +551,12 @@
         const unsigned v = s_bin[wave * SEG_BINS + lane];
         const unsigned incl = gs_wave_incl_scan(v);
         s_bin[wave * SEG_BINS + lane] = incl - v;
-        if (lane == 63) sl.count[wave] = incl;
-    }
-    __syncthreads();
+        if (lane == 63) { sl.count[wave] = incl; s_total[wave] = incl; }
+    }
+    __syncthreads();
+    unsigned obase[SEG_CLASSES];
+    unsigned oempty = 0u;
+    for (int c = SEG_CLASSES - 1; c >= 0; --c) { obase[c] = oempty; oempty += s_total[c]; }
     for (int i = threadIdx.x; i < n_tiles; i += 1024) {
         const unsigned beg = (unsigned)offsets[i];
         unsigned end = n;
@@ -557,6 +565,9 @@
             const int c = seg_class(end - beg);
             const unsigned pos = atomicAdd(&s_bin[c * SEG_BINS + seg_bin(end - beg)], 1u);
             sl.lists[(size_t)c * n_tiles + pos] = i;
+            if (sl.order) sl.order[obase[c] + pos] = i;
+        } else if (sl.order) {
+            sl.order[oempty + atomicAdd(&s_total[SEG_CLASSES], 1u)] = i;
         }
     }
 }
@@ -711,7 +722,7 @@
 
 static int bin_front_tile_first(int V, const uint32_t* depth_keys, const uint32_t* tile_rects, const uint32_t* tile_counts,
                                 const int64_t* counts_dev, int64_t n_isects, int key_bits, int tile_w, int tile_h, int32_t* flatten_ids_sorted,
-                                int32_t* isect_offsets, void* ws, int64_t* status_dev, hipStream_t s)
+                                int32_t* isect_offsets, void* ws, int64_t* status_dev, int32_t* order, int32_t* bcount, hipStream_t s)
 {
     const int n_tiles = tile_w * tile_h;
     const GsCount vc{ (long long)V, (const long long*)counts_dev }, ic{ (long long)n_isects, counts_dev ? (const long long*)counts_dev + 1 : nullptr };
@@ -721,7 +732,8 @@
     int32_t* lists = (int32_t*)p; p += align256((size_t)SEG_CLASSES * n_tiles * 4);
     u64* items = (u64*)p;
     hipLaunchKernelGGL(tile_offsets_scan_kernel, dim3(1), dim3(1024), 0, s, n_tiles, (const unsigned*)tile_counts, ic, isect_offsets,
-                       SegLists{ class_count, lists, cursor, (const long long*)counts_dev, (long long)V, (long long)n_isects, (long long*)status_dev });
+                       SegLists{ class_count, lists, cursor, (const long long*)counts_dev, (long long)V, (long long)n_isects, (long long*)status_dev,
+                                 order, bcount });
     GS_CHECK_LAUNCH();
     const bool f64 = key_bits == 24;
     hipLaunchKernelGGL(bin_scatter_kernel, dim3(gs_cdiv(V, SC_TILE)), dim3(SC_THREADS), (size_t)n_tiles * 4, s, vc,
@@ -749,9 +761,9 @@
     return GS_OK;
 }
 
-extern "C" int gs_isect_bin_front(int V_cap, const uint32_t* depth_keys, const uint32_t* tile_rects, const uint32_t* tile_counts,
-                                  const int64_t* counts_dev, int64_t n_isects_cap, int key_bits, int tile_w, int tile_h, int32_t* flatten_ids_sorted,
-                                  int32_t* isect_offsets, void* ws, size_t ws_bytes, int64_t* status_dev, void* stream)
+static int bin_front_impl(int V_cap, const uint32_t* depth_keys, const uint32_t* tile_rects, const uint32_t* tile_counts,
+                          const int64_t* counts_dev, int64_t n_isects_cap, int key_bits, int tile_w, int tile_h, int32_t* flatten_ids_sorted,
+                          int32_t* isect_offsets, void* ws, size_t ws_bytes, int64_t* status_dev, int32_t* tile_order, int32_t* bwd_bcount, void* stream)
 {
     const int V = V_cap;
     const int64_t n_isects = n_isects_cap;
@@ -761,12 +773,14 @@
     GS_CHECK_ARG(isect_offsets != nullptr && (counts_dev == nullptr || status_dev != nullptr), "null argument");
     hipStream_t s = (hipStream_t)stream;
     const int n_tiles = tile_w * tile_h;
+    GS_CHECK_ARG((tile_order == nullptr && bwd_bcount == nullptr) || (tile_order != nullptr && bwd_bcount != nullptr && tile_counts != nullptr &&
+                 n_tiles <= BF_HIST_MAX && V > 0 && n_isects > 0), "tile order: needs order and bcount, tile_counts, <= 8192 tiles and a non-empty view");
     if (V == 0 || n_isects == 0) { GS_CHECK_HIP(gs_zero_async(isect_offsets, sizeof(int32_t) * (size_t)n_tiles, s)); return GS_OK; }
     GS_CHECK_ARG(depth_keys != nullptr && tile_rects != nullptr && flatten_ids_sorted != nullptr && ws != nullptr, "null argument");
     if (tile_counts != nullptr && n_tiles <= BF_HIST_MAX) {
         if (ws_bytes < tf_ws_bytes(n_isects, n_tiles)) { gs_set_error("gs_isect_bin_front: workspace too small"); return GS_ENOSPC; }
         return bin_front_tile_first(V, depth_keys, tile_rects, tile_counts, counts_dev, n_isects, key_bits, tile_w, tile_h, flatten_ids_sorted,
-                                    isect_offsets, ws, status_dev, s);
+                                    isect_offsets, ws, status_dev, tile_order, bwd_bcount, s);
     }
     if (ws_bytes < bf_radix_ws_bytes((size_t)V, (size_t)n_isects)) { gs_set_error("gs_isect_bin_front: workspace too small for the radix path (no tile_counts)"); return GS_ENOSPC; }
     const GsCount vc{ (long long)V, (const long long*)counts_dev }, ic{ (long long)n_isects, counts_dev ? (const long long*)counts_dev + 1 : nullptr };
@@ -818,6 +832,24 @@
     hipLaunchKernelGGL(bin_offsets_tiles_kernel, dim3(gs_cdiv(n_isects, 256)), dim3(256), 0, s, ic, tile_ids, n_tiles, isect_offsets);
     GS_CHECK_LAUNCH();
     return GS_OK;
+}
+
+extern "C" int gs_isect_bin_front(int V_cap, const uint32_t* depth_keys, const uint32_t* tile_rects, const uint32_t* tile_counts,
+                                  const int64_t* counts_dev, int64_t n_isects_cap, int key_bits, int tile_w, int tile_h, int32_t* flatten_ids_sorted,
+                                  int32_t* isect_offsets, void* ws, size_t ws_bytes, int64_t* status_dev, void* stream)
+{
+    return bin_front_impl(V_cap, depth_keys, tile_rects, tile_counts, counts_dev, n_isects_cap, key_bits, tile_w, tile_h, flatten_ids_sorted,
+                          isect_offsets, ws, ws_bytes, status_dev, nullptr, nullptr, stream);
+}
+
+extern "C" int gs_isect_bin_front_order(int V_cap, const uint32_t* depth_keys, const uint32_t* tile_rects, const uint32_t* tile_counts,
+                                        const int64_t* counts_dev, int64_t n_isects_cap, int key_bits, int tile_w, int tile_h,
+                                        int32_t* flatten_ids_sorted, int32_t* isect_offsets, void* ws, size_t ws_bytes, int64_t* status_dev,
+                                        int32_t* order, int32_t* bcount, void* stream)
+{
+    GS_CHECK_ARG(order != nullptr && bcount != nullptr, "order and bcount must not be NULL");
+    return bin_front_impl(V_cap, depth_keys, tile_rects, tile_counts, counts_dev, n_isects_cap, key_bits, tile_w, tile_h, flatten_ids_sorted,
+                          isect_offsets, ws, ws_bytes, status_dev, order, bcount, stream);
 }
 
 static int isect_bin_impl(int V, const float* means2d, const int32_t* radii, const float* depths, int64_t n_isects,
diff --git a/geosplatting_amd/engine.py b/geosplatting_amd/engine.py
--- a/geosplatting_amd/engine.py
+++ b/geosplatting_amd/engine.py
@@ -60,7 +60,7 @@
     key_bits: int; key_base: int
     status: Optional[Tensor]
     tight: bool
-    early: Dict[int, Tuple[Tensor, Tensor]]
+    early: Dict[int, Tuple[Tensor, ...]]
 
 
 @dataclass
@@ -75,6 +75,18 @@
     tail_job: Optional[dict]
     smooth_grads: Optional[Tuple[Tensor, Tensor, Tensor]] = None
     captured: bool = False
+    snapshot: bool = False
+
+
+def step_stores_rows(prefilter: bool, n_views: int, N: int) -> bool:
+    return bool(prefilter) and n_views > 0 and N > 0
+
+
+def step_scratch(bucket: GradBucket, N: int, n_tex: int, sm_sizes: Sequence[int], stores_rows: bool):
+    assert bucket.names[-1] == "exposure"
+    sizes = [n_tex] + list(sm_sizes) + [3 * N, N]
+    sc = bucket.zero_with_scratch(sizes, zero_from="exposure", n_stored=2) if stores_rows else bucket.zero_with_scratch(sizes)
+    return sc[0], sc[1:-2], sc[-2], sc[-1]
 
 
 class RenderStep:
@@ -163,7 +175,7 @@
                 fr = self._front(geo, cameras[0], cam_t, None, records=False)
                 binned, _, _ = F.bin_stage(fr, i_cap, self._status, prepare=False)
             self._seen_counts.append((fr.host_counts, fr.event))
-            geo.early[0] = (binned["flatten_ids"], binned["isect_offsets"])
+            geo.early[0] = (binned["flatten_ids"], binned["isect_offsets"], binned["raster_ws"])
             for t in (scales_act, opac_act):
                 t.record_stream(side)
         return geo
@@ -173,7 +185,8 @@
         keys = (geo.key_base, geo.key_bits, geo.status) if binning else (0, 32, None)
         return F.front_stage(p.means.detach(), p.quats.detach(), geo.scales_act, geo.opac_act, p.normals.detach(), p.kd.detach(),
                              p.ks.detach(), *cam_t, e, cam.width, cam.height, self.min_roughness, self.max_metallic, _MODE[self.mode],
-                             *keys, want_packed_index=records, records=records, binning=binning, tight_tiles=geo.tight)
+                             *keys, want_packed_index=records, records=records, binning=binning, tight_tiles=geo.tight,
+                             copy_counts=binning)
 
     def _env_args(self, env: TextureSplitSum):
         env_d = TextureSplitSum(env.base.detach(), [l.detach().contiguous() for l in env.levels], env.min_roughness, env.max_roughness)
@@ -223,22 +236,23 @@
             tex_res.append(tex_res[-1] // 2)
         tex_sizes = [6 * tex_res[-1] * tex_res[-1] * 3] + [6 * r * r * 3 for r in tex_res]
         sm_sizes = [3 * N, 2 * N, 3 * N, 1, max([c.width * c.height for c in cameras] + [1])] if smoothing is not None else []
-        sc = self.bucket.zero_with_scratch([3 * N, N, sum(tex_sizes)] + sm_sizes)
+        g_tex, sm, g_scales_act, g_opac_act = step_scratch(self.bucket, N, sum(tex_sizes), sm_sizes,
+                                                           step_stores_rows(self.prefilter, len(cameras), N))
         b = self.bucket.unpack()
         smooth_grads = None
         self.last_smoothing_loss = self.last_attribute_renders = None
         if smoothing is not None:
-            smooth_grads = (sc[3].view(N, 3), sc[4].view(N, 2), sc[5].view(N, 3))
-            smooth_loss, zero_alphas = sc[6].view(()), sc[7]
+            smooth_grads = (sm[0].view(N, 3), sm[1].view(N, 2), sm[2].view(N, 3))
+            smooth_loss, zero_alphas = sm[3].view(()), sm[4]
             bg9 = smoothing.background.detach().to(dev, f32).reshape(3).repeat(3).contiguous()
             self.last_smoothing_loss = smooth_loss
             self.last_attribute_renders = [] if keep_images else None
-        g_scales_act = sc[0].view(N, 3); g_opac_act = sc[1]
+        g_scales_act = g_scales_act.view(N, 3)
         exposure = p.exposure.detach().reshape(1).contiguous()
         if env is None:
             env = self._pyramid(sharded, world)
         env_d, e = self._env_args(env)
-        g_flat, g_base, g_levels, eg = F.texel_grads(env_d, sc[2])
+        g_flat, g_base, g_levels, eg = F.texel_grads(env_d, g_tex)
         self.last_texel_grads = (g_base, g_levels)
         images = []
         tail = self._tail_stream
@@ -270,21 +284,22 @@
         def bin_view(item):
             fr, j, side = item
             with torch.cuda.stream(side):
-                if i_cap is not None:
+                if i_cap is not None and fr.host_counts is not None:
                     self._seen_counts.append((fr.host_counts, fr.event))
                 state, V, I = F.bin_stage(fr, i_cap, self._status, binned=early.get(j))
                 if i_cap is None:
                     self._exact_max_i = max(self._exact_max_i, I)
                     self._key_lo, self._key_hi = F.learn_depth_range(self._key_lo, self._key_hi, fr.host_counts)
                     F.release_counts4(fr.host_counts)
+                ev = torch.cuda.Event(); ev.record(side)
                 state["v_packed"] = torch.zeros(max(V, 1), lib.gs_raster_grad_stride(3), dtype=f32, device=dev)
                 if smoothing is not None:
                     state["v_packed9"] = torch.zeros(max(V, 1), lib.gs_raster_grad_stride(9), dtype=f32, device=dev)
-                ev = torch.cuda.Event(); ev.record(side)
+                ev_b = torch.cuda.Event(); ev_b.record(side)
             for t in state.values():
                 if isinstance(t, torch.Tensor):
                     t.record_stream(main)
-            return state, V, I, ev
+            return state, V, I, ev, ev_b
 
         n_views = len(cameras)
         proj = [start_view(cameras[j], j) for j in range(min(2, n_views))]
@@ -292,7 +307,7 @@
         for i, cam in enumerate(cameras):
             vm, K, cam_pos = cam_ts.pop(i)
             W, H = cam.width, cam.height
-            s, V, I, ev = binned
+            s, V, I, ev, ev_b = binned
             main.wait_event(ev)
             kev = self.kernel_events
             if kev is not None:
@@ -305,6 +320,7 @@
             v_img = upstream(i, img).contiguous()
             if kev is not None:
                 k2 = torch.cuda.Event(enable_timing=True); k2.record(main)
+            main.wait_event(ev_b)
             F.composite_bwd(s, V, I, W, H, tone, exposure, render, alphas, last_ids, log_ws, v_img, b["exposure"])
             if kev is not None:
                 k3 = torch.cuda.Event(enable_timing=True); k3.record(main)
@@ -339,6 +355,7 @@
             if pstream is not None:
                 pstream.wait_stream(main)
             smooth_grads = None
+        snapshot = False
         if i_cap is not None:
             if torch.cuda.is_current_stream_capturing():
                 if self._status_host is None:
@@ -346,11 +363,7 @@
                 self._status_host.copy_(self._status, non_blocking=True)
                 self._status_event = torch.cuda.Event(); self._status_event.record()
             else:
-                snap = self._status_pool.pop() if self._status_pool else torch.zeros(4, dtype=torch.int64).pin_memory()
-                snap.copy_(self._status, non_blocking=True)
-                self._status.fill_(0)
-                ev_s = torch.cuda.Event(); ev_s.record()
-                self._status_pending.append((snap, ev_s))
+                snapshot = True
         if tail_job is None:
             with torch.cuda.stream(pstream if pstream is not None else main):
                 L.check(lib.gs_activation_chain(L.i64(N), L.ptr(g_scales_act), L.ptr(scales_act), L.ptr(g_opac_act), L.ptr(opac_act),
@@ -359,7 +372,7 @@
                 for t in (scales_act, opac_act):
                     t.record_stream(pstream)
         return _Views(b, images if keep_images else None, g_base, g_levels, g_flat, env, sharded, world, all_reduce, main, pstream,
-                      tail_job, smooth_grads)
+                      tail_job, smooth_grads, snapshot=snapshot)
 
     def _step(self, cameras, upstream, all_reduce, keep_images, smoothing: Optional[Smoothing] = None):
         geo = self._geometry(cameras, bin_first=self.prefilter)
@@ -384,6 +397,7 @@
             g_cube = as_splitsum_backward(ctx.g_base, ctx.g_levels, min_roughness=env.min_roughness, max_roughness=env.max_roughness,
                                           rank=dist.get_rank(), world=ctx.world, group=grp, sharded=True)
             b["cubemap"].copy_(g_cube)
+            self._snapshot_status(ctx)
             if pstream is not None:
                 main.wait_stream(pstream)
             self.bucket.all_reduce_names(["exposure"])
@@ -395,10 +409,20 @@
         if self.prefilter:
             as_splitsum_backward(ctx.g_base, ctx.g_levels, min_roughness=env.min_roughness, max_roughness=env.max_roughness,
                                  out=b["cubemap"])
+        self._snapshot_status(ctx)
         if pstream is not None:
             main.wait_stream(pstream)
         finish()
         return b, ctx.images
+
+    def _snapshot_status(self, ctx: _Views) -> None:
+        if not ctx.snapshot:
+            return
+        snap = self._status_pool.pop() if self._status_pool else torch.zeros(4, dtype=torch.int64).pin_memory()
+        snap.copy_(self._status, non_blocking=True)
+        self._status.fill_(0)
+        ev_s = torch.cuda.Event(); ev_s.record()
+        self._status_pending.append((snap, ev_s))
 
     def _chunked_tail(self, ctx: _Views):
         job = ctx.tail_job
diff --git a/geosplatting_amd/front.py b/geosplatting_amd/front.py
--- a/geosplatting_amd/front.py
+++ b/geosplatting_amd/front.py
@@ -33,7 +33,7 @@
                 viewmat: Tensor, K: Tensor, cam_pos: Tensor, env_struct, W: int, H: int, min_roughness: float, max_metallic: float,
                 mode: int, key_base: int = 0, key_bits: int = 32, status: Optional[Tensor] = None, tile_size: int = 16,
                 eps2d: float = 0.3, near: float = 0.01, far: float = 1e10, radius_clip: float = 0.0, want_packed_index: bool = False,
-                records: bool = True, binning: bool = True, tight_tiles: bool = False) -> Front:
+                records: bool = True, binning: bool = True, tight_tiles: bool = False, copy_counts: bool = True) -> Front:
     lib = L.lib()
     dev = means.device
     N = means.shape[0]
@@ -52,10 +52,12 @@
                              C.byref(env_struct) if env_struct is not None else None, W, H, tile_size, L.f32(eps2d), L.f32(near), L.f32(far), L.f32(radius_clip),
                              C.c_uint32(int(key_base) & 0xffffffff), int(key_bits), L.ptr(fr.vis), L.ptr(fr.keys), L.ptr(fr.rects),
                              L.ptr(fr.tile_counts), L.ptr(fr.packed_index), 1 if tight_tiles else 0, L.ptr(fr.counts), L.ptr(status), L.ptr(ws), C.c_size_t(ws_bytes), L.stream()), "gs_front_fwd")
-    fr.host_counts = pinned_counts4()
-    fr.host_counts.copy_(fr.counts, non_blocking=True)
-    fr.event = torch.cuda.Event()
-    fr.event.record()
+    fr.host_counts = fr.event = None
+    if copy_counts:
+        fr.host_counts = pinned_counts4()
+        fr.host_counts.copy_(fr.counts, non_blocking=True)
+        fr.event = torch.cuda.Event()
+        fr.event.record()
     fr.whs = (W, H, tile_size)
     fr.key_bits = int(key_bits)
     fr.N = N
@@ -98,26 +100,43 @@
         counts = None
     else:
         V, I, counts = fr.N, int(i_cap), fr.counts
+    rws_bytes = lib.gs_raster_ws_bytes(L.i64(I), V, W, H, tile_size)
+    rws = None
     if binned is not None:
-        flat, offsets = binned
+        flat, offsets = binned[0], binned[1]
+        rws = binned[2] if len(binned) > 2 else None
+        assert rws is None or rws.numel() == rws_bytes, "binned=: the raster workspace of other sizes"
     else:
         flat = torch.empty(max(I, 1), dtype=torch.int32, device=dev)
         offsets = torch.empty(th * tw, dtype=torch.int32, device=dev)
         bin_bytes = lib.gs_isect_bin_front_ws_bytes(V, L.i64(I), tw, th)
         bin_ws = torch.empty(max(bin_bytes, 1), dtype=torch.uint8, device=dev)
-        L.check(lib.gs_isect_bin_front(V, L.ptr(fr.keys), L.ptr(fr.rects), L.ptr(fr.tile_counts), L.ptr(counts), L.i64(I), fr.key_bits, tw, th,
-                                       L.ptr(flat), L.ptr(offsets), L.ptr(bin_ws), C.c_size_t(bin_bytes),
-                                       L.ptr(status) if counts is not None else None, st), "gs_isect_bin_front")
+        if fr.tile_counts is not None and V > 0 and I > 0:
+            rws = torch.empty(rws_bytes, dtype=torch.uint8, device=dev)
+            order, bcount = C.c_void_p(), C.c_void_p()
+            L.check(lib.gs_raster_ws_order(L.ptr(rws), C.c_size_t(rws_bytes), L.i64(I), V, W, H, tile_size, C.byref(order), C.byref(bcount)),
+                    "gs_raster_ws_order")
+            L.check(lib.gs_isect_bin_front_order(V, L.ptr(fr.keys), L.ptr(fr.rects), L.ptr(fr.tile_counts), L.ptr(counts), L.i64(I), fr.key_bits,
+                                                 tw, th, L.ptr(flat), L.ptr(offsets), L.ptr(bin_ws), C.c_size_t(bin_bytes),
+                                                 L.ptr(status) if counts is not None else None, order, bcount, st), "gs_isect_bin_front_order")
+        else:
+            L.check(lib.gs_isect_bin_front(V, L.ptr(fr.keys), L.ptr(fr.rects), L.ptr(fr.tile_counts), L.ptr(counts), L.i64(I), fr.key_bits, tw, th,
+                                           L.ptr(flat), L.ptr(offsets), L.ptr(bin_ws), C.c_size_t(bin_bytes),
+                                           L.ptr(status) if counts is not None else None, st), "gs_isect_bin_front")
     if not prepare:
-        return dict(flatten_ids=flat, isect_offsets=offsets, counts=counts, keys=fr.keys, rects=fr.rects, tile_counts=fr.tile_counts), V, I
-    rws_bytes = lib.gs_raster_ws_bytes(L.i64(I), V, W, H, tile_size)
-    rws = torch.empty(rws_bytes, dtype=torch.uint8, device=dev)
+        return dict(flatten_ids=flat, isect_offsets=offsets, counts=counts, keys=fr.keys, rects=fr.rects, tile_counts=fr.tile_counts,
+                    raster_ws=rws), V, I
+    ordered = rws is not None
+    if rws is None:
+        rws = torch.empty(rws_bytes, dtype=torch.uint8, device=dev)
     if counts is None:
-        L.check(lib.gs_raster_prepare_vis(W, H, tile_size, 3, V, L.ptr(fr.vis), L.i64(I), L.ptr(offsets), L.ptr(flat), L.ptr(rws),
-                                          C.c_size_t(rws_bytes), st), "gs_raster_prepare_vis")
-    else:
-        L.check(lib.gs_raster_prepare_vis_cap(W, H, tile_size, 3, V, L.ptr(fr.vis), L.i64(I), L.ptr(counts), L.ptr(offsets), L.ptr(flat),
-                                              L.ptr(rws), C.c_size_t(rws_bytes), st), "gs_raster_prepare_vis_cap")
+        prep = lib.gs_raster_prepare_vis_ordered if ordered else lib.gs_raster_prepare_vis
+        L.check(prep(W, H, tile_size, 3, V, L.ptr(fr.vis), L.i64(I), L.ptr(offsets), L.ptr(flat), L.ptr(rws), C.c_size_t(rws_bytes), st),
+                "gs_raster_prepare_vis")
+    else:
+        prep = lib.gs_raster_prepare_vis_ordered_cap if ordered else lib.gs_raster_prepare_vis_cap
+        L.check(prep(W, H, tile_size, 3, V, L.ptr(fr.vis), L.i64(I), L.ptr(counts), L.ptr(offsets), L.ptr(flat), L.ptr(rws),
+                     C.c_size_t(rws_bytes), st), "gs_raster_prepare_vis_cap")
     state = dict(vis_records=fr.vis, flatten_ids=flat, isect_offsets=offsets, raster_ws=rws, counts=counts, keys=fr.keys, rects=fr.rects,
                  tile_counts=fr.tile_counts, packed_index=fr.packed_index)
     return state, V, I
diff --git a/geosplatting_amd/parallel.py b/geosplatting_amd/parallel.py
--- a/geosplatting_amd/parallel.py
+++ b/geosplatting_amd/parallel.py
@@ -40,7 +40,7 @@
         else:
             self.comm_stream = None
 
-    def zero_with_scratch(self, sizes: Sequence[int]) -> List[Tensor]:
+    def zero_with_scratch(self, sizes: Sequence[int], zero_from: Optional[str] = None, n_stored: int = 0) -> List[Tensor]:
         offs, off = [], self.numel
         for n in sizes:
             offs.append(off)
@@ -49,7 +49,9 @@
             self.storage = torch.zeros(off, dtype=torch.float32, device=self.storage.device)
             self.flat = self.storage[:self.numel]
         else:
-            self.storage[:off].zero_()
+            begin = 0 if zero_from is None else self.offsets[zero_from]
+            end = off if n_stored <= 0 else offs[len(sizes) - n_stored]
+            self.storage[begin:end].zero_()
         return [self.storage[o:o + int(n)] for o, n in zip(offs, sizes)]
 
     def view(self, name: str) -> Tensor:
diff --git a/geosplatting_amd/viewbatch.py b/geosplatting_amd/viewbatch.py
--- a/geosplatting_amd/viewbatch.py
+++ b/geosplatting_amd/viewbatch.py
@@ -265,7 +265,7 @@
     for x in (fr.vis, fr.counts, fr.packed_index):
         if x is not None:
             x.record_stream(main)
-    state, V, I = F.bin_stage(fr, i_cap, status, binned=(state["flatten_ids"], state["isect_offsets"]))
+    state, V, I = F.bin_stage(fr, i_cap, status, binned=(state["flatten_ids"], state["isect_offsets"], state["raster_ws"]))
     if v_packed is not None:
         state["v_packed"] = v_packed
     img, render, alphas, last_ids = F.composite_fwd(state, V, I, W, H, tone, exposure, log_ws)
diff --git a/include/geosplat_hip.h b/include/geosplat_hip.h
--- a/include/geosplat_hip.h
+++ b/include/geosplat_hip.h
@@ -310,6 +310,17 @@
 int gs_isect_bin_front(int V_cap, const uint32_t* depth_keys, const uint32_t* tile_rects, const uint32_t* tile_counts,
                        const int64_t* counts_dev, int64_t n_isects_cap, int key_bits, int tile_w, int tile_h, int32_t* flatten_ids_sorted,
                        int32_t* isect_offsets, void* ws, size_t ws_bytes, int64_t* status_dev, void* stream);
+int gs_isect_bin_front_order(int V_cap, const uint32_t* depth_keys, const uint32_t* tile_rects, const uint32_t* tile_counts,
+                             const int64_t* counts_dev, int64_t n_isects_cap, int key_bits, int tile_w, int tile_h,
+                             int32_t* flatten_ids_sorted, int32_t* isect_offsets, void* ws, size_t ws_bytes, int64_t* status_dev,
+                             int32_t* order, int32_t* bcount, void* stream);
+int gs_raster_ws_order(void* ws, size_t ws_bytes, int64_t n_isects, int V, int W, int H, int tile_size, int32_t** order,
+                       int32_t** bcount);
+int gs_raster_prepare_vis_ordered(int W, int H, int tile_size, int D, int V, const float* vis_records, int64_t n_isects,
+                                  const int32_t* offsets, const int32_t* flatten_ids, void* ws, size_t ws_bytes, void* stream);
+int gs_raster_prepare_vis_ordered_cap(int W, int H, int tile_size, int D, int V_cap, const float* vis_records, int64_t n_isects_cap,
+                                      const int64_t* counts_dev, const int32_t* offsets, const int32_t* flatten_ids, void* ws,
+                                      size_t ws_bytes, void* stream);
 int gs_tail_bwd(int V_cap, const int64_t* counts_dev, const float* means, const float* quats, const float* scales,
                 const float* opacities, const float* normals, const float* kd, const float* ks, const float* viewmat,
                 const float* K, const float* cam_pos, float min_roughness, float max_metallic, int mode, const GsEnv* env,
```

After: 771.8, median of 6. About the same (+0.4%).
